# yamiel-abreu/distributed-pytorch-training

Hardware: AMD Instinct MI355X
Metric: images/sec (whole node) ResNet-50 bf16 training (higher is better)
Workload: dtype bf16

## Files before the change

csrc/bindings.cpp:

```cpp
#include <ATen/ATen.h>
#include <c10/hip/HIPGuard.h>
#include <c10/hip/HIPStream.h>
#include <torch/extension.h>

#include "kernels/kernels.h"
#include "host_comm.h"
#include "pg_comm.h"
#include "rccl_comm.h"
#include "watchdog.h"
#include "reducer.h"

namespace py = pybind11;
using at::Tensor;

namespace {

hipStream_t cur_stream(const Tensor& t) {
  return c10::hip::getCurrentHIPStream(t.device().index()).stream();
}

dpt::WireType wire_of(const Tensor& t) {
  switch (t.scalar_type()) {
    case at::kFloat: return dpt::WireType::kF32;
    case at::kBFloat16: return dpt::WireType::kBF16;
// ... 607 lines not shown
  dpt::launch_im2col(x.data_ptr(), x.scalar_type() == at::kBFloat16, reinterpret_cast<uint16_t*>(a.data_ptr()), N, H,
                     W, C, (int)R, (int)S, (int)stride, (int)pad, (int)Kp, cur_stream(x));
  return a;
}

void check_bf16_contig(const Tensor& t, const char* name) {
  TORCH_CHECK(t.is_cuda() && t.scalar_type() == at::kBFloat16 && t.is_contiguous(), name,
              " must be a contiguous bf16 GPU tensor");
  TORCH_CHECK(reinterpret_cast<uintptr_t>(t.data_ptr()) % 16 == 0, name, " must be 16-byte aligned");
}

std::vector<Tensor> attn_fwd(Tensor qkv, int64_t heads, double scale) {
  check_bf16_contig(qkv, "qkv");
  TORCH_CHECK(qkv.dim() == 3 && qkv.size(2) == 3 * heads * 64, "attn_fwd: qkv must be [B, S, 3*H*64]");
  const int B = qkv.size(0), S = qkv.size(1), H = heads;
  TORCH_CHECK(dpt::attn_supported(S, 64), "attn_fwd: needs S <= 256 and head dim 64");
  auto ctx = at::empty({B, S, H * 64}, qkv.options());
  auto lse = at::empty({(int64_t)B * H, dpt::attn_lse_stride(S)}, qkv.options().dtype(at::kFloat));
  if (B * H == 0) return {ctx, lse};
  c10::hip::HIPGuard guard(qkv.device().index());
  dpt::launch_attn_fwd(reinterpret_cast<const uint16_t*>(qkv.data_ptr()), reinterpret_cast<uint16_t*>(ctx.data_ptr()),
                       lse.data_ptr<float>(), B, S, H, (float)scale, cur_stream(qkv));
  return {ctx, lse};
}

Tensor attn_bwd(Tensor qkv, Tensor out, Tensor dout, Tensor lse, int64_t heads, double scale) {
  check_bf16_contig(qkv, "qkv");
  check_bf16_contig(out, "out");
  check_bf16_contig(dout, "grad_output");
  TORCH_CHECK(qkv.dim() == 3, "attn_bwd: qkv must be [B, S, 3*H*64]");
  const int B = qkv.size(0), S = qkv.size(1), H = heads;
  TORCH_CHECK(dpt::attn_supported(S, 64), "attn_bwd: needs S <= 256 and head dim 64");
  TORCH_CHECK(out.sizes() == dout.sizes() && out.dim() == 3 && out.size(0) == B && out.size(1) == S &&
                  out.size(2) == H * 64 && qkv.size(2) == 3 * H * 64, "attn_bwd: shape mismatch");
  TORCH_CHECK(lse.is_cuda() && lse.scalar_type() == at::kFloat && lse.is_contiguous() &&
                  lse.numel() == (int64_t)B * H * dpt::attn_lse_stride(S), "attn_bwd: bad lse");
  auto dqkv = at::empty_like(qkv);
  if (B * H == 0) return dqkv;
  c10::hip::HIPGuard guard(qkv.device().index());
  dpt::launch_attn_bwd(reinterpret_cast<const uint16_t*>(qkv.data_ptr()), reinterpret_cast<const uint16_t*>(out.data_ptr()),
                       reinterpret_cast<const uint16_t*>(dout.data_ptr()), lse.data_ptr<float>(),
                       reinterpret_cast<uint16_t*>(dqkv.data_ptr()), B, S, H, (float)scale, cur_stream(qkv));
  return dqkv;
}

std::vector<Tensor> attn_stream_fwd(Tensor qkv, int64_t heads, double scale) {
  check_bf16_contig(qkv, "qkv");
  TORCH_CHECK(qkv.dim() == 3 && qkv.size(2) == 3 * heads * 64, "attn_stream_fwd: qkv must be [B, S, 3*H*64]");
  const int B = qkv.size(0), S = qkv.size(1), H = heads;
  TORCH_CHECK(dpt::attn_stream_supported(S, 64), "attn_stream_fwd: needs 1 <= S <= 4096 and head dim 64");
  TORCH_CHECK((int64_t)B * H * ((S + 31) / 32) < (1LL << 31), "attn_stream_fwd: B * H * S too large for one grid");
  auto ctx = at::empty({B, S, H * 64}, qkv.options());
  auto lse = at::empty({(int64_t)B * H, dpt::attn_lse_stride(S)}, qkv.options().dtype(at::kFloat));
  if (B * H == 0) return {ctx, lse};
  c10::hip::HIPGuard guard(qkv.device().index());
  dpt::launch_attn_stream_fwd(reinterpret_cast<const uint16_t*>(qkv.data_ptr()),
                              reinterpret_cast<uint16_t*>(ctx.data_ptr()), lse.data_ptr<float>(), B, S, H,
                              (float)scale, cur_stream(qkv));
  return {ctx, lse};
}

Tensor attn_stream_bwd(Tensor qkv, Tensor out, Tensor dout, Tensor lse, int64_t heads, double scale) {
  check_bf16_contig(qkv, "qkv");
  check_bf16_contig(out, "out");
  check_bf16_contig(dout, "grad_output");
  TORCH_CHECK(qkv.dim() == 3, "attn_stream_bwd: qkv must be [B, S, 3*H*64]");
  const int B = qkv.size(0), S = qkv.size(1), H = heads;
  TORCH_CHECK(dpt::attn_stream_supported(S, 64), "attn_stream_bwd: needs 1 <= S <= 4096 and head dim 64");
  TORCH_CHECK(out.sizes() == dout.sizes() && out.dim() == 3 && out.size(0) == B && out.size(1) == S &&
                  out.size(2) == H * 64 && qkv.size(2) == 3 * H * 64, "attn_stream_bwd: shape mismatch");
  TORCH_CHECK(lse.is_cuda() && lse.scalar_type() == at::kFloat && lse.is_contiguous() &&
                  lse.numel() == (int64_t)B * H * dpt::attn_lse_stride(S), "attn_stream_bwd: bad lse");
  TORCH_CHECK((int64_t)B * H * ((S + 31) / 32) < (1LL << 31), "attn_stream_bwd: B * H * S too large for one grid");
  auto dqkv = at::empty_like(qkv);
  if (B * H == 0) return dqkv;
  auto dsum = at::empty_like(lse);
  c10::hip::HIPGuard guard(qkv.device().index());
  dpt::launch_attn_stream_bwd(reinterpret_cast<const uint16_t*>(qkv.data_ptr()),
                              reinterpret_cast<const uint16_t*>(out.data_ptr()),
                              reinterpret_cast<const uint16_t*>(dout.data_ptr()), lse.data_ptr<float>(),
                              dsum.data_ptr<float>(), reinterpret_cast<uint16_t*>(dqkv.data_ptr()), B, S, H,
                              (float)scale, cur_stream(qkv));
  return dqkv;
}

std::tuple<int64_t, int64_t, int64_t> attn_stream_tiles() {
  int qb, kc, qc;
  dpt::attn_stream_tiles(&qb, &kc, &qc);
  return {qb, kc, qc};
}

Tensor space_to_depth2(Tensor x, bool out_f16) {
  TORCH_CHECK(x.is_cuda() && x.dim() == 4 && (x.scalar_type() == at::kFloat || x.scalar_type() == at::kBFloat16),
              "space_to_depth2: x must be a 4-d fp32/bf16 GPU tensor");
  TORCH_CHECK(x.is_contiguous(at::MemoryFormat::ChannelsLast), "space_to_depth2: x must be channels_last");
  const int N = x.size(0), C = x.size(1), H = x.size(2), W = x.size(3);
  TORCH_CHECK(C <= 4 && H % 2 == 0 && W % 2 == 0, "space_to_depth2: needs C <= 4 and even H, W");
  auto a = at::empty({N, 16, H / 2, W / 2},
                     x.options().dtype(out_f16 ? at::kHalf : at::kBFloat16).memory_format(at::MemoryFormat::ChannelsLast));
  c10::hip::HIPGuard guard(x.device().index());
  dpt::launch_space_to_depth2(x.data_ptr(), x.scalar_type() == at::kBFloat16, reinterpret_cast<uint16_t*>(a.data_ptr()),
                              N, H, W, C, cur_stream(x), out_f16);
  return a;
}

std::vector<Tensor> bn_fwd_train(Tensor x, c10::optional<Tensor> residual, c10::optional<Tensor> weight,
                                 c10::optional<Tensor> bias, c10::optional<Tensor> running_mean,
                                 c10::optional<Tensor> running_var, c10::optional<Tensor> num_batches,
                                 double momentum, double eps, bool relu, c10::optional<Tensor> psum,
                                 c10::optional<Tensor> psq, bool apply, c10::optional<Tensor> mask_out) {
  auto [M, C] = bn_rows(x, "x");
  TORCH_CHECK(dpt::bn_supported(C), "fused BN: unsupported channel count ", C);
  const void* rp = nullptr;
  if (residual.has_value() && residual->defined()) {
    TORCH_CHECK(residual->sizes() == x.sizes() && residual->scalar_type() == x.scalar_type(), "residual mismatch");
    bn_rows(*residual, "residual");
    rp = residual->data_ptr();
  }
  int64_t* nb = nullptr;
  if (num_batches.has_value() && num_batches->defined()) {
    TORCH_CHECK(num_batches->is_cuda() && num_batches->scalar_type() == at::kLong, "num_batches must be int64 GPU");
    nb = num_batches->data_ptr<int64_t>();
  }
  auto y = apply ? at::empty_like(x) : at::empty({0}, x.options());
  void* yp = apply ? y.data_ptr() : nullptr;
  auto fopt = x.options().dtype(at::kFloat);
  auto mean = at::empty({C}, fopt), invstd = at::empty({C}, fopt);
  auto coef = at::empty({2 * C}, fopt);
  uint8_t* mp = relu_mask_ptr(mask_out, M, C, x, "bn_fwd_train");
  TORCH_CHECK(mp == nullptr || (relu && rp != nullptr && apply), "bn_fwd_train: mask_out needs relu + residual");
  c10::hip::HIPGuard guard(x.device().index());
  if (psum.has_value() && psum->defined()) {
    TORCH_CHECK(psq.has_value() && psq->defined(), "bn_fwd_train: psum without psq");
    TORCH_CHECK(psum->is_cuda() && psum->scalar_type() == at::kFloat && psum->dim() == 2 && psum->size(0) == C &&
                    psum->is_contiguous() && psq->sizes() == psum->sizes() && psq->is_contiguous(),
                "bn_fwd_train: partials must be contiguous fp32 [C, chunks]");
    dpt::launch_bn_fwd_from_partials(bn_dtype(x), x.data_ptr(), rp, yp, M, C, psum->data_ptr<float>(),
                                     psq->data_ptr<float>(), (int)psum->size(1), f32_param(weight, C, "weight"),
                                     f32_param(bias, C, "bias"), (float)eps, (float)momentum,
                                     f32_param(running_mean, C, "running_mean"),
                                     f32_param(running_var, C, "running_var"), nb, mean.data_ptr<float>(),
                                     invstd.data_ptr<float>(), coef.data_ptr<float>(), relu, cur_stream(x), mp);
    return {y, mean, invstd, coef};
  }
  auto ws = at::empty({dpt::bn_workspace_floats(M, C)}, fopt);
  dpt::launch_bn_fwd_train(bn_dtype(x), x.data_ptr(), rp, yp, M, C, f32_param(weight, C, "weight"),
                           f32_param(bias, C, "bias"), (float)eps, (float)momentum,
                           f32_param(running_mean, C, "running_mean"), f32_param(running_var, C, "running_var"), nb,
                           mean.data_ptr<float>(), invstd.data_ptr<float>(), coef.data_ptr<float>(),
                           ws.data_ptr<float>(), relu, cur_stream(x), mp);
  return {y, mean, invstd, coef};
}

Tensor bn_apply_aff(Tensor x, Tensor x2, Tensor coef, Tensor coef2, c10::optional<Tensor> mask_out) {
  auto [M, C] = bn_rows(x, "x");
  TORCH_CHECK(dpt::bn_supported(C), "fused BN: unsupported channel count ", C);
  TORCH_CHECK(x2.sizes() == x.sizes() && x2.scalar_type() == x.scalar_type(), "bn_apply_aff: x2 mismatch");
  bn_rows(x2, "x2");
  const float* a = f32_param(coef, 2 * C, "coef");
  const float* a2 = f32_param(coef2, 2 * C, "coef2");
  auto y = at::empty_like(x);
  c10::hip::HIPGuard guard(x.device().index());
  uint8_t* mp = relu_mask_ptr(mask_out, M, C, x, "bn_apply_aff");
  dpt::launch_bn_apply_aff(bn_dtype(x), x.data_ptr(), x2.data_ptr(), y.data_ptr(), M, C, a, a + C, a2, a2 + C,
                           cur_stream(x), mp);
  return y;
}

std::vector<Tensor> bn2_bwd_partials(Tensor dz, Tensor x, Tensor x2, c10::optional<Tensor> weight,
                                     c10::optional<Tensor> weight2, Tensor mean, Tensor invstd, Tensor mean2,
                                     Tensor invstd2, Tensor p1, Tensor p2, Tensor p3, bool want_dparams) {
  auto [M, C] = bn_rows(x, "x");
  TORCH_CHECK(dz.sizes() == x.sizes() && x2.sizes() == x.sizes() && dz.scalar_type() == x.scalar_type() &&
                  x2.scalar_type() == x.scalar_type(), "bn2_bwd_partials: shape/dtype mismatch");
  bn_rows(dz, "dz");
  bn_rows(x2, "x2");
  for (const Tensor* t : {&p1, &p2, &p3})
    TORCH_CHECK(t->is_cuda() && t->scalar_type() == at::kFloat && t->dim() == 2 && t->size(0) == C &&
                    t->is_contiguous() && t->sizes() == p1.sizes(), "bn2_bwd_partials: partials must be fp32 [C, chunks]");
  auto fopt = x.options().dtype(at::kFloat);
  auto dx = at::empty_like(x), dx2 = at::empty_like(x2);
  Tensor dg = want_dparams ? at::empty({C}, fopt) : Tensor(), db = want_dparams ? at::empty({C}, fopt) : Tensor();
  Tensor dg2 = want_dparams ? at::empty({C}, fopt) : Tensor(), db2 = want_dparams ? at::empty({C}, fopt) : Tensor();
  auto kbuf = at::empty({6 * C}, fopt);
  c10::hip::HIPGuard guard(x.device().index());
  dpt::launch_bn2_bwd_from_partials(
      bn_dtype(x), dz.data_ptr(), x.data_ptr(), x2.data_ptr(), M, C, f32_param(weight, C, "weight"),
      f32_param(mean, C, "mean"), f32_param(invstd, C, "invstd"), f32_param(weight2, C, "weight2"),
      f32_param(mean2, C, "mean2"), f32_param(invstd2, C, "invstd2"), p1.data_ptr<float>(), p2.data_ptr<float>(),
      p3.data_ptr<float>(), (int)p1.size(1), want_dparams ? dg.data_ptr<float>() : nullptr,
      want_dparams ? db.data_ptr<float>() : nullptr, want_dparams ? dg2.data_ptr<float>() : nullptr,
      want_dparams ? db2.data_ptr<float>() : nullptr, dx.data_ptr(), dx2.data_ptr(), kbuf.data_ptr<float>(),
      cur_stream(x));
  return {dx, dx2, dg, db, dg2, db2};
}

Tensor bn_apply(Tensor x, c10::optional<Tensor> residual, Tensor a, Tensor b, bool relu) {
  auto [M, C] = bn_rows(x, "x");
  TORCH_CHECK(dpt::bn_supported(C), "fused BN: unsupported channel count ", C);
  const void* rp = nullptr;
  if (residual.has_value() && residual->defined()) {
    TORCH_CHECK(residual->sizes() == x.sizes() && residual->scalar_type() == x.scalar_type(), "residual mismatch");
    bn_rows(*residual, "residual");
    rp = residual->data_ptr();
  }
  auto y = at::empty_like(x);
  c10::hip::HIPGuard guard(x.device().index());
  dpt::launch_bn_apply(bn_dtype(x), x.data_ptr(), rp, y.data_ptr(), M, C, f32_param(a, C, "a"),
                       f32_param(b, C, "b"), relu, cur_stream(x));
  return y;
}

std::vector<Tensor> bn_bwd(Tensor dy, c10::optional<Tensor> dy2, c10::optional<Tensor> y, Tensor x,
                           c10::optional<Tensor> weight, Tensor mean, Tensor invstd, bool relu, bool want_dz,
                           bool want_dparams, c10::optional<Tensor> coef) {
  auto [M, C] = bn_rows(x, "x");
  auto [Md, Cd] = bn_rows(dy, "grad_output");
  TORCH_CHECK(M == Md && C == Cd && dy.scalar_type() == x.scalar_type(), "grad_output mismatch");
  const void* d2 = nullptr;
  if (dy2.has_value() && dy2->defined()) {
    auto [M2, C2] = bn_rows(*dy2, "grad_output2");
    TORCH_CHECK(M2 == M && C2 == C && dy2->scalar_type() == x.scalar_type(), "grad_output2 mismatch");
    d2 = dy2->data_ptr();
  }
  const bool make_dz = want_dz || d2 != nullptr;
  const float* cp = nullptr;
  if (relu && !make_dz && coef.has_value() && coef->defined()) cp = f32_param(*coef, 2 * C, "coef");
  const void* yp = nullptr;
  if (relu && cp == nullptr) {
    TORCH_CHECK(y.has_value() && y->defined(), "relu backward needs the saved output (or coef)");
    bn_rows(*y, "y");
    yp = y->data_ptr();
  }
  auto fopt = x.options().dtype(at::kFloat);
  auto dx = at::empty_like(x);
  Tensor dz = make_dz ? at::empty_like(x) : Tensor();
  Tensor dg = want_dparams ? at::empty({C}, fopt) : Tensor();
  Tensor db = want_dparams ? at::empty({C}, fopt) : Tensor();
  auto ws = at::empty({dpt::bn_workspace_floats(M, C)}, fopt);
  c10::hip::HIPGuard guard(x.device().index());
  dpt::launch_bn_bwd(bn_dtype(x), dy.data_ptr(), d2, yp, x.data_ptr(), M, C, f32_param(weight, C, "weight"),
                     f32_param(mean, C, "mean"), f32_param(invstd, C, "invstd"), cp,
                     want_dparams ? dg.data_ptr<float>() : nullptr, want_dparams ? db.data_ptr<float>() : nullptr,
                     dx.data_ptr(), make_dz ? dz.data_ptr() : nullptr, ws.data_ptr<float>(), relu, cur_stream(x));
  return {dx, dg, db, dz};
}

std::vector<Tensor> bn_bwd_partials(Tensor dy, Tensor x, c10::optional<Tensor> weight, Tensor mean, Tensor invstd,
                                    c10::optional<Tensor> coef, Tensor p1, Tensor p2, bool want_dparams, bool from_dz) {
  auto [M, C] = bn_rows(x, "x");
  auto [Md, Cd] = bn_rows(dy, "grad_output");
  TORCH_CHECK(M == Md && C == Cd && dy.scalar_type() == x.scalar_type(), "grad_output mismatch");
  TORCH_CHECK(p1.is_cuda() && p1.scalar_type() == at::kFloat && p1.dim() == 2 && p1.size(0) == C &&
                  p1.is_contiguous() && p2.sizes() == p1.sizes() && p2.is_contiguous(),
              "bn_bwd_partials: partials must be contiguous fp32 [C, chunks]");
  TORCH_CHECK(from_dz || (coef.has_value() && coef->defined()), "bn_bwd_partials: coef needed unless from_dz");
  auto fopt = x.options().dtype(at::kFloat);
  auto dx = at::empty_like(x);
  Tensor dg = want_dparams ? at::empty({C}, fopt) : Tensor();
  Tensor db = want_dparams ? at::empty({C}, fopt) : Tensor();
  auto kbuf = at::empty({3 * C}, fopt);
  c10::hip::HIPGuard guard(x.device().index());
  dpt::launch_bn_bwd_from_partials(bn_dtype(x), dy.data_ptr(), x.data_ptr(), M, C, f32_param(weight, C, "weight"),
                                   f32_param(mean, C, "mean"), f32_param(invstd, C, "invstd"),
                                   f32_param(coef, 2 * C, "coef"), p1.data_ptr<float>(), p2.data_ptr<float>(),
                                   (int)p1.size(1), want_dparams ? dg.data_ptr<float>() : nullptr,
                                   want_dparams ? db.data_ptr<float>() : nullptr, dx.data_ptr(), kbuf.data_ptr<float>(),
                                   cur_stream(x), from_dz);
  return {dx, dg, db};
}

std::vector<Tensor> maxpool_fwd(Tensor x, int64_t k, int64_t stride, int64_t pad, c10::optional<Tensor> bn_coef) {
  TORCH_CHECK(x.is_cuda() && x.dim() == 4 && x.is_contiguous(at::MemoryFormat::ChannelsLast),
              "maxpool: x must be a 4-D channels_last GPU tensor");
  const int64_t B = x.size(0), C = x.size(1), H = x.size(2), W = x.size(3);
  TORCH_CHECK(!(bn_coef.has_value() && bn_coef->defined()) || k == 3, "maxpool: the folded BN needs a 3x3 window");
  TORCH_CHECK(C % 8 == 0 && k >= 1 && k * k <= 255 && stride >= 1 && pad >= 0 && pad <= k / 2, "maxpool: bad config");
  const int64_t Ho = (H + 2 * pad - k) / stride + 1, Wo = (W + 2 * pad - k) / stride + 1;
  auto y = at::empty({B, C, Ho, Wo}, x.options().memory_format(at::MemoryFormat::ChannelsLast));
  auto idx = at::empty({B, C, Ho, Wo}, x.options().dtype(at::kByte).memory_format(at::MemoryFormat::ChannelsLast));
  c10::hip::HIPGuard guard(x.device().index());
  dpt::launch_maxpool_fwd(bn_dtype(x), x.data_ptr(), y.data_ptr(), idx.data_ptr<uint8_t>(), B, (int)H, (int)W,
                          (int)C, (int)Ho, (int)Wo, (int)k, (int)stride, (int)pad, cur_stream(x),
                          bn_coef.has_value() && bn_coef->defined() ? f32_param(bn_coef, 2 * C, "bn_coef") : nullptr);
  
  return {y, idx};
}

std::vector<Tensor> maxpool_bwd(Tensor dy, Tensor idx, int64_t H, int64_t W, int64_t k, int64_t stride, int64_t pad,
                                c10::optional<Tensor> dy2, c10::optional<Tensor> bn_x, c10::optional<Tensor> bn_mean,
                                c10::optional<Tensor> bn_coef) {
  TORCH_CHECK(dy.is_cuda() && dy.dim() == 4 && dy.is_contiguous(at::MemoryFormat::ChannelsLast),
              "maxpool_bwd: grad must be channels_last");
  TORCH_CHECK(idx.sizes() == dy.sizes() && idx.scalar_type() == at::kByte &&
                  idx.is_contiguous(at::MemoryFormat::ChannelsLast), "maxpool_bwd: idx mismatch");
  const int64_t B = dy.size(0), C = dy.size(1), Ho = dy.size(2), Wo = dy.size(3);
  TORCH_CHECK(C % 8 == 0 && Ho == (H + 2 * pad - k) / stride + 1 && Wo == (W + 2 * pad - k) / stride + 1,
              "maxpool_bwd: geometry mismatch");
  const bool two = dy2.has_value() && dy2->defined();
  if (two)
    TORCH_CHECK(dy2->sizes() == dy.sizes() && dy2->scalar_type() == dy.scalar_type() &&
                    dy2->is_contiguous(at::MemoryFormat::ChannelsLast), "maxpool_bwd: dy2 must match grad_output");
  auto dx = at::empty({B, C, H, W}, dy.options().memory_format(at::MemoryFormat::ChannelsLast));
  const bool bns = bn_x.has_value() && bn_x->defined();
  Tensor p1, p2;
  if (bns) {
    TORCH_CHECK(k == 3 && stride == 2 && pad == 1, "maxpool_bwd: BN statistics only for the 3x3/2/1 pool");
    TORCH_CHECK(C <= 512 && (C & (C - 1)) == 0, "maxpool_bwd: BN statistics need a power-of-two C <= 512");
    TORCH_CHECK(bn_x->sizes() == dx.sizes() && bn_x->scalar_type() == dy.scalar_type() &&
                    bn_x->is_contiguous(at::MemoryFormat::ChannelsLast), "maxpool_bwd: bn_x must match dx");
    const int chunks = dpt::maxpool_bwd_bn_chunks(B, (int)H, (int)W, (int)C);
    p1 = at::empty({C, chunks}, dy.options().dtype(at::kFloat));
    p2 = at::empty({C, chunks}, dy.options().dtype(at::kFloat));
  }
  c10::hip::HIPGuard guard(dy.device().index());
  dpt::launch_maxpool_bwd(bn_dtype(dy), dy.data_ptr(), two ? dy2->data_ptr() : nullptr, idx.data_ptr<uint8_t>(),
                          dx.data_ptr(), B, (int)H, (int)W,
                          (int)C, (int)Ho, (int)Wo, (int)k, (int)stride, (int)pad, cur_stream(dy), bns ? bn_x->data_ptr() : nullptr,
                          bns ? f32_param(bn_mean, C, "bn_mean") : nullptr, bns ? f32_param(bn_coef, 2 * C, "bn_coef") : nullptr,
                          bns ? p1.data_ptr<float>() : nullptr, bns ? p2.data_ptr<float>() : nullptr);
  if (bns) return {dx, p1, p2};
  
  return {dx};
}

std::vector<Tensor> gap_bwd_bnr(Tensor g, Tensor y, Tensor x, Tensor mean) {
  TORCH_CHECK(g.is_cuda() && g.dim() == 2 && g.is_contiguous(), "gap_bwd_bnr: g must be a contiguous [N, C]");
  auto [M, C] = bn_rows(y, "y");
  auto [Mx, Cx] = bn_rows(x, "x");
  TORCH_CHECK(M == Mx && C == Cx && x.scalar_type() == y.scalar_type() && g.size(1) == C && g.size(0) == y.size(0),
              "gap_bwd_bnr: shape mismatch");
  TORCH_CHECK(C % 8 == 0 && 256 % (C / 8) == 0, "gap_bwd_bnr: needs C/8 | 256");
  const int64_t N = y.size(0), HW = y.size(2) * y.size(3);
  auto dz = at::empty_like(y);
  const int chunks = dpt::gap_bwd_bnr_chunks(M, C);
  auto p1 = at::empty({C, chunks}, y.options().dtype(at::kFloat));
  auto p2 = at::empty({C, chunks}, y.options().dtype(at::kFloat));
  c10::hip::HIPGuard guard(y.device().index());
  dpt::launch_gap_bwd_bnr(bn_dtype(y), bn_dtype(g), g.data_ptr(), dz.data_ptr(), y.data_ptr(), x.data_ptr(),
                          f32_param(mean, C, "mean"), N, HW, C, p1.data_ptr<float>(), p2.data_ptr<float>(),
                          cur_stream(y));
  return {dz, p1, p2};
}

Tensor gap_bwd(Tensor g, int64_t H, int64_t W, at::ScalarType dtype) {
  TORCH_CHECK(g.is_cuda() && g.dim() == 2 && g.is_contiguous() && g.size(1) % 8 == 0, "gap_bwd: g must be [N, C], C % 8 == 0");
  TORCH_CHECK(dtype == at::kFloat || dtype == at::kBFloat16 || dtype == at::kHalf, "gap_bwd: dtype");
  const int64_t N = g.size(0), C = g.size(1);
  TORCH_CHECK(N * H * W * (C / 8) < (int64_t(1) << 32) - 256, "gap_bwd: too large");
  auto dx = at::empty({N, C, H, W}, g.options().dtype(dtype).memory_format(at::MemoryFormat::ChannelsLast));
  c10::hip::HIPGuard guard(g.device().index());
  dpt::launch_gap_bwd(bn_dtype(dx), bn_dtype(g), g.data_ptr(), dx.data_ptr(), N, H * W, C, cur_stream(g));
  return dx;
}

int act16_kind(const Tensor& t, const char* name) {
  TORCH_CHECK(t.is_cuda() && t.is_contiguous(), name, " must be a contiguous GPU tensor");
  if (t.scalar_type() == at::kBFloat16) return 1;
  TORCH_CHECK(t.scalar_type() == at::kHalf, name, " must be bf16 or fp16");
  return 2;
}

int param_kind(const Tensor& t, int64_t D, const char* name) {
// ... 74 lines not shown
                     want_dparams ? dg.data_ptr<float>() : nullptr, want_dparams ? db.data_ptr<float>() : nullptr,
                     dbias.defined() ? dbias.data_ptr() : nullptr, dbk, T, D, cur_stream(sv));
  return {gx, ga, dg, db, dbias};
}

Tensor gelu_fwd(Tensor u, c10::optional<Tensor> bias) {
  const int kind = act16_kind(u, "gelu: u");
  const int64_t F = u.size(-1), T = u.numel() / F;
  TORCH_CHECK(F % 8 == 0, "gelu: width must be a multiple of 8");
  const void* bp = nullptr;
  int bk = 0;
  if (bias.has_value() && bias->defined()) {
    bk = param_kind(*bias, F, "gelu: bias");
    bp = bias->data_ptr();
  }
  auto h = at::empty_like(u);
  c10::hip::HIPGuard guard(u.device().index());
  dpt::launch_gelu_fwd(kind, static_cast<const uint16_t*>(u.data_ptr()), bp, bk, static_cast<uint16_t*>(h.data_ptr()),
                       T, F, cur_stream(u));
  return h;
}

std::vector<Tensor> gelu_bwd(Tensor gh, Tensor u, c10::optional<Tensor> bias, bool want_dbias) {
  const int kind = act16_kind(u, "gelu_bwd: u");
  TORCH_CHECK(act16_kind(gh, "gelu_bwd: grad") == kind && gh.sizes() == u.sizes(), "gelu_bwd: grad must match u");
  const int64_t F = u.size(-1), T = u.numel() / F;
  TORCH_CHECK(F % 8 == 0, "gelu_bwd: width must be a multiple of 8");
  const void* bp = nullptr;
  int bk = 0;
  if (bias.has_value() && bias->defined()) {
    bk = param_kind(*bias, F, "gelu_bwd: bias");
    bp = bias->data_ptr();
  }
  auto gu = at::empty_like(u);
  Tensor db = (want_dbias && bp) ? at::empty({F}, u.options().dtype(bias->scalar_type())) : Tensor();
  auto part = at::empty({(int64_t)dpt::gelu_bwd_chunks(T, F) * F}, u.options().dtype(at::kFloat));
  c10::hip::HIPGuard guard(u.device().index());
  dpt::launch_gelu_bwd(kind, static_cast<const uint16_t*>(gh.data_ptr()), static_cast<const uint16_t*>(u.data_ptr()),
                       bp, bk, static_cast<uint16_t*>(gu.data_ptr()), part.data_ptr<float>(),
                       db.defined() ? db.data_ptr() : nullptr, bk, T, F, cur_stream(u));
  return {gu, db};
}

std::vector<Tensor> linear_dgrad_dgelu(Tensor dy, Tensor wt, Tensor u, Tensor bias) {
  const int kind = act16_kind(u, "linear_dgrad_dgelu: u");
  TORCH_CHECK(act16_kind(dy, "linear_dgrad_dgelu: grad") == kind && act16_kind(wt, "linear_dgrad_dgelu: wt") == kind,
              "linear_dgrad_dgelu: grad, wt and u must share one 16-bit dtype");
  TORCH_CHECK(dy.dim() == 2 && wt.dim() == 2 && u.dim() == 2 && dy.is_contiguous() && wt.is_contiguous() &&
                  u.is_contiguous(), "linear_dgrad_dgelu: contiguous 2-D operands");
  const int64_t T = dy.size(0), n_out = dy.size(1), n_in = wt.size(0);
  TORCH_CHECK(wt.size(1) == n_out && u.size(0) == T && u.size(1) == n_in, "linear_dgrad_dgelu: shape mismatch");
  TORCH_CHECK(n_in % 128 == 0 && n_out % 64 == 0, "linear_dgrad_dgelu: n_in % 128 == 0 and n_out % 64 == 0");
  const bool b16 = bias.scalar_type() == u.scalar_type();
  TORCH_CHECK((b16 || bias.scalar_type() == at::kFloat) && bias.is_contiguous() && bias.numel() == n_in &&
                  bias.is_cuda(), "linear_dgrad_dgelu: fp32 or u-typed bias of n_in elements on the device");
  TORCH_CHECK(T * n_out < (1ll << 31) && T * n_in < (1ll << 31), "linear_dgrad_dgelu: too many elements");
  auto gu = at::empty_like(u);
  auto part = at::empty({(int64_t)dpt::linear_dgrad_dgelu_tiles(T), n_in}, u.options().dtype(at::kFloat));
  c10::hip::HIPGuard guard(u.device().index());
  dpt::launch_linear_dgrad_dgelu(static_cast<const uint16_t*>(dy.data_ptr()), static_cast<const uint16_t*>(wt.data_ptr()),
                                 static_cast<const uint16_t*>(u.data_ptr()),
                                 b16 ? nullptr : bias.data_ptr<float>(),
                                 b16 ? static_cast<const uint16_t*>(bias.data_ptr()) : nullptr,
                                 static_cast<uint16_t*>(gu.data_ptr()), part.data_ptr<float>(), T, (int)n_out,
                                 (int)n_in, kind == 2, cur_stream(u));
  return {gu, part};
}

Tensor bias_grad16(Tensor gy, int64_t out_kind) {
  const int kind = act16_kind(gy, "bias_grad16: grad");
  const int64_t F = gy.size(-1), T = gy.numel() / F;
  TORCH_CHECK(F % 8 == 0 && (out_kind >= 0 && out_kind <= 2), "bias_grad16: F % 8 == 0, kind 0..2");
  auto db = at::empty({F}, gy.options().dtype(out_kind == 0 ? at::kFloat : kind_dtype((int)out_kind)));
  auto part = at::empty({(int64_t)dpt::gelu_bwd_chunks(T, F) * F}, gy.options().dtype(at::kFloat));
  c10::hip::HIPGuard guard(gy.device().index());
  dpt::launch_bias_grad16(kind, static_cast<const uint16_t*>(gy.data_ptr()), part.data_ptr<float>(), db.data_ptr(),
                          (int)out_kind, T, F, cur_stream(gy));
  return db;
}

Tensor sum_partials(Tensor part, int64_t out_kind) {
  TORCH_CHECK(part.is_cuda() && part.scalar_type() == at::kFloat && part.is_contiguous() && part.dim() >= 2,
              "sum_partials: contiguous fp32 [S, ...]");
  const int64_t S = part.size(0), n = part.numel() / S;
  TORCH_CHECK(n % 4 == 0 && out_kind >= 0 && out_kind <= 2, "sum_partials: n % 4 == 0, kind 0..2");
  auto out = at::empty(part.sizes().slice(1),
                       part.options().dtype(out_kind == 0 ? at::kFloat : kind_dtype((int)out_kind)));
  c10::hip::HIPGuard guard(part.device().index());
  dpt::launch_sum_partials(part.data_ptr<float>(), n, (int)S, out.data_ptr(), (int)out_kind, cur_stream(part));
  return out;
}

Tensor colsum_rows(Tensor part, int64_t out_kind) {
  TORCH_CHECK(part.is_cuda() && part.scalar_type() == at::kFloat && part.is_contiguous() && part.dim() == 2,
              "colsum_rows: contiguous fp32 [n, D]");
  TORCH_CHECK(out_kind >= 0 && out_kind <= 2, "colsum_rows: kind 0..2");
  auto out = at::empty({part.size(1)}, part.options().dtype(out_kind == 0 ? at::kFloat : kind_dtype((int)out_kind)));
  c10::hip::HIPGuard guard(part.device().index());
  dpt::launch_colsum_rows(part.data_ptr<float>(), part.size(0), part.size(1), out.data_ptr(), (int)out_kind,
                          cur_stream(part));
  return out;
}

void copy_rows16(Tensor src, Tensor dst) {
  TORCH_CHECK(src.is_cuda() && dst.is_cuda() && src.device() == dst.device(), "copy_rows16: GPU tensors");
  TORCH_CHECK(src.scalar_type() == dst.scalar_type() && src.element_size() == 2, "copy_rows16: same 16-bit dtype");
  TORCH_CHECK(src.sizes() == dst.sizes() && src.dim() >= 1 && src.dim() <= 5, "copy_rows16: same shape, <= 5 dims");
  const int nd = (int)src.dim();
  const int64_t L = src.size(nd - 1);
  TORCH_CHECK(src.stride(nd - 1) == 1 && dst.stride(nd - 1) == 1 && L % 8 == 0, "copy_rows16: rows must be contiguous, L % 8 == 0");
  TORCH_CHECK(reinterpret_cast<uintptr_t>(src.data_ptr()) % 16 == 0 && reinterpret_cast<uintptr_t>(dst.data_ptr()) % 16 == 0,
              "copy_rows16: 16-byte aligned data");
  int n[4] = {1, 1, 1, 1};
  int64_t ss[4] = {0, 0, 0, 0}, ds[4] = {0, 0, 0, 0};
  for (int d = 0; d < nd - 1; ++d) {
    const int slot = 4 - (nd - 1) + d;
    TORCH_CHECK(src.size(d) < (1LL << 31), "copy_rows16: dim too large");
    TORCH_CHECK(src.stride(d) % 8 == 0 && dst.stride(d) % 8 == 0, "copy_rows16: row starts must be 16-byte aligned");
    n[slot] = (int)src.size(d);
    ss[slot] = src.stride(d);
    ds[slot] = dst.stride(d);
  }
  TORCH_CHECK((int64_t)n[0] * n[1] * n[2] * n[3] < (1LL << 32), "copy_rows16: too many rows");
  c10::hip::HIPGuard guard(src.device().index());
  dpt::launch_rows_copy16(static_cast<const uint16_t*>(src.data_ptr()), static_cast<uint16_t*>(dst.data_ptr()), n, ss,
                          ds, (int)L, cur_stream(src));
}

}

PYBIND11_MODULE(TORCH_EXTENSION_NAME, m) {
  m.doc() = "MI355X-native runtime: gfx950 kernels, RCCL communicator, C++ gradient reducer";
  m.def("grad_check", &grad_check, py::arg("grad"), py::arg("scale"), py::arg("host_factor"), py::arg("found_inf"));
  m.def("sgd_step", &sgd_step, py::arg("param"), py::arg("grad"), py::arg("momentum_buffer"), py::arg("lr"),
        py::arg("momentum"), py::arg("dampening"), py::arg("weight_decay"), py::arg("nesterov"), py::arg("scale"),
        py::arg("host_factor"), py::arg("found_inf"), py::arg("step"), py::arg("zero_grad"),
        py::arg("shadow") = py::none());
  m.def("adam_step", &adam_step, py::arg("param"), py::arg("grad"), py::arg("exp_avg"), py::arg("exp_avg_sq"),
        py::arg("lr"), py::arg("beta1"), py::arg("beta2"), py::arg("eps"), py::arg("weight_decay"), py::arg("adamw"),
        py::arg("scale"), py::arg("host_factor"), py::arg("found_inf"), py::arg("step"), py::arg("zero_grad"),
        py::arg("shadow") = py::none());
  m.def("optim_tail", &optim_tail, py::arg("scale"), py::arg("growth_tracker"), py::arg("found_inf"),
        py::arg("step"), py::arg("growth_factor"), py::arg("backoff_factor"), py::arg("growth_interval"));
  m.def("pack_bf16", &pack_bf16);
  m.def("unpack_bf16", &unpack_bf16);
  m.def("accumulate_metrics", &accumulate_metrics, py::arg("logits"), py::arg("targets"), py::arg("loss"), py::arg("acc"));
  m.def("augment", &augment, py::arg("data"), py::arg("idx"), py::arg("offs"), py::arg("flips"), py::arg("out"),
        py::arg("nhwc"), py::arg("pad"), py::arg("mean"), py::arg("std"));
  m.def("bn_supported", [](int64_t C) { return dpt::bn_supported(C); });
  m.def("bn_fwd_train", &bn_fwd_train, py::arg("x"), py::arg("residual"), py::arg("weight"), py::arg("bias"),
        py::arg("running_mean"), py::arg("running_var"), py::arg("num_batches"), py::arg("momentum"), py::arg("eps"),
        py::arg("relu"), py::arg("psum") = py::none(), py::arg("psq") = py::none(), py::arg("apply") = true,
        py::arg("mask_out") = py::none());
  m.def("bn_apply", &bn_apply, py::arg("x"), py::arg("residual"), py::arg("a"), py::arg("b"), py::arg("relu"));
  m.def("bn_apply_aff", &bn_apply_aff, py::arg("x"), py::arg("x2"), py::arg("coef"), py::arg("coef2"),
        py::arg("mask_out") = py::none());
  m.def("bn2_bwd_partials", &bn2_bwd_partials, py::arg("dz"), py::arg("x"), py::arg("x2"), py::arg("weight"),
        py::arg("weight2"), py::arg("mean"), py::arg("invstd"), py::arg("mean2"), py::arg("invstd2"), py::arg("p1"),
        py::arg("p2"), py::arg("p3"), py::arg("want_dparams"));
  m.def("bn_bwd", &bn_bwd, py::arg("grad_output"), py::arg("grad_output2"), py::arg("y"), py::arg("x"),
        py::arg("weight"), py::arg("mean"), py::arg("invstd"), py::arg("relu"), py::arg("want_dz"),
        py::arg("want_dparams"), py::arg("coef") = py::none());
  m.def("ln_supported", &dpt::ln_supported, py::arg("D"));
  m.def("ln_fwd", &ln_fwd, py::arg("x"), py::arg("a"), py::arg("bias"), py::arg("gamma"), py::arg("beta"),
        py::arg("eps"), py::arg("out_kind") = 1);
  m.def("ln_bwd", &ln_bwd, py::arg("grad_s"), py::arg("grad_h"), py::arg("s"), py::arg("mean"), py::arg("rstd"),
        py::arg("gamma"), py::arg("want_ga"), py::arg("bias_like"), py::arg("want_dparams"));
  m.def("gelu_fwd", &gelu_fwd, py::arg("u"), py::arg("bias"));
  m.def("gelu_bwd", &gelu_bwd, py::arg("grad"), py::arg("u"), py::arg("bias"), py::arg("want_dbias"));
  m.def("linear_dgrad_dgelu", &linear_dgrad_dgelu, py::arg("grad"), py::arg("wt"), py::arg("u"), py::arg("bias"));
  m.def("vit_set_gelu_blocks_per_cu", &dpt::vit_set_gelu_blocks_per_cu, py::arg("n"));
  m.def("copy_rows16", &copy_rows16, py::arg("src"), py::arg("dst"));
  m.def("bias_grad16", &bias_grad16, py::arg("grad"), py::arg("out_kind"));
  m.def("sum_partials", &sum_partials, py::arg("part"), py::arg("out_kind"));
  m.def("colsum_rows", &colsum_rows, py::arg("part"), py::arg("out_kind"));
  m.def("maxpool_fwd", &maxpool_fwd, py::arg("x"), py::arg("k"), py::arg("stride"), py::arg("pad"),
        py::arg("bn_coef") = py::none());
  m.def("gap_bwd", &gap_bwd, py::arg("g"), py::arg("H"), py::arg("W"), py::arg("dtype"));
  m.def("gap_bwd_bnr", &gap_bwd_bnr, py::arg("g"), py::arg("y"), py::arg("x"), py::arg("mean"));
  m.def("maxpool_bwd", &maxpool_bwd, py::arg("grad_output"), py::arg("idx"), py::arg("H"), py::arg("W"),
        py::arg("k"), py::arg("stride"), py::arg("pad"), py::arg("grad_output2") = py::none(),
        py::arg("bn_x") = py::none(), py::arg("bn_mean") = py::none(), py::arg("bn_coef") = py::none());
  m.def("conv_fwd", &conv_fwd, py::arg("x"), py::arg("w"), py::arg("stride"), py::arg("pad"), py::arg("want_stats"),
        py::arg("out_h") = 0, py::arg("out_w") = 0);
  m.def("space_to_depth2", &space_to_depth2, py::arg("x"), py::arg("out_f16") = false);
  m.def("conv_wgrad", &conv_wgrad, py::arg("grad_output"), py::arg("x"), py::arg("weight_shape"), py::arg("stride"),
        py::arg("pad"), py::arg("fp32_out"), py::arg("target_blocks") = 0);
  m.def("conv_f32_fwd", &conv_f32_fwd, py::arg("x"), py::arg("w"), py::arg("stride"), py::arg("pad"),
        py::arg("split") = false);
  m.def("conv_f32_dgrad", &conv_f32_dgrad, py::arg("grad_output"), py::arg("w"), py::arg("stride"), py::arg("pad"),
        py::arg("H"), py::arg("W"), py::arg("split") = false);
  m.def("conv_f32_wgrad", &conv_f32_wgrad, py::arg("grad_output"), py::arg("x"), py::arg("weight_shape"),
        py::arg("stride"), py::arg("pad"), py::arg("split") = false);
  m.def("im2col", &im2col, py::arg("x"), py::arg("R"), py::arg("S"), py::arg("stride"), py::arg("pad"), py::arg("Kp"));
  m.def("attn_fwd", &attn_fwd, py::arg("qkv"), py::arg("heads"), py::arg("scale"));
  m.def("attn_set_bwd_split", &dpt::attn_set_bwd_split, py::arg("on"));
  m.def("attn_bwd", &attn_bwd, py::arg("qkv"), py::arg("out"), py::arg("grad_output"), py::arg("lse"),
        py::arg("heads"), py::arg("scale"));
  m.def("attn_stream_fwd", &attn_stream_fwd, py::arg("qkv"), py::arg("heads"), py::arg("scale"));
  m.def("attn_stream_bwd", &attn_stream_bwd, py::arg("qkv"), py::arg("out"), py::arg("grad_output"), py::arg("lse"),
        py::arg("heads"), py::arg("scale"));
  m.def("attn_stream_tiles", &attn_stream_tiles,
        "(queries per workgroup, keys per chunk, query rows per backward chunk) of the streaming attention kernels");
  m.def("conv_set_variant", &dpt::conv_set_variant, py::arg("variant"));
  m.def("bn_set_skip_finalize", &dpt::bn_set_skip_finalize, py::arg("on"),
        "measurement only: skip every BatchNorm finalize launch (wrong values; timing upper bound)");
  m.def("conv_set_splitk_policy", &dpt::conv_set_splitk_policy, py::arg("tiles"), py::arg("eager_tiles"),
        py::arg("eager_min_k"), py::arg("target"), "split-K thresholds (A/B knob; <= 0 keeps a value)");
  m.def("conv_set_big", &dpt::conv_set_big, py::arg("on"));
  m.def("conv_set_halo", &dpt::conv_set_halo, py::arg("on"));
  m.def("conv_set_breg", &dpt::conv_set_breg, py::arg("mode"));
  m.def("conv_set_wgrad_stages", &dpt::conv_set_wgrad_stages, py::arg("mode"));
  m.def("conv_get_breg", &dpt::conv_get_breg);
  m.def("conv_set_streamk", &dpt::conv_set_streamk, py::arg("mode"), py::arg("eff") = 0.0);
  m.def("conv_get_streamk", &dpt::conv_get_streamk);
  m.def("conv_sk_prepare", &dpt::conv_sk_prepare);
  m.def("conv_sk_errors", &dpt::conv_sk_errors);
  m.def("conv_sk_blocks", &dpt::conv_sk_blocks, py::arg("tiles"), py::arg("nk"), py::arg("bn"), py::arg("mode"));
  m.def("conv_set_wgrad_target", &dpt::conv_set_wgrad_target, py::arg("blocks"));
  m.def("conv_set_wgrad_halo", &dpt::conv_set_wgrad_halo, py::arg("mode"));
  m.def("conv_fwd_splits", [](int64_t M, int Cout, int64_t K, bool graph) {
          return dpt::conv_fwd_splits_for(M, Cout, K, graph);
        }, py::arg("M"), py::arg("Cout"), py::arg("K"), py::arg("graph") = false);
  m.def("conv_set_splitk", &dpt::conv_set_splitk, py::arg("mode"));
  m.def("conv_get_splitk", &dpt::conv_get_splitk);
  m.def("conv_set_fwd_shape_policy", &dpt::conv_set_fwd_shape_policy, py::arg("bits"));
  m.def("conv_dgrad", &conv_dgrad, py::arg("grad_output"), py::arg("w"), py::arg("pad"));
  m.def("conv_dgrad_bnstats", &conv_dgrad_bnstats, py::arg("grad_output"), py::arg("w"), py::arg("pad"),
        py::arg("bn_x"), py::arg("bn_mean"), py::arg("bn_coef"), py::arg("bn_y") = py::none(),
        py::arg("bn_res") = py::none(), py::arg("w_flipped") = py::none(), py::arg("bn_x2") = py::none(),
        py::arg("bn_mean2") = py::none(), py::arg("wgrad_reduce") = nullptr, py::arg("bn_mask") = py::none(),
        py::arg("bn_res_s2") = false);
  m.def("conv_wt_flip_multi", &conv_wt_flip_multi, py::arg("ws"));
  m.def("conv_dgrad_preflipped", &conv_dgrad_preflipped, py::arg("grad_output"), py::arg("w_flipped"), py::arg("pad"),
        py::arg("wgrad_reduce") = nullptr);
  m.def("bn_bwd_partials", &bn_bwd_partials, py::arg("grad_output"), py::arg("x"), py::arg("weight"), py::arg("mean"),
        py::arg("invstd"), py::arg("coef"), py::arg("p1"), py::arg("p2"), py::arg("want_dparams"),
        py::arg("from_dz") = false);
  m.def("conv_dgrad_s2", &conv_dgrad_s2, py::arg("grad_output"), py::arg("w"), py::arg("pad"), py::arg("H"),
        py::arg("W"), py::arg("bn_x") = py::none(), py::arg("bn_mean") = py::none(), py::arg("bn_coef") = py::none(),
        py::arg("wgrad_reduce") = nullptr, py::arg("compact") = false);
  m.def("conv_dgrad_flip", &conv_dgrad_flip, py::arg("grad_output"), py::arg("w"), py::arg("pad"),
        py::arg("wgrad_reduce") = nullptr);
  py::class_<PendingReduce, PendingReducePtr>(m, "PendingWgradReduce")
      .def_property_readonly("done", &PendingReduce::done)
      .def_property_readonly("splits", [](const PendingReduce& p) { return p.r.splits; });
  m.def("conv_wgrad_deferred", &conv_wgrad_deferred, py::arg("grad_output"), py::arg("x"), py::arg("weight_shape"),
        py::arg("stride"), py::arg("pad"));
  m.def("conv_reduce_flush", &conv_reduce_flush, py::arg("pending"));
  m.def("rccl_version", []() { return std::string(dpt::rccl_version_string()); });

  py::class_<dpt::Collective, std::shared_ptr<dpt::Collective>>(m, "Collective")
      .def("all_reduce", [](dpt::Collective& c, Tensor t, bool on_current_stream) {
             TORCH_CHECK(t.is_cuda() && t.is_contiguous(), "all_reduce needs a contiguous GPU tensor");
             c10::hip::HIPGuard guard(t.device().index());
             hipStream_t s = cur_stream(t);
             c.all_reduce(t.data_ptr(), (size_t)t.numel(), wire_of(t), on_current_stream ? s : c.stream());
           }, py::arg("tensor"), py::arg("on_current_stream") = true)
      .def("broadcast", [](dpt::Collective& c, Tensor t, int root) {
             TORCH_CHECK(t.is_cuda() && t.is_contiguous(), "broadcast needs a contiguous GPU tensor");
             c10::hip::HIPGuard guard(t.device().index());
             c.broadcast(t.data_ptr(), (size_t)t.numel(), wire_of(t), root, cur_stream(t));
           }, py::arg("tensor"), py::arg("root") = 0)
      .def("abort", &dpt::Collective::abort)
      .def("destroy", &dpt::Collective::destroy)
      .def("check", &dpt::Collective::check)
      .def_property_readonly("kind", &dpt::Collective::kind)
      .def_property_readonly("ops", &dpt::Collective::ops)
      .def_property_readonly("sequence_hash", &dpt::Collective::sequence_hash)
      .def_property_readonly("rank", &dpt::Collective::rank)
      .def_property_readonly("world_size", &dpt::Collective::world_size)
      .def_property_readonly("device", &dpt::Collective::device)
      .def("track", [](dpt::Collective& c) {
             c10::hip::HIPGuard guard(c.device());
             c.track(c10::hip::getCurrentHIPStream(c.device()).stream());
           }, "hand the watchdog a completion marker for the work enqueued on the current stream")
      .def("_test_spin", [](dpt::Collective& c, double ms, bool on_current_stream) {
             TORCH_CHECK(ms >= 0 && ms <= 20000, "spin: 0..20000 ms");
             c10::hip::HIPGuard guard(c.device());
             dpt::launch_spin(ms, on_current_stream ? c10::hip::getCurrentHIPStream(c.device()).stream()
                                                    : c.stream());
           }, py::arg("ms"), py::arg("on_current_stream") = false,
           "test hook: enqueue a wall-clock busy-wait on the communicator (or current) stream");

  py::class_<dpt::RcclComm, dpt::Collective, std::shared_ptr<dpt::RcclComm>>(m, "RcclComm")
      .def(py::init<const std::string&, int, int, int, int, int, double>(), py::arg("unique_id"), py::arg("rank"),
           py::arg("world_size"), py::arg("device"), py::arg("min_ctas") = 0, py::arg("max_ctas") = 0,
           py::arg("init_timeout_s") = 0.0,
           py::call_guard<py::gil_scoped_release>())
      .def_property_readonly("min_ctas", &dpt::RcclComm::min_ctas)
      .def_property_readonly("max_ctas", &dpt::RcclComm::max_ctas)
      .def_property_readonly("handle", &dpt::RcclComm::handle)
      .def("inject_async_error", &dpt::RcclComm::inject_async_error, py::arg("message"))
      .def_static("new_unique_id", []() { return py::bytes(dpt::RcclComm::new_unique_id()); })
      .def("enable_watchdog", &dpt::RcclComm::enable_watchdog, py::arg("timeout_s"), py::arg("poll_s") = 0.5,
           py::arg("exit_grace_s") = 30.0)
      .def_property_readonly("watchdog_tripped", &dpt::RcclComm::watchdog_tripped)
      .def_property_readonly("watchdog_outstanding", &dpt::RcclComm::watchdog_outstanding)
      .def_property_readonly("watchdog_tracked", &dpt::RcclComm::watchdog_tracked)
      .def("async_error", &dpt::RcclComm::async_error);

  py::class_<dpt::HostBridgeComm, dpt::Collective, std::shared_ptr<dpt::HostBridgeComm>>(m, "HostBridgeComm")
      .def(py::init([](py::object ar, py::object bc, int rank, int ws, int dev, bool async_mode, py::object pg) {
             c10::intrusive_ptr<c10d::ProcessGroup> p;
             if (!pg.is_none()) p = pg.cast<c10::intrusive_ptr<c10d::ProcessGroup>>();
             return std::make_shared<dpt::HostBridgeComm>(std::move(ar), std::move(bc), rank, ws, dev, async_mode,
                                                          std::move(p));
           }),
           py::arg("all_reduce_fn"), py::arg("broadcast_fn"), py::arg("rank"), py::arg("world_size"),
// ... 56 lines not shown
```

csrc/kernels/bn_kernels.hip:

```cpp
#include <cstdlib>

#include "carry.h"
#include "common.h"
#include "kernels.h"

namespace dpt {

struct BF16 {
  using raw = uint16_t;
  __device__ static void load8(const void* p, int64_t i, float f[8]) {
    uint4 w = *reinterpret_cast<const uint4*>(static_cast<const uint16_t*>(p) + i);
    uint32_t u[4] = {w.x, w.y, w.z, w.w};
#pragma unroll
    for (int k = 0; k < 4; ++k) {
      f[2 * k] = bf16_to_f32(u[k] & 0xffff);
      f[2 * k + 1] = bf16_to_f32(u[k] >> 16);
    }
  }
  __device__ static void store8(void* p, int64_t i, const float f[8]) {
    uint4 w;
    w.x = (uint32_t)f32_to_bf16(f[0]) | ((uint32_t)f32_to_bf16(f[1]) << 16);
    w.y = (uint32_t)f32_to_bf16(f[2]) | ((uint32_t)f32_to_bf16(f[3]) << 16);
    w.z = (uint32_t)f32_to_bf16(f[4]) | ((uint32_t)f32_to_bf16(f[5]) << 16);
    w.w = (uint32_t)f32_to_bf16(f[6]) | ((uint32_t)f32_to_bf16(f[7]) << 16);
    *reinterpret_cast<uint4*>(static_cast<uint16_t*>(p) + i) = w;
  }
  __device__ static bool pos16(uint32_t h) { return !(h & 0x8000u) && (h & 0x7fffu) && (h & 0x7fffu) <= 0x7f80u; }
  __device__ static uint32_t store8m(void* p, int64_t i, const float f[8]) {
    uint32_t h[8];
#pragma unroll
    for (int k = 0; k < 8; ++k) h[k] = f32_to_bf16(f[k]);
    *reinterpret_cast<uint4*>(static_cast<uint16_t*>(p) + i) =
        make_uint4(h[0] | (h[1] << 16), h[2] | (h[3] << 16), h[4] | (h[5] << 16), h[6] | (h[7] << 16));
    uint32_t m = 0;
#pragma unroll
    for (int k = 0; k < 8; ++k) m |= (pos16(h[k]) ? 1u : 0u) << k;
    return m;
  }
  __device__ static void pos8(const void* p, int64_t i, bool m[8]) {
    uint4 w = *reinterpret_cast<const uint4*>(static_cast<const uint16_t*>(p) + i);
    uint32_t u[4] = {w.x, w.y, w.z, w.w};
#pragma unroll
    for (int k = 0; k < 4; ++k) {
      uint16_t lo = u[k] & 0xffff, hi = u[k] >> 16;
      m[2 * k] = !(lo & 0x8000) && (lo & 0x7fff) && (lo & 0x7fff) <= 0x7f80;
      m[2 * k + 1] = !(hi & 0x8000) && (hi & 0x7fff) && (hi & 0x7fff) <= 0x7f80;
    }
  }
};

struct F16 {
  __device__ static void load8(const void* p, int64_t i, float f[8]) {
    uint4 w = *reinterpret_cast<const uint4*>(static_cast<const uint16_t*>(p) + i);
    uint32_t u[4] = {w.x, w.y, w.z, w.w};
#pragma unroll
    for (int k = 0; k < 4; ++k) {
      f[2 * k] = f16_to_f32(u[k] & 0xffff);
      f[2 * k + 1] = f16_to_f32(u[k] >> 16);
    }
  }
  __device__ static uint16_t to16(float v) { return __builtin_bit_cast(uint16_t, (_Float16)v); }
  __device__ static void store8(void* p, int64_t i, const float f[8]) {
    uint4 w;
    w.x = (uint32_t)to16(f[0]) | ((uint32_t)to16(f[1]) << 16);
    w.y = (uint32_t)to16(f[2]) | ((uint32_t)to16(f[3]) << 16);
    w.z = (uint32_t)to16(f[4]) | ((uint32_t)to16(f[5]) << 16);
    w.w = (uint32_t)to16(f[6]) | ((uint32_t)to16(f[7]) << 16);
    *reinterpret_cast<uint4*>(static_cast<uint16_t*>(p) + i) = w;
  }
  __device__ static uint32_t store8m(void* p, int64_t i, const float f[8]) {
    store8(p, i, f);
    uint32_t m = 0;
#pragma unroll
    for (int k = 0; k < 8; ++k) m |= ((float)__builtin_bit_cast(_Float16, to16(f[k])) > 0.0f ? 1u : 0u) << k;
    return m;
  }
  __device__ static void pos8(const void* p, int64_t i, bool m[8]) {
    float f[8];
    load8(p, i, f);
#pragma unroll
    for (int k = 0; k < 8; ++k) m[k] = f[k] > 0.0f;
  }
};

struct F32 {
  __device__ static void load8(const void* p, int64_t i, float f[8]) {
    const float4* q = reinterpret_cast<const float4*>(static_cast<const float*>(p) + i);
    float4 a = q[0], b = q[1];
    f[0] = a.x; f[1] = a.y; f[2] = a.z; f[3] = a.w; f[4] = b.x; f[5] = b.y; f[6] = b.z; f[7] = b.w;
  }
  __device__ static void store8(void* p, int64_t i, const float f[8]) {
    float4* q = reinterpret_cast<float4*>(static_cast<float*>(p) + i);
    q[0] = make_float4(f[0], f[1], f[2], f[3]);
    q[1] = make_float4(f[4], f[5], f[6], f[7]);
  }
  __device__ static uint32_t store8m(void* p, int64_t i, const float f[8]) {
    store8(p, i, f);
    uint32_t m = 0;
#pragma unroll
    for (int k = 0; k < 8; ++k) m |= (f[k] > 0.0f ? 1u : 0u) << k;
    return m;
  }
  __device__ static void pos8(const void* p, int64_t i, bool m[8]) {
    float f[8];
    load8(p, i, f);
#pragma unroll
    for (int k = 0; k < 8; ++k) m[k] = f[k] > 0.0f;
  }
};

template <typename IO>
__global__ __launch_bounds__(kBlock) void bn_fwd_stats_kernel(const void* __restrict__ x, int64_t M, int C,
                                                              int64_t rows_per_chunk, int chunks,
                                                              float* __restrict__ psum,
                                                              float* __restrict__ psq) {
  __shared__ float lds[2 * kBlock * 8];
  const int tpr = C >> 3, rpi = kBlock / tpr;
  const int cg = threadIdx.x % tpr, rr = threadIdx.x / tpr;
  const int64_t row0 = (int64_t)blockIdx.x * rows_per_chunk;
  const int64_t row1 = min(row0 + rows_per_chunk, M);
  float s[8] = {0, 0, 0, 0, 0, 0, 0, 0}, q[8] = {0, 0, 0, 0, 0, 0, 0, 0};
  int64_t r = row0 + rr;
  for (; r + 3 * rpi < row1; r += 4 * rpi) {
    float a[4][8];
#pragma unroll
    for (int u = 0; u < 4; ++u) IO::load8(x, (r + u * rpi) * C + cg * 8, a[u]);
#pragma unroll
    for (int u = 0; u < 4; ++u)
#pragma unroll
      for (int k = 0; k < 8; ++k) {
        s[k] += a[u][k];
        q[k] += a[u][k] * a[u][k];
      }
  }
  for (; r < row1; r += rpi) {
    float a[8];
    IO::load8(x, r * C + cg * 8, a);
#pragma unroll
    for (int k = 0; k < 8; ++k) { s[k] += a[k]; q[k] += a[k] * a[k]; }
  }
  float* ls = lds;
  float* lq = lds + kBlock * 8;
#pragma unroll
  for (int k = 0; k < 8; ++k) {
    ls[rr * C + cg * 8 + k] = s[k];
    lq[rr * C + cg * 8 + k] = q[k];
  }
  __syncthreads();
  for (int c = threadIdx.x; c < C; c += kBlock) {
    float ts = 0.f, tq = 0.f;
    for (int j = 0; j < rpi; ++j) { ts += ls[j * C + c]; tq += lq[j * C + c]; }
    psum[(int64_t)c * chunks + blockIdx.x] = ts;
    psq[(int64_t)c * chunks + blockIdx.x] = tq;
  }
}

__global__ __launch_bounds__(kBlock) void bn_fwd_finalize_kernel(
    const float* __restrict__ psum, const float* __restrict__ psq, int chunks, int C, int64_t M,
    const float* __restrict__ gamma, const float* __restrict__ beta, float eps, float momentum,
    float* run_mean, float* run_var, int64_t* num_batches, float* save_mean, float* save_invstd,
    float* coef_a, float* coef_b) {
  const int lane = threadIdx.x & 63, wave = threadIdx.x >> 6;
  const int64_t c = (int64_t)blockIdx.x * 8 + wave * 2 + (lane >> 5);
  const int part = lane & 31;
  if (blockIdx.x == 0 && threadIdx.x == 0 && num_batches) num_batches[0] += 1;
  if (c >= C) return;
  double s, q;
  half_wave_sum2(psum, psq, c, chunks, part, s, q);
  if (part != 0) return;
  const double mean = s / (double)M;
  double var = q / (double)M - mean * mean;
  if (var < 0.0) var = 0.0;
  const float invstd = (float)(1.0 / sqrt(var + (double)eps));
  const float g = gamma ? gamma[c] : 1.0f, bt = beta ? beta[c] : 0.0f;
  const float a = g * invstd;
  save_mean[c] = (float)mean;
  save_invstd[c] = invstd;
  coef_a[c] = a;
  coef_b[c] = bt - (float)mean * a;
  if (run_mean) {
    const double unbiased = M > 1 ? var * (double)M / (double)(M - 1) : var;
    run_mean[c] = (1.0f - momentum) * run_mean[c] + momentum * (float)mean;
    run_var[c] = (1.0f - momentum) * run_var[c] + momentum * (float)unbiased;
  }
}


template <int NT>
__global__ __launch_bounds__(NT) void bn_fwd_finalize_wide_kernel(
    const float* __restrict__ psum, const float* __restrict__ psq, int chunks, int C, int64_t M,
    const float* __restrict__ gamma, const float* __restrict__ beta, float eps, float momentum,
    float* run_mean, float* run_var, int64_t* num_batches, float* save_mean, float* save_invstd,
    float* coef_a, float* coef_b) {
  __shared__ double red[2][NT / 64];
  const int c = blockIdx.x, lane = threadIdx.x & 63, wave = threadIdx.x >> 6;
  if (c == 0 && threadIdx.x == 0 && num_batches) num_batches[0] += 1;
  double s, q;
  block_row_sum2<NT>(psum + (int64_t)c * chunks, psq + (int64_t)c * chunks, chunks, s, q);
  if (lane == 0) { red[0][wave] = s; red[1][wave] = q; }
  __syncthreads();
  if (threadIdx.x != 0) return;
  s = 0.0;
  q = 0.0;
#pragma unroll
  for (int w = 0; w < NT / 64; ++w) { s += red[0][w]; q += red[1][w]; }
  const double mean = s / (double)M;
  double var = q / (double)M - mean * mean;
  if (var < 0.0) var = 0.0;
  const float invstd = (float)(1.0 / sqrt(var + (double)eps));
  const float g = gamma ? gamma[c] : 1.0f, bt = beta ? beta[c] : 0.0f;
  const float a = g * invstd;
  save_mean[c] = (float)mean;
  save_invstd[c] = invstd;
  coef_a[c] = a;
  coef_b[c] = bt - (float)mean * a;
  if (run_mean) {
    const double unbiased = M > 1 ? var * (double)M / (double)(M - 1) : var;
    run_mean[c] = (1.0f - momentum) * run_mean[c] + momentum * (float)mean;
    run_var[c] = (1.0f - momentum) * run_var[c] + momentum * (float)unbiased;
  }
}

template <typename IO, bool RELU, bool RES, bool AFF = false>
__global__ __launch_bounds__(kBlock) void bn_fwd_apply_kernel(const void* __restrict__ x,
                                                              const void* __restrict__ res,
                                                              void* __restrict__ y,
                                                              const float* __restrict__ coef_a,
                                                              const float* __restrict__ coef_b,
                                                              int64_t M, int C, int rev,
                                                              const float* __restrict__ coef_a2 = nullptr,
                                                              const float* __restrict__ coef_b2 = nullptr,
                                                              uint8_t* __restrict__ mask = nullptr) {
  const int tpr = C >> 3, rpi = kBlock / tpr;
  const int cg = threadIdx.x % tpr, rr = threadIdx.x / tpr;
  float a[8], b[8], a2[8], b2[8];
#pragma unroll
  for (int k = 0; k < 8; ++k) {
    a[k] = coef_a[cg * 8 + k];
    b[k] = coef_b[cg * 8 + k];
    a2[k] = AFF ? coef_a2[cg * 8 + k] : 0.f;
    b2[k] = AFF ? coef_b2[cg * 8 + k] : 0.f;
  }
  const int64_t stride = (int64_t)gridDim.x * rpi;
  for (int64_t rf = (int64_t)blockIdx.x * rpi + rr; rf < M; rf += 2 * stride) {
    const bool two = rf + stride < M;
    const int64_t r = rev ? M - 1 - rf : rf;
    const int64_t r2 = rev ? r - stride : r + stride;
    float v0[8], v1[8], q0[8], q1[8];
    IO::load8(x, r * C + cg * 8, v0);
    if (two) IO::load8(x, r2 * C + cg * 8, v1);
    if (RES) {
      IO::load8(res, r * C + cg * 8, q0);
      if (two) IO::load8(res, r2 * C + cg * 8, q1);
    }
#pragma unroll
    for (int k = 0; k < 8; ++k) {
      float o0 = __builtin_fmaf(v0[k], a[k], b[k]);
      float o1 = __builtin_fmaf(v1[k], a[k], b[k]);
      if (RES && AFF) {
        o0 += __builtin_fmaf(q0[k], a2[k], b2[k]);
        o1 += __builtin_fmaf(q1[k], a2[k], b2[k]);
      } else if (RES) {
// ... 173 lines not shown
    mu[k] = mean[cg * 8 + k];
    c1[k] = k1[cg * 8 + k];
    c2[k] = k2[cg * 8 + k];
    c3[k] = k3[cg * 8 + k];
    fa[k] = MX ? coef[cg * 8 + k] : 0.f;
    fb[k] = MX ? coef[C + cg * 8 + k] : 0.f;
  }
  const int64_t stride = (int64_t)apply_grid * rpi;
  for (int64_t rf = (int64_t)blockIdx.x * rpi + rr; rf < M; rf += stride) {
    const int64_t r = rev ? M - 1 - rf : rf;
    float g[8], xv[8], o[8];
    bool m[8];
    IO::load8(dy, r * C + cg * 8, g);
    IO::load8(x, r * C + cg * 8, xv);
    if (RELU && !FROM_DZ) relu_mask8<IO, MX>(y, r * C + cg * 8, xv, fa, fb, m);
#pragma unroll
    for (int k = 0; k < 8; ++k) {
      float dz = (FROM_DZ || !RELU || m[k]) ? g[k] : 0.0f;
      o[k] = c1[k] * dz + c2[k] * (xv[k] - mu[k]) + c3[k];
    }
    IO::store8(dx, r * C + cg * 8, o);
  }
}

template <typename IO>
__global__ __launch_bounds__(kBlock) void bn_bwd_apply2_kernel(const void* __restrict__ dz,
                                                               const void* __restrict__ x,
                                                               const void* __restrict__ x2,
                                                               const float* __restrict__ mean,
                                                               const float* __restrict__ mean2,
                                                               const float* __restrict__ k,
                                                               const float* __restrict__ j, void* dx, void* dx2,
                                                               int64_t M, int C, int rev) {
  const int tpr = C >> 3, rpi = kBlock / tpr;
  const int cg = threadIdx.x % tpr, rr = threadIdx.x / tpr;
  float mu[8], mu2[8], c1[8], c2[8], c3[8], e1[8], e2[8], e3[8];
#pragma unroll
  for (int q = 0; q < 8; ++q) {
    const int c = cg * 8 + q;
    mu[q] = mean[c];
    mu2[q] = mean2[c];
    c1[q] = k[c]; c2[q] = k[C + c]; c3[q] = k[2 * C + c];
    e1[q] = j[c]; e2[q] = j[C + c]; e3[q] = j[2 * C + c];
  }
  const int64_t stride = (int64_t)gridDim.x * rpi;
  for (int64_t rf = (int64_t)blockIdx.x * rpi + rr; rf < M; rf += stride) {
    const int64_t r = rev ? M - 1 - rf : rf;
    const int64_t off = r * C + cg * 8;
    float g[8], xv[8], x2v[8], o[8], o2[8];
    IO::load8(dz, off, g);
    IO::load8(x, off, xv);
    IO::load8(x2, off, x2v);
#pragma unroll
    for (int q = 0; q < 8; ++q) {
      o[q] = c1[q] * g[q] + c2[q] * (xv[q] - mu[q]) + c3[q];
      o2[q] = e1[q] * g[q] + e2[q] * (x2v[q] - mu2[q]) + e3[q];
    }
    IO::store8(dx, off, o);
    IO::store8(dx2, off, o2);
  }
}

bool bn_supported(int64_t C) {
  return C >= 8 && C % 8 == 0 && C <= 8 * kBlock && kBlock % (C / 8) == 0;
}

constexpr int kBnMaxChunks = 512;
constexpr int kBnBwdUnroll = 2;
constexpr int kBnApplyMax = 32768;
constexpr int kBnBwdApplyMax = 4 * kMaxBlocks;
constexpr int kBnReverse = 1;

BnGeometry bn_geometry(int64_t M, int64_t C) {
  BnGeometry g;
  const int64_t rpi = kBlock / (C / 8);
  int64_t rows = (M + kBnMaxChunks - 1) / kBnMaxChunks;
  if (rows < 64) rows = 64;
  rows = (rows + rpi - 1) / rpi * rpi;
  g.rows_per_chunk = rows;
  g.chunks = (int)((M + rows - 1) / rows);
  if (g.chunks < 1) g.chunks = 1;
  int64_t apply = (M + rpi * 2 - 1) / (rpi * 2);
  g.apply_blocks = (int)(apply < 1 ? 1 : (apply > kBnApplyMax ? kBnApplyMax : apply));
  return g;
}

template <typename IO>
static void fwd_apply_dispatch(bool relu, bool res, const void* x, const void* r, void* y, const float* a,
                               const float* b, int64_t M, int C, int blocks, hipStream_t s, uint8_t* mask = nullptr) {
  dim3 gr(blocks), bl(kBlock);
  const int rev = kBnReverse;
  if (relu && res)
    hipLaunchKernelGGL((bn_fwd_apply_kernel<IO, true, true>), gr, bl, 0, s, x, r, y, a, b, M, C, rev, nullptr, nullptr,
                       mask);
  else if (relu) hipLaunchKernelGGL((bn_fwd_apply_kernel<IO, true, false>), gr, bl, 0, s, x, r, y, a, b, M, C, rev);
  else if (res) hipLaunchKernelGGL((bn_fwd_apply_kernel<IO, false, true>), gr, bl, 0, s, x, r, y, a, b, M, C, rev);
  else hipLaunchKernelGGL((bn_fwd_apply_kernel<IO, false, false>), gr, bl, 0, s, x, r, y, a, b, M, C, rev);
}

void launch_bn_fwd_train(int dtype, const void* x, const void* res, void* y, int64_t M, int64_t C,
                         const float* gamma, const float* beta, float eps, float momentum, float* run_mean,
                         float* run_var, int64_t* num_batches, float* save_mean, float* save_invstd,
                         float* save_coef, float* workspace, bool relu, hipStream_t s, uint8_t* mask) {
  BnGeometry g = bn_geometry(M, C);
  float* psum = workspace;
  float* psq = psum + (int64_t)C * g.chunks;
  float* ca = save_coef ? save_coef : psq + (int64_t)C * g.chunks;
  float* cb = ca + C;
  dim3 bl(kBlock);
  switch (dtype) {
    case 0: hipLaunchKernelGGL(bn_fwd_stats_kernel<F32>, dim3(g.chunks), bl, 0, s, x, M, (int)C, g.rows_per_chunk, g.chunks, psum, psq); break;
    case 1: hipLaunchKernelGGL(bn_fwd_stats_kernel<BF16>, dim3(g.chunks), bl, 0, s, x, M, (int)C, g.rows_per_chunk, g.chunks, psum, psq); break;
    default: hipLaunchKernelGGL(bn_fwd_stats_kernel<F16>, dim3(g.chunks), bl, 0, s, x, M, (int)C, g.rows_per_chunk, g.chunks, psum, psq); break;
  }
  hipLaunchKernelGGL(bn_fwd_finalize_kernel, dim3((unsigned)((C + 7) / 8)), bl, 0, s, psum, psq, g.chunks, (int)C, M,
                     gamma, beta, eps, momentum, run_mean, run_var, num_batches, save_mean, save_invstd, ca, cb);
  if (y == nullptr) return;
  switch (dtype) {
    case 0: fwd_apply_dispatch<F32>(relu, res != nullptr, x, res, y, ca, cb, M, (int)C, g.apply_blocks, s, mask); break;
    case 1: fwd_apply_dispatch<BF16>(relu, res != nullptr, x, res, y, ca, cb, M, (int)C, g.apply_blocks, s, mask); break;
    default: fwd_apply_dispatch<F16>(relu, res != nullptr, x, res, y, ca, cb, M, (int)C, g.apply_blocks, s, mask); break;
  }
}

void launch_bn_fwd_from_partials(int dtype, const void* x, const void* res, void* y, int64_t M, int64_t C,
                                 const float* psum, const float* psq, int chunks, const float* gamma,
                                 const float* beta, float eps, float momentum, float* run_mean, float* run_var,
                                 int64_t* num_batches, float* save_mean, float* save_invstd, float* save_coef,
                                 bool relu, hipStream_t s, uint8_t* mask) {
  BnGeometry g = bn_geometry(M, C);
  float* ca = save_coef;
  float* cb = ca + C;
  if (g_bn_skip_finalize) {
  } else if (chunks > 256) {
#define DPT_FWD_FIN(NT)                                                                                        \
  hipLaunchKernelGGL(bn_fwd_finalize_wide_kernel<NT>, dim3((unsigned)C), dim3(NT), 0, s, psum, psq, chunks, (int)C, \
                     M, gamma, beta, eps, momentum, run_mean, run_var, num_batches, save_mean, save_invstd, ca, cb)
    if (chunks > 8192) DPT_FWD_FIN(1024);
    else DPT_FWD_FIN(kBlock);
#undef DPT_FWD_FIN
  } else
    hipLaunchKernelGGL(bn_fwd_finalize_kernel, dim3((unsigned)((C + 7) / 8)), dim3(kBlock), 0, s, psum, psq, chunks,
                       (int)C, M, gamma, beta, eps, momentum, run_mean, run_var, num_batches, save_mean, save_invstd,
                       ca, cb);
  if (y == nullptr) return;
  switch (dtype) {
    case 0: fwd_apply_dispatch<F32>(relu, res != nullptr, x, res, y, ca, cb, M, (int)C, g.apply_blocks, s, mask); break;
    case 1: fwd_apply_dispatch<BF16>(relu, res != nullptr, x, res, y, ca, cb, M, (int)C, g.apply_blocks, s, mask); break;
    default: fwd_apply_dispatch<F16>(relu, res != nullptr, x, res, y, ca, cb, M, (int)C, g.apply_blocks, s, mask); break;
  }
}

void launch_bn_apply(int dtype, const void* x, const void* res, void* y, int64_t M, int64_t C,
                     const float* coef_a, const float* coef_b, bool relu, hipStream_t s) {
  BnGeometry g = bn_geometry(M, C);
  switch (dtype) {
    case 0: fwd_apply_dispatch<F32>(relu, res != nullptr, x, res, y, coef_a, coef_b, M, (int)C, g.apply_blocks, s); break;
    case 1: fwd_apply_dispatch<BF16>(relu, res != nullptr, x, res, y, coef_a, coef_b, M, (int)C, g.apply_blocks, s); break;
    default: fwd_apply_dispatch<F16>(relu, res != nullptr, x, res, y, coef_a, coef_b, M, (int)C, g.apply_blocks, s); break;
  }
}

template <typename IO, int UNR>
static void bwd_stats_dispatch(bool relu, const void* dy, const void* dy2, const void* y, const void* x,
                               const float* mean, const float* coef, int64_t M, int C, const BnGeometry& g,
                               float* p1, float* p2, void* dz, hipStream_t s) {
  dim3 bl(kBlock), gs(g.chunks);
  const int64_t rpc = g.rows_per_chunk;
#define DPT_BN_STATS(R, T, W, MXV) \
  hipLaunchKernelGGL((bn_bwd_stats_kernel<IO, R, T, W, UNR, MXV>), gs, bl, 0, s, dy, dy2, y, x, mean, coef, M, C, \
                     rpc, g.chunks, p1, p2, dz)
  if (dz != nullptr) {
    if (relu && dy2) DPT_BN_STATS(true, true, true, false);
    else if (relu) DPT_BN_STATS(true, false, true, false);
    else if (dy2) DPT_BN_STATS(false, true, true, false);
    else DPT_BN_STATS(false, false, true, false);
  } else {
    if (relu && coef) DPT_BN_STATS(true, false, false, true);
    else if (relu) DPT_BN_STATS(true, false, false, false);
    else DPT_BN_STATS(false, false, false, false);
  }
#undef DPT_BN_STATS
}

template <typename IO>
static void bwd_dispatch(bool relu, const void* dy, const void* dy2, const void* y, const void* x,
                         const float* mean, const float* coef, int64_t M, int C, const BnGeometry& g, float* p1,
                         float* p2, const float* gamma, const float* invstd, float* dgamma, float* dbeta,
                         float* k1, float* k2, float* k3, void* dx, void* dz, hipStream_t s) {
  dim3 bl(kBlock);
  bwd_stats_dispatch<IO, kBnBwdUnroll>(relu, dy, dy2, y, x, mean, coef, M, C, g, p1, p2, dz, s);
  launch_bn_bwd_fin(make_bn_bwd_fin(p1, p2, g.chunks, C, M, gamma, invstd, dgamma, dbeta, k1, k2, k3, 0), s);
  dim3 ga(g.apply_blocks * 2 > kBnBwdApplyMax ? kBnBwdApplyMax : g.apply_blocks * 2);
  if (dz != nullptr) hipLaunchKernelGGL((bn_bwd_apply_kernel<IO, false, true, false>), ga, bl, 0, s, dz, y, x, mean, coef, k1, k2, k3, dx, M, C, kBnReverse, ReduceCarry{});
  else if (relu && coef) hipLaunchKernelGGL((bn_bwd_apply_kernel<IO, true, false, true>), ga, bl, 0, s, dy, y, x, mean, coef, k1, k2, k3, dx, M, C, kBnReverse, ReduceCarry{});
  else if (relu) hipLaunchKernelGGL((bn_bwd_apply_kernel<IO, true, false, false>), ga, bl, 0, s, dy, y, x, mean, coef, k1, k2, k3, dx, M, C, kBnReverse, ReduceCarry{});
  else hipLaunchKernelGGL((bn_bwd_apply_kernel<IO, false, false, false>), ga, bl, 0, s, dy, y, x, mean, coef, k1, k2, k3, dx, M, C, kBnReverse, ReduceCarry{});
}

void launch_bn_bwd(int dtype, const void* dy, const void* dy2, const void* y, const void* x, int64_t M,
                   int64_t C, const float* gamma, const float* mean, const float* invstd, const float* coef,
                   float* dgamma, float* dbeta, void* dx, void* dz, float* workspace, bool relu, hipStream_t s) {
  BnGeometry g = bn_geometry(M, C);
  float* p1 = workspace;
  float* p2 = p1 + (int64_t)C * g.chunks;
  float* k1 = p2 + (int64_t)C * g.chunks;
  float* k2 = k1 + C;
  float* k3 = k2 + C;
  switch (dtype) {
    case 0: bwd_dispatch<F32>(relu, dy, dy2, y, x, mean, dz ? nullptr : coef, M, (int)C, g, p1, p2, gamma, invstd, dgamma, dbeta, k1, k2, k3, dx, dz, s); break;
    case 1: bwd_dispatch<BF16>(relu, dy, dy2, y, x, mean, dz ? nullptr : coef, M, (int)C, g, p1, p2, gamma, invstd, dgamma, dbeta, k1, k2, k3, dx, dz, s); break;
    default: bwd_dispatch<F16>(relu, dy, dy2, y, x, mean, dz ? nullptr : coef, M, (int)C, g, p1, p2, gamma, invstd, dgamma, dbeta, k1, k2, k3, dx, dz, s); break;
  }
}


void launch_bn_bwd_apply_pre(int dtype, const void* dy, const void* x, int64_t M, int64_t C, const float* mean,
                             const float* coef, const float* kbuf, void* dx, hipStream_t s, bool from_dz) {
  BnGeometry g = bn_geometry(M, C);
  const float* k1 = kbuf;
  const float* k2 = k1 + C;
  const float* k3 = k2 + C;
  dim3 bl(kBlock);
  ReduceCarry rc;
  const int ga = (g.apply_blocks * 2 > kBnBwdApplyMax ? kBnBwdApplyMax : g.apply_blocks * 2) +
                 take_attached_reduce(rc);
  if (from_dz) {
    switch (dtype) {
      case 0: hipLaunchKernelGGL((bn_bwd_apply_kernel<F32, false, true, false>), dim3(ga), bl, 0, s, dy, nullptr, x, mean, coef, k1, k2, k3, dx, M, (int)C, kBnReverse, rc); break;
      case 1: hipLaunchKernelGGL((bn_bwd_apply_kernel<BF16, false, true, false>), dim3(ga), bl, 0, s, dy, nullptr, x, mean, coef, k1, k2, k3, dx, M, (int)C, kBnReverse, rc); break;
      default: hipLaunchKernelGGL((bn_bwd_apply_kernel<F16, false, true, false>), dim3(ga), bl, 0, s, dy, nullptr, x, mean, coef, k1, k2, k3, dx, M, (int)C, kBnReverse, rc); break;
    }
    return;
  }
  switch (dtype) {
    case 0: hipLaunchKernelGGL((bn_bwd_apply_kernel<F32, true, false, true>), dim3(ga), bl, 0, s, dy, nullptr, x, mean, coef, k1, k2, k3, dx, M, (int)C, kBnReverse, rc); break;
    case 1: hipLaunchKernelGGL((bn_bwd_apply_kernel<BF16, true, false, true>), dim3(ga), bl, 0, s, dy, nullptr, x, mean, coef, k1, k2, k3, dx, M, (int)C, kBnReverse, rc); break;
    default: hipLaunchKernelGGL((bn_bwd_apply_kernel<F16, true, false, true>), dim3(ga), bl, 0, s, dy, nullptr, x, mean, coef, k1, k2, k3, dx, M, (int)C, kBnReverse, rc); break;
  }
}

void launch_bn_bwd_from_partials(int dtype, const void* dy, const void* x, int64_t M, int64_t C, const float* gamma,
                                 const float* mean, const float* invstd, const float* coef, const float* p1,
                                 const float* p2, int chunks, float* dgamma, float* dbeta, void* dx, float* kbuf,
                                 hipStream_t s, bool from_dz) {
  BnGeometry g = bn_geometry(M, C);
  float* k1 = kbuf;
  float* k2 = k1 + C;
  float* k3 = k2 + C;
  dim3 bl(kBlock);
  launch_bn_bwd_fin(make_bn_bwd_fin(p1, p2, chunks, (int)C, M, gamma, invstd, dgamma, dbeta, k1, k2, k3, -1), s);
  launch_bn_bwd_apply_pre(dtype, dy, x, M, C, mean, coef, kbuf, dx, s, from_dz);
}

void launch_bn_apply_aff(int dtype, const void* x, const void* x2, void* y, int64_t M, int64_t C, const float* a,
                         const float* b, const float* a2, const float* b2, hipStream_t s, uint8_t* mask) {
  BnGeometry g = bn_geometry(M, C);
  dim3 gr(g.apply_blocks), bl(kBlock);
  switch (dtype) {
    case 0: hipLaunchKernelGGL((bn_fwd_apply_kernel<F32, true, true, true>), gr, bl, 0, s, x, x2, y, a, b, M, (int)C, kBnReverse, a2, b2, mask); break;
    case 1: hipLaunchKernelGGL((bn_fwd_apply_kernel<BF16, true, true, true>), gr, bl, 0, s, x, x2, y, a, b, M, (int)C, kBnReverse, a2, b2, mask); break;
    default: hipLaunchKernelGGL((bn_fwd_apply_kernel<F16, true, true, true>), gr, bl, 0, s, x, x2, y, a, b, M, (int)C, kBnReverse, a2, b2, mask); break;
  }
}

void launch_bn2_bwd_from_partials(int dtype, const void* dz, const void* x, const void* x2, int64_t M, int64_t C,
                                  const float* gamma, const float* mean, const float* invstd, const float* gamma2,
                                  const float* mean2, const float* invstd2, const float* p1, const float* p2,
                                  const float* p3, int chunks, float* dgamma, float* dbeta, float* dgamma2,
                                  float* dbeta2, void* dx, void* dx2, float* kbuf, hipStream_t s) {
  BnGeometry g = bn_geometry(M, C);
  float* k = kbuf;
  float* j = kbuf + 3 * C;
  dim3 bl(kBlock);
  const BnBwdFin f1 = make_bn_bwd_fin(p1, p2, chunks, (int)C, M, gamma, invstd, dgamma, dbeta, k, k + C, k + 2 * C, -1);
  const BnBwdFin f2 =
      make_bn_bwd_fin(p1, p3, chunks, (int)C, M, gamma2, invstd2, dgamma2, dbeta2, j, j + C, j + 2 * C, -1);
  if (!g_bn_skip_finalize)
    hipLaunchKernelGGL(bn_bwd_finalize2_kernel, dim3((unsigned)(f1.blocks + f2.blocks)), dim3(kBlock), 0, s, f1, f2);
  dim3 ga(g.apply_blocks * 2 > kBnBwdApplyMax ? kBnBwdApplyMax : g.apply_blocks * 2);
  switch (dtype) {
    case 0: hipLaunchKernelGGL(bn_bwd_apply2_kernel<F32>, ga, bl, 0, s, dz, x, x2, mean, mean2, k, j, dx, dx2, M, (int)C, kBnReverse); break;
    case 1: hipLaunchKernelGGL(bn_bwd_apply2_kernel<BF16>, ga, bl, 0, s, dz, x, x2, mean, mean2, k, j, dx, dx2, M, (int)C, kBnReverse); break;
    default: hipLaunchKernelGGL(bn_bwd_apply2_kernel<F16>, ga, bl, 0, s, dz, x, x2, mean, mean2, k, j, dx, dx2, M, (int)C, kBnReverse); break;
  }
}

int64_t bn_workspace_floats(int64_t M, int64_t C) {
  BnGeometry g = bn_geometry(M, C);
  return 2 * (int64_t)C * g.chunks + 3 * C;
}

}
```

csrc/kernels/conv_kernels.hip:

```cpp
#include <algorithm>
#include <cmath>
#include <cstdlib>
#include <mutex>
#include <stdexcept>
#include <type_traits>

#include "carry.h"
#include "gelu.h"
#include "common.h"
#include "kernels.h"
#include "mfma.h"

namespace dpt {


#ifndef DPT_WGRAD_WAVES
#define DPT_WGRAD_WAVES 4
#endif
#ifndef DPT_CONV_HALF_EPI
#define DPT_CONV_HALF_EPI 0
#endif

namespace conv {

constexpr int BM = 128;
constexpr int BK = 64;
constexpr int kThreads = 256;
constexpr int kRowBytes = BK * 2;

__device__ __forceinline__ int swz(int row, int chunk) { return chunk ^ ((row >> 1) & 7); }

__device__ __forceinline__ int opaque_v(int v) {
  asm volatile("" : "+v"(v));
  return v;
}

__device__ __forceinline__ int xcd_remap(int bid, int nwg) {
  const int q = nwg >> 3, r = nwg & 7, xcd = bid & 7, idx = bid >> 3;
  return (xcd < r ? xcd * (q + 1) : r * (q + 1) + (xcd - r) * q) + idx;
}

}

typedef _Float16 f16x8_t __attribute__((ext_vector_type(8)));
typedef _Float16 f16x2_t __attribute__((ext_vector_type(2)));

template <bool F16>
__device__ __forceinline__ f32x16_t cmfma(bf16x8_t a, bf16x8_t b, f32x16_t c) {
  if constexpr (F16)
    return __builtin_amdgcn_mfma_f32_32x32x16_f16(__builtin_bit_cast(f16x8_t, a), __builtin_bit_cast(f16x8_t, b), c,
                                                  0, 0, 0);
  else
    return __builtin_amdgcn_mfma_f32_32x32x16_bf16(a, b, c, 0, 0, 0);
}
template <bool F16>
__device__ __forceinline__ uint32_t cpack(f32x2_t v) {
  if constexpr (F16) return __builtin_bit_cast(uint32_t, __builtin_convertvector(v, f16x2_t));
  else return __builtin_bit_cast(uint32_t, __builtin_convertvector(v, bf16x2_t));
}
template <bool F16>
__device__ __forceinline__ float cunpack(uint32_t u, int h) {
  if constexpr (F16) return (float)__builtin_bit_cast(_Float16, (uint16_t)(h ? (u >> 16) : (u & 0xffffu)));
  else return __uint_as_float(h ? (u & 0xffff0000u) : (u << 16));
}

struct ConvSk {
  float* part = nullptr;
  unsigned* flags = nullptr;
  unsigned* err = nullptr;
  int G = 0;
  uint32_t part_bytes = 0;
};

struct ConvFwdArgs {
  const uint16_t* x = nullptr;
  const uint16_t* w = nullptr;
  uint16_t* y = nullptr;
  float* psum = nullptr;
  float* psq = nullptr;
  int N = 0, H = 0, W = 0, C = 0, Ho = 0, Wo = 0, Cout = 0, R = 0, S = 0, stride = 0, pad = 0;
  int64_t M = 0;
  int m_tiles = 0, n_tiles = 0;
  int mt256 = 0;
  const uint16_t* bnx = nullptr;
  const float* bn_mean = nullptr;
  const float* bn_coef = nullptr;
  float* bp1 = nullptr;
  float* bp2 = nullptr;
  const uint16_t* bny = nullptr;
  const uint16_t* bnres = nullptr;
  const uint8_t* bnmask = nullptr;
  int rHo = 0, rWo = 0;
  const uint16_t* bias16 = nullptr;
  const uint16_t* bnx2 = nullptr;
  const float* bn_mean2 = nullptr;
  float* bp3 = nullptr;
  int Rw = 0, Sw = 0, tr0 = 0, trs = 0, ts0 = 0, tss = 0;
  int oH = 0, oW = 0, oph = 0, opw = 0;
  int bp_ld = 0, bp_off = 0;
  int f16 = 0;
  float* part = nullptr;
  int splits = 1, kps = 0;
  ReduceCarry red;
  ConvSk sk;
};


template <int N>
__device__ __forceinline__ void vmcnt_wait() {
  asm volatile("s_waitcnt vmcnt(%0)" ::"n"(N) : "memory");
}

template <int RB>
__device__ __forceinline__ bf16x8_t wg_frag(const unsigned char* img, int krow0, int col0, int lane) {
  return tr_frag<RB, false>(img, krow0, col0, lane);
}

__device__ __attribute__((aligned(64))) uint4 g_conv_zero16[4];

template <int BMT, int BN, int STAGES, bool LDSEPI, bool BKN, bool STATS = true, bool BNB = false,
          bool BNR = false, bool REMAP = false, bool ZSIB = false, bool BNR2 = false, bool F16 = false,
          int NT = conv::kThreads, bool SPLIT = false, bool HALO = false, int HB = 1, bool SK = false,
          bool DGELU = false, bool BREG = false, bool RS2 = false>
__global__ __launch_bounds__(NT, (SK || BREG) ? 4 : 2) void conv_fwd_kernel(ConvFwdArgs p) {
  static_assert(!RS2 || (BNR && !BNR2 && !REMAP && LDSEPI && !HALO && !BREG), "RS2 config");
  using namespace conv;
  constexpr int BM = BMT;
  constexpr int NW = NT / 64;
  constexpr int WCOL = BREG ? 32 : 64;
  constexpr int WN = BN / WCOL;
  constexpr int WM = NW / WN;
  constexpr int MI = BM / (WM * 32);
  constexpr int NI = WCOL / 32;
  static_assert(WM * WN == NW && MI >= 1 && MI * WM * 32 == BM, "conv_fwd_kernel: bad wave tiling");
  constexpr int A_PER_T = BM * 8 / NT;
  constexpr int B_PER_T = BN * 8 / NT;
  static_assert(!HALO || (BMT == 128 && STAGES == 1 && !BKN && !SPLIT && NT == conv::kThreads), "HALO config");
  static_assert(!SK || (STAGES == 1 && !HALO && !SPLIT && LDSEPI && !BNR2 && NT == conv::kThreads), "SK config");
  static_assert(!DGELU || (BNB && !BNR && !STATS && !REMAP && LDSEPI && !SK), "DGELU config");
  static_assert(!BREG || (BMT == 128 && STAGES == 1 && LDSEPI && !BKN && !SPLIT && !SK && HB == 1 &&
                          NT == conv::kThreads && (BN == 128 || BN == 64)), "BREG config");
  constexpr int HROWS = 136;
  static_assert(HB == 1 || (HALO && HB == 3), "HB");
  constexpr int A_BYTES = (HALO ? HROWS : BM) * kRowBytes, B_BYTES = BN * kRowBytes;
  constexpr int STAGE = A_BYTES + (BREG ? 0 : HB * B_BYTES);
  constexpr int NSTAGE = BREG ? 2 : STAGES;
  constexpr int C_STRIDE = BN * 2 + 16;
  constexpr int RED = 2 * WM * BN * 4;
  constexpr int ZROW = NSTAGE * STAGE;
  constexpr int LDS_MAIN = NSTAGE * STAGE + (HALO ? kRowBytes : 0);
  constexpr bool HALF = DPT_CONV_HALF_EPI && LDSEPI && BM == 128 && NT == conv::kThreads && MI * 32 <= 64 && !BNB &&
                        !SPLIT;
  constexpr int EROWS = HALF ? 64 : BM;
  constexpr int LDS_EPI = (LDSEPI ? EROWS * C_STRIDE : 0) + RED;
  constexpr int LDS = LDS_MAIN > LDS_EPI ? LDS_MAIN : LDS_EPI;
  __shared__ __attribute__((aligned(16))) unsigned char lds[LDS];
  if constexpr (NT == conv::kThreads) {
    if (p.red.blocks) {
      const int nconv = (int)gridDim.x - p.red.blocks;
      if ((int)blockIdx.x >= nconv) {
        carry_reduce(p.red, (int)blockIdx.x - nconv, lds);
        return;
      }
    }
  }

  const int tid = threadIdx.x, lane = tid & 63, wid = tid >> 6;
  const int wm = wid / WN, wn = wid % WN;
  const int tiles = (BM == 256 ? p.mt256 : p.m_tiles) * p.n_tiles;
  const int nk_all = (int)((int64_t)p.R * p.S * p.C / BK);

  auto tile_body = [&](const int mt, const int nt, const int sp, const int ks0, const int ks1, const int sk_role,
                       const int sk_slot, const int sk_c0, const int sk_c1) {
  const int tid = SK ? conv::opaque_v((int)threadIdx.x) : (int)threadIdx.x, lane = tid & 63;
  const int wid = SK ? __builtin_amdgcn_readfirstlane(tid >> 6) : tid >> 6;
  const int wm = wid / WN, wn = wid % WN;
  const int64_t m0 = (int64_t)mt * BM;
  const int n0 = nt * BN;

  int hi0[A_PER_T], wi0[A_PER_T], aoff[A_PER_T];
  const int64_t HoWo = (int64_t)p.Ho * p.Wo;
#pragma unroll
  for (int i = 0; i < A_PER_T; ++i) {
    const int arow = (wid * A_PER_T + i) * 8 + (lane >> 3);
    const int achunk = (lane & 7) ^ ((arow >> 1) & 7);
    const int64_t m = m0 + arow;
    if (m < p.M) {
      const int64_t n = m / HoWo;
      const int rem = (int)(m - n * HoWo);
      const int ho = rem / p.Wo, wo = rem - ho * p.Wo;
      hi0[i] = ho * p.stride - p.pad;
      wi0[i] = wo * p.stride - p.pad + (p.C < BK ? achunk * 8 / p.C : 0);
      aoff[i] = (int)(((n * p.H + hi0[i]) * (int64_t)p.W + wo * p.stride - p.pad) * p.C + achunk * 8);
    } else {
      hi0[i] = -(1 << 28);
      wi0[i] = 0;
      aoff[i] = 0;
    }
  }
  const int64_t Kg = (int64_t)p.R * p.S * p.C;
  int woff[B_PER_T];
  constexpr int RBK = BN * 2;
  constexpr int KN_RPI = 1024 / RBK;
#pragma unroll
  for (int i = 0; i < B_PER_T; ++i) {
    if (BKN) {
      const int krow = (wid * B_PER_T + i) * KN_RPI + lane / (RBK / 16);
      const int kchunk = wg_slot<RBK>(krow, lane % (RBK / 16));
      woff[i] = krow * p.Rw * p.Sw * p.Cout + n0 + kchunk * 8;
    } else {
      const int brow = (wid * B_PER_T + i) * 8 + (lane >> 3);
      const int bchunk = (lane & 7) ^ ((brow >> 1) & 7);
      woff[i] = (int)((n0 + brow) * Kg) + bchunk * 8;
    }
  }
  constexpr uint32_t kOOB = 0xFFFFFF00u;
  const __amdgpu_buffer_rsrc_t rx = __builtin_amdgcn_make_buffer_rsrc(
// ... 2375 lines not shown
```

csrc/kernels/kernels.h:

```cpp
#pragma once

#include <hip/hip_runtime.h>
#include <stdint.h>

namespace dpt {

struct AugNorm {
  float mean[4];
  float inv_std[4];
};

void launch_grad_check(const float* g, int64_t n, const float* scale, float host_factor,
                       float* found_inf, hipStream_t s);
void launch_sgd(float* p, float* g, float* buf, int64_t n, float lr, float momentum,
                float dampening, float wd, bool nesterov, const float* scale, float host_factor,
                const float* found_inf, const float* step, bool zero_grad, uint16_t* shadow,
                int shadow_kind, hipStream_t s);
void launch_adam(float* p, float* g, float* m, float* v, int64_t n, double lr, double beta1,
                 double beta2, double eps, double wd, bool adamw, const float* scale, float host_factor,
                 const float* found_inf, const float* step, bool zero_grad, uint16_t* shadow,
                 int shadow_kind, hipStream_t s);
void launch_optim_tail(float* scale, int* growth_tracker, float* found_inf, float* step,
                       float growth_factor, float backoff_factor, int growth_interval,
                       hipStream_t s);

void launch_pack_bf16(const float* src, uint16_t* dst, int64_t n, hipStream_t s);
void launch_unpack_bf16(const uint16_t* src, float* dst, int64_t n, const float* scale,
                        float host_factor, float* found_inf, hipStream_t s);
void launch_spin(double ms, hipStream_t s);

void launch_metrics(const void* logits, int dtype, int64_t rows, int64_t cols, int64_t ld,
                    const int64_t* targets, const float* loss, double* acc, hipStream_t s);

void launch_augment(const uint8_t* data, const int64_t* idx, const int32_t* offs,
                    const uint8_t* flips, void* out, bool out_bf16, bool nhwc, int64_t B, int C,
                    int H, int W, int pad, AugNorm norm, hipStream_t s);

struct BnGeometry {
  int64_t rows_per_chunk;
  int chunks;
  int apply_blocks;
};
bool bn_supported(int64_t C);
BnGeometry bn_geometry(int64_t M, int64_t C);
int64_t bn_workspace_floats(int64_t M, int64_t C);
void launch_bn_fwd_train(int dtype, const void* x, const void* res, void* y, int64_t M, int64_t C,
                         const float* gamma, const float* beta, float eps, float momentum, float* run_mean,
                         float* run_var, int64_t* num_batches, float* save_mean, float* save_invstd,
                         float* save_coef, float* workspace, bool relu, hipStream_t s, uint8_t* mask = nullptr);
void launch_bn_fwd_from_partials(int dtype, const void* x, const void* res, void* y, int64_t M, int64_t C,
                                 const float* psum, const float* psq, int chunks, const float* gamma,
                                 const float* beta, float eps, float momentum, float* run_mean, float* run_var,
                                 int64_t* num_batches, float* save_mean, float* save_invstd, float* save_coef,
                                 bool relu, hipStream_t s, uint8_t* mask = nullptr);
void launch_bn_bwd_from_partials(int dtype, const void* dy, const void* x, int64_t M, int64_t C, const float* gamma,
                                 const float* mean, const float* invstd, const float* coef, const float* p1,
                                 const float* p2, int chunks, float* dgamma, float* dbeta, void* dx, float* kbuf,
                                 hipStream_t s, bool from_dz = false);
void launch_bn_apply_aff(int dtype, const void* x, const void* x2, void* y, int64_t M, int64_t C, const float* a,
                         const float* b, const float* a2, const float* b2, hipStream_t s, uint8_t* mask = nullptr);
void launch_bn2_bwd_from_partials(int dtype, const void* dz, const void* x, const void* x2, int64_t M, int64_t C,
                                  const float* gamma, const float* mean, const float* invstd, const float* gamma2,
                                  const float* mean2, const float* invstd2, const float* p1, const float* p2,
                                  const float* p3, int chunks, float* dgamma, float* dbeta, float* dgamma2,
                                  float* dbeta2, void* dx, void* dx2, float* kbuf, hipStream_t s);
void bn_set_skip_finalize(int on);
void launch_bn_apply(int dtype, const void* x, const void* res, void* y, int64_t M, int64_t C,
                     const float* coef_a, const float* coef_b, bool relu, hipStream_t s);
void launch_bn_bwd(int dtype, const void* dy, const void* dy2, const void* y, const void* x, int64_t M,
                   int64_t C, const float* gamma, const float* mean, const float* invstd, const float* coef,
                   float* dgamma, float* dbeta, void* dx, void* dz, float* workspace, bool relu, hipStream_t s);

void launch_maxpool_fwd(int dtype, const void* x, void* y, uint8_t* idx, int64_t B, int H, int W, int C, int Ho,
                        int Wo, int K, int S, int P, hipStream_t s, const float* coef = nullptr);
void launch_gap_bwd(int dtype, int gdtype, const void* g, void* dx, int64_t N, int64_t HW, int64_t C, hipStream_t s);
int gap_bwd_bnr_chunks(int64_t M, int64_t C);
void launch_gap_bwd_bnr(int dtype, int gdtype, const void* g, void* dz, const void* y, const void* x,
                        const float* mean, int64_t N, int64_t HW, int64_t C, float* p1, float* p2, hipStream_t s);
void launch_maxpool_bwd(int dtype, const void* dy, const void* dy2, const uint8_t* idx, void* dx, int64_t B, int H,
                        int W, int C, int Ho, int Wo, int K, int S, int P, hipStream_t s, const void* bnx = nullptr,
                        const float* bn_mean = nullptr, const float* bn_coef = nullptr, float* bp1 = nullptr,
                        float* bp2 = nullptr);
int maxpool_bwd_bn_chunks(int64_t B, int H, int W, int C);

constexpr int kGatherMax = 48;
struct GatherBatch {
  const void* src[kGatherMax];
  float* dst[kGatherMax];
  int64_t numel[kGatherMax];
  int8_t kind[kGatherMax];
  int count;
};
void launch_gather(const GatherBatch& batch, bool accumulate, hipStream_t s);

bool ln_supported(int64_t D);
int ln_bwd_blocks(int64_t T);
int gelu_bwd_chunks(int64_t T, int64_t F);
void vit_set_gelu_blocks_per_cu(int n);
void launch_ln_fwd(int kind, const float* x, const uint16_t* a, const void* bias, int bias_kind, const float* gamma,
                   const float* beta, float* s_out, uint16_t* h_out, float* mean, float* rstd, int64_t T, int64_t D,
                   float eps, hipStream_t s);
void launch_ln_bwd(int kind, const float* gs, const uint16_t* gh, const float* sv, const float* mean,
                   const float* rstd, const float* gamma, float* gx, uint16_t* ga, float* part, float* dgamma,
                   float* dbeta, void* dbias, int dbias_kind, int64_t T, int64_t D, hipStream_t s);
void launch_gelu_fwd(int kind, const uint16_t* u, const void* bias, int bias_kind, uint16_t* h, int64_t T, int64_t F,
                     hipStream_t s);
void launch_gelu_bwd(int kind, const uint16_t* gh, const uint16_t* u, const void* bias, int bias_kind, uint16_t* gu,
                     float* part, void* dbias, int dbias_kind, int64_t T, int64_t F, hipStream_t s);
void launch_bias_grad16(int kind, const uint16_t* gy, float* part, void* dbias, int dbias_kind, int64_t T, int64_t F,
                        hipStream_t s);
void launch_sum_partials(const float* part, int64_t n, int S, void* out, int out_kind, hipStream_t s);
void launch_colsum_rows(const float* part, int64_t n, int64_t D, void* out, int out_kind, hipStream_t s);
void launch_rows_copy16(const uint16_t* src, uint16_t* dst, const int n[4], const int64_t ss[4], const int64_t ds[4],
                        int L, hipStream_t s);

bool conv_supported(int C, int Cout);
bool conv_supported_narrow(int C, int Cout, int S);
int conv_m_tiles(int64_t M);
void conv_set_variant(int v);
void conv_set_big(int on);
void conv_set_wgrad_stages(int mode);
void conv_set_breg(int mode);
int conv_get_breg();
void conv_set_halo(int on);
void launch_linear_dgrad_dgelu(const uint16_t* dy, const uint16_t* wt, const uint16_t* u, const float* bias,
                               const uint16_t* bias16, uint16_t* gu, float* bp1, int64_t T, int n_out, int n_in,
                               bool f16, hipStream_t s);
int linear_dgrad_dgelu_tiles(int64_t T);
void conv_set_streamk(int mode, double eff);
int conv_get_streamk();
void conv_sk_prepare();
unsigned conv_sk_errors();
int conv_sk_blocks(int64_t tiles, int nk, int bn, int mode);
void conv_set_wgrad_target(int blocks);
int conv_fwd_splits(int64_t M, int Cout, int64_t K, int* kps = nullptr, hipStream_t s = nullptr);
int conv_fwd_splits_for(int64_t M, int Cout, int64_t K, bool graph, int* kps = nullptr);
int conv_split_cols(int64_t M);
void conv_set_splitk_policy(int tiles, int eager_tiles, int eager_min_k, int target);
void conv_set_splitk(int mode);
int conv_get_splitk();
void conv_set_fwd_shape_policy(int bits);
void launch_conv_fwd(const uint16_t* x, const uint16_t* w, uint16_t* y, int N, int H, int W, int C, int Cout,
                     int R, int S, int stride, int pad, float* psum, float* psq, hipStream_t s, int Ho = 0,
                     int Wo = 0, bool f16 = false, float* ws = nullptr);
struct ConvWgradPlan {
  int Ho, Wo, bmw, bnw, splits, steps_per_split;
  int64_t part_floats;
  int halo = 0;
};
void conv_set_wgrad_halo(int mode);
ConvWgradPlan conv_wgrad_plan(int N, int H, int W, int C, int Cout, int R, int S, int stride, int pad, int Ho = 0,
                              int Wo = 0, int target_blocks = 0);
struct WgradReduce {
  const float* part;
  void* out;
  int64_t n4;
  int splits, kind;
  bool consumed;
};
void launch_wgrad_reduce(const WgradReduce& r, hipStream_t s);
void launch_conv_wgrad(const uint16_t* dy, const uint16_t* x, float* part, void* dw, int dw_kind, int N, int H,
                       int W, int C, int Cout, int R, int S, int stride, int pad, const ConvWgradPlan& plan,
                       hipStream_t s, bool f16 = false, WgradReduce* defer = nullptr);
void launch_bn_bwd_apply_pre(int dtype, const void* dy, const void* x, int64_t M, int64_t C, const float* mean,
                             const float* coef, const float* kbuf, void* dx, hipStream_t s, bool from_dz);
struct ReduceCarry;
int take_attached_reduce(ReduceCarry& rc);
class AttachWgradReduce {
 public:
  AttachWgradReduce(WgradReduce* r, hipStream_t s);
  ~AttachWgradReduce();
  AttachWgradReduce(const AttachWgradReduce&) = delete;
  AttachWgradReduce& operator=(const AttachWgradReduce&) = delete;

 private:
  WgradReduce* r_;
  hipStream_t s_;
};
void launch_conv_dgrad_bnstats(const uint16_t* dy, const uint16_t* wt, uint16_t* dx, int N, int Ho, int Wo, int Cout,
                               int C, int R, int S, int pad, const uint16_t* bnx, const float* bn_mean,
                               const float* bn_coef, float* bp1, float* bp2, hipStream_t s,
                               const uint16_t* bny = nullptr, const uint16_t* bnres = nullptr,
                               const uint16_t* bnx2 = nullptr, const float* bn_mean2 = nullptr,
                               float* bp3 = nullptr, bool f16 = false, float* ws = nullptr,
                               const uint8_t* bnmask = nullptr, bool res_s2 = false);
constexpr int kWtFlipMax = 64;
struct WtFlipBatch {
  const uint16_t* w[kWtFlipMax];
  uint16_t* wt[kWtFlipMax];
  int Cout[kWtFlipMax], R[kWtFlipMax], S[kWtFlipMax], C[kWtFlipMax];
  int blk0[kWtFlipMax];
  int count;
};
void launch_conv_wt_flip_multi(WtFlipBatch b, hipStream_t s);
struct ConvS2Plan {
  int chunks;
  int64_t ws_floats;
};
ConvS2Plan conv_dgrad_s2_plan(int N, int H, int W, int C, int Cout, int R, int S, int pad, hipStream_t s);
void launch_conv_dgrad_s2(const uint16_t* dy, const uint16_t* w, uint16_t* dx, int N, int Ho, int Wo, int Cout,
                          int C, int R, int S, int pad, int H, int W, hipStream_t s, const uint16_t* bnx = nullptr,
                          const float* bn_mean = nullptr, const float* bn_coef = nullptr, float* bp1 = nullptr,
                          float* bp2 = nullptr, bool f16 = false, float* ws = nullptr, bool compact = false);
int conv_dgrad_s2_chunks(int N, int H, int W, int R, int S, int pad);
void launch_conv_dgrad(const uint16_t* dy, const uint16_t* w, uint16_t* dx, int N, int Ho, int Wo, int Cout, int C,
                       int R, int S, int pad, hipStream_t s, bool f16 = false);
void launch_space_to_depth2(const void* x, bool x_bf16, uint16_t* a, int N, int H, int W, int C, hipStream_t s,
                            bool out_f16 = false);
void launch_im2col(const void* x, bool x_bf16, uint16_t* a, int N, int H, int W, int C, int R, int S, int stride,
                   int pad, int Kp, hipStream_t s);
void launch_conv_wt_flip(const uint16_t* w, uint16_t* wt, int Cout, int R, int S, int C, hipStream_t s);

bool attn_supported(int S, int Dh);
int attn_lse_stride(int S);
void attn_set_bwd_split(int on);
void launch_attn_fwd(const uint16_t* qkv, uint16_t* ctx, float* lse2, int B, int S, int H, float scale,
                     hipStream_t s);
void launch_attn_bwd(const uint16_t* qkv, const uint16_t* out, const uint16_t* dout, const float* lse2,
                     uint16_t* dqkv, int B, int S, int H, float scale, hipStream_t s);

bool attn_stream_supported(int S, int Dh);
// ... 15 lines not shown
```

csrc/kernels/mfma.h:

```cpp
#pragma once

#include <hip/hip_runtime.h>
#include <stdint.h>

namespace dpt {

typedef __bf16 bf16x8_t __attribute__((ext_vector_type(8)));
typedef float f32x16_t __attribute__((ext_vector_type(16)));
typedef __bf16 bf16x2_t __attribute__((ext_vector_type(2)));
typedef float f32x2_t __attribute__((ext_vector_type(2)));
typedef short i16x4_t __attribute__((ext_vector_type(4)));
typedef short i16x8_t __attribute__((ext_vector_type(8)));

__device__ __forceinline__ f32x16_t mfma32(bf16x8_t a, bf16x8_t b, f32x16_t c) {
  return __builtin_amdgcn_mfma_f32_32x32x16_bf16(a, b, c, 0, 0, 0);
}

template <int RB>
__device__ __forceinline__ int wg_slot(int row, int ch) {
  if (RB == 256 || RB == 512) return ch ^ (((row & 3) << 2) | ((row >> 2) & 3));
  return ch ^ ((((row >> 1) & 1) << 2) | ((row >> 2) & 3));
}

template <int RB>
__device__ __forceinline__ bf16x8_t row_frag(const unsigned char* img, int row, int ch) {
  return *reinterpret_cast<const bf16x8_t*>(img + row * RB + wg_slot<RB>(row, ch) * 16);
}

template <int RB, bool PERM = false>
__device__ __forceinline__ bf16x8_t tr_frag(const unsigned char* img, int krow0, int col0, int lane) {
  const int g = lane >> 4, q = (lane & 15) >> 2, pp = lane & 3;
  const int colb = col0 + 16 * (g & 1) + 4 * pp;
  const int ch = colb >> 3, sub = (colb & 7) * 2;
  const int r1 = PERM ? krow0 + 4 * (g >> 1) + q : krow0 + 8 * (g >> 1) + q;
  const int r2 = PERM ? r1 + 8 : r1 + 4;
  typedef __attribute__((address_space(3))) i16x4_t lds_v4;
  const i16x4_t lo = __builtin_amdgcn_ds_read_tr16_b64_v4i16(
      (lds_v4*)(img + r1 * RB + wg_slot<RB>(r1, ch) * 16 + sub));
  const i16x4_t hi = __builtin_amdgcn_ds_read_tr16_b64_v4i16(
      (lds_v4*)(img + r2 * RB + wg_slot<RB>(r2, ch) * 16 + sub));
  i16x8_t v = {lo[0], lo[1], lo[2], lo[3], hi[0], hi[1], hi[2], hi[3]};
  return __builtin_bit_cast(bf16x8_t, v);
}

__device__ __forceinline__ bf16x8_t acc_frag(const f32x16_t& x, int s) {
  bf16x8_t f;
#pragma unroll
  for (int j = 0; j < 8; j += 2) {
    const f32x2_t v = {x[8 * s + j], x[8 * s + j + 1]};
    const bf16x2_t h = __builtin_convertvector(v, bf16x2_t);
    f[j] = h[0];
    f[j + 1] = h[1];
  }
  return f;
}

}
```

distributed_pytorch_training_amd/models/layers.py:

```python
from __future__ import annotations

import os
from typing import Optional

import torch
import torch.nn as nn
import torch.nn.functional as F

from ..ops import bn as fused_bn
from ..ops.conv_f32 import NativeConv2d
from ..ops import pool as fused_pool


class FusedBatchNorm2d(nn.BatchNorm2d):

    def can_fuse(self, x: torch.Tensor) -> bool:
        if not (self.affine and self.track_running_stats and self.momentum is not None):
            return False
        if not self.training and torch.is_grad_enabled() and x.requires_grad:
            return False
        return fused_bn.bn_act_supported(x, self.num_features)

    def act(self, x: torch.Tensor, relu: bool, residual: Optional[torch.Tensor], pair: bool = False):
        if self.training:
            return fused_bn.bn_act_train(x, residual, self.weight, self.bias, self.running_mean,
                                         self.running_var, self.num_batches_tracked, self.momentum,
                                         self.eps, relu, pair)
        y = fused_bn.bn_act_eval(x, residual, self.weight, self.bias, self.running_mean,
                                 self.running_var, self.eps, relu)
        return (y, y) if pair else y

    def forward(self, x: torch.Tensor) -> torch.Tensor:
        if self.can_fuse(x):
            return self.act(x, False, None)
        return super().forward(x)


def bn_act(bn: nn.Module, x: torch.Tensor, relu: bool = True,
           residual: Optional[torch.Tensor] = None) -> torch.Tensor:
    if isinstance(bn, FusedBatchNorm2d) and bn.can_fuse(x):
        return bn.act(x, relu, residual)
    out = bn(x)
    if residual is not None:
        out += residual
    return F.relu(out, inplace=True) if relu else out


class DeferredBN:

    __slots__ = ("bn", "x")

    def __init__(self, bn: nn.Module, x: torch.Tensor) -> None:
        self.bn, self.x = bn, x

    def materialize(self) -> torch.Tensor:
        return self.bn(self.x)


DS_FUSE = os.environ.get("DPT_DS_FUSE", "1") != "0"


def downsample_branch(ds: nn.Module, x: torch.Tensor, tail_bn: nn.Module):
    if (DS_FUSE and isinstance(ds, nn.Sequential) and len(ds) == 2 and isinstance(ds[1], FusedBatchNorm2d)
            and isinstance(tail_bn, FusedBatchNorm2d) and ds[1].training and tail_bn.training
            and torch.is_grad_enabled()):
        h = ds[0](x)
        return DeferredBN(ds[1], h) if ds[1].can_fuse(h) else ds[1](h)
    return ds(x)


def bn_act_block_out(bn: nn.Module, x: torch.Tensor, residual):
    if isinstance(residual, DeferredBN):
        if (isinstance(bn, FusedBatchNorm2d) and bn.can_fuse(x) and bn.training
                and residual.x.shape == x.shape and residual.x.dtype == x.dtype):
            return fused_bn.bn2_add_relu_train(x, bn, residual.x, residual.bn)
        residual = residual.materialize()
    if isinstance(bn, FusedBatchNorm2d) and bn.can_fuse(x):
        return bn.act(x, True, residual, pair=True)
    return bn_act(bn, x, True, residual)


STEM_FUSE = os.environ.get("DPT_STEM_FUSE", "1") != "0"


def bn_relu_maxpool(bn: nn.Module, pool: nn.Module, x: torch.Tensor):
    if (STEM_FUSE and isinstance(bn, FusedBatchNorm2d) and isinstance(pool, FusedMaxPool2d) and pool.dpt_pair
            and bn.training and torch.is_grad_enabled() and bn.can_fuse(x)
            and fused_pool.bn_relu_maxpool_supported(x, bn, pool)):
        return fused_pool.bn_relu_maxpool_train(x, bn)
    return pool(bn_act(bn, x))


def split_block_input(x):
    return x if isinstance(x, tuple) else (x, x)


class FusedMaxPool2d(nn.MaxPool2d):

    dpt_pair = False

    def forward(self, x: torch.Tensor):
        if not self.return_indices and fused_pool.maxpool_supported(
                x, self.kernel_size, self.stride, self.padding, self.dilation, self.ceil_mode):
            as_int = lambda v: v if isinstance(v, int) else v[0]
            pair = self.dpt_pair and self.training and torch.is_grad_enabled()
            return fused_pool.max_pool2d_nhwc(x, as_int(self.kernel_size), as_int(self.stride),
                                              as_int(self.padding), pair)
        return super().forward(x)


class FusedAdaptiveAvgPool2d(nn.AdaptiveAvgPool2d):

    def forward(self, x: torch.Tensor) -> torch.Tensor:
        if fused_pool.gap_supported(x) and torch.is_grad_enabled() and x.requires_grad:
            return fused_pool.global_avg_pool_nhwc(x)
        return super().forward(x)


class GemmConv1x1(nn.Conv2d):

    def gemm_ok(self, x: torch.Tensor) -> bool:
        return (x.is_cuda and x.dim() == 4 and self.groups == 1 and self.bias is None
                and self.kernel_size == (1, 1) and self.stride == (1, 1) and self.padding == (0, 0)
                and self.dilation == (1, 1) and x.is_contiguous(memory_format=torch.channels_last))

    def forward(self, x: torch.Tensor) -> torch.Tensor:
        if not self.gemm_ok(x):
            return super().forward(x)
        n, c, h, w = x.shape
        y = F.linear(x.permute(0, 2, 3, 1), self.weight.view(self.out_channels, c))
        return y.permute(0, 3, 1, 2)


def set_conv_routing(model: nn.Module, native_conv: bool = True, min_pixels=None, native_f32=None,
                     f32_mode=None) -> None:
    if f32_mode is not None:
        from ..ops.conv_f32 import MODES
        if f32_mode not in MODES:
            raise ValueError(f"f32_mode must be one of {MODES} or None, got {f32_mode!r}")
    for m in model.modules():
        if type(m) is nn.Conv2d:
            m.__class__ = NativeConv2d
        if isinstance(m, nn.Conv2d):
            m.dpt_native_conv = bool(native_conv)
            m.dpt_min_pixels = min_pixels
            m.dpt_native_conv_f32 = None if native_f32 is None else bool(native_f32)
            m.dpt_conv_f32_mode = f32_mode


def fuse_native_layers(model: nn.Module, gemm_1x1: bool = False, native_conv: bool = True,
                       min_pixels=None, native_f32=None, f32_mode=None) -> int:
    set_conv_routing(model, native_conv, min_pixels, native_f32, f32_mode)
    n = fuse_batchnorm(model)
    for parent in model.modules():
        for name, child in list(parent.named_children()):
            new_cls = None
            if type(child) is nn.MaxPool2d:
                new_cls = FusedMaxPool2d
            elif type(child) is nn.AdaptiveAvgPool2d and child.output_size in (1, (1, 1)):
                new_cls = FusedAdaptiveAvgPool2d
            elif gemm_1x1 and type(child) is nn.Conv2d and child.kernel_size == (1, 1) \
                    and child.stride == (1, 1) and child.groups == 1 and child.bias is None:
                new_cls = GemmConv1x1
            if new_cls is not None:
                new = new_cls.__new__(new_cls)
                new.__dict__ = child.__dict__
                if new_cls is FusedMaxPool2d and name == "maxpool" and hasattr(parent, "layer1"):
                    new.dpt_pair = True
                setattr(parent, name, new)
                n += 1
    tag_conv_bn_pairs(model)
    return n


def tag_conv_bn_pairs(model: nn.Module) -> int:
    n = 0
    for parent in model.modules():
        kids = dict(parent.named_children())
        pairs = []
        if isinstance(parent, nn.Sequential):
            seq = list(parent)
            pairs = [(a, b) for a, b in zip(seq, seq[1:])]
        else:
            for name, child in kids.items():
                if name.startswith("conv") and ("bn" + name[4:]) in kids:
                    pairs.append((child, kids["bn" + name[4:]]))
        for conv, bn in pairs:
            if isinstance(conv, nn.Conv2d) and isinstance(bn, FusedBatchNorm2d) and conv.bias is None:
                conv.dpt_bn_stats = True
                n += 1
    return n


def fuse_batchnorm(model: nn.Module) -> int:
    n = 0
    for parent in model.modules():
        for name, child in list(parent.named_children()):
            if type(child) is nn.BatchNorm2d:
                new = FusedBatchNorm2d.__new__(FusedBatchNorm2d)
                new.__dict__ = child.__dict__
                setattr(parent, name, new)
                n += 1
    return n
```

distributed_pytorch_training_amd/models/resnet.py:

```python
from __future__ import annotations

from typing import List, Optional, Type, Union

import torch
import torch.nn as nn

from .layers import bn_act, bn_act_block_out, bn_relu_maxpool, downsample_branch, split_block_input


def _conv3x3(cin: int, cout: int, stride: int = 1) -> nn.Conv2d:
    return nn.Conv2d(cin, cout, kernel_size=3, stride=stride, padding=1, bias=False)


def _conv1x1(cin: int, cout: int, stride: int = 1) -> nn.Conv2d:
    return nn.Conv2d(cin, cout, kernel_size=1, stride=stride, bias=False)


class BasicBlock(nn.Module):
    expansion = 1

    def __init__(self, cin: int, width: int, stride: int = 1,
                 downsample: Optional[nn.Module] = None) -> None:
        super().__init__()
        self.conv1 = _conv3x3(cin, width, stride)
        self.bn1 = nn.BatchNorm2d(width)
        self.relu = nn.ReLU(inplace=True)
        self.conv2 = _conv3x3(width, width)
        self.bn2 = nn.BatchNorm2d(width)
        self.downsample = downsample
        self.stride = stride

    def forward(self, x):
        xc, xi = split_block_input(x)
        out = bn_act(self.bn1, self.conv1(xc))
        identity = xi if self.downsample is None else downsample_branch(self.downsample, xi, self.bn2)
        return bn_act_block_out(self.bn2, self.conv2(out), identity)


class Bottleneck(nn.Module):

    expansion = 4

    def __init__(self, cin: int, width: int, stride: int = 1,
                 downsample: Optional[nn.Module] = None) -> None:
        super().__init__()
        self.conv1 = _conv1x1(cin, width)
        self.bn1 = nn.BatchNorm2d(width)
        self.conv2 = _conv3x3(width, width, stride)
        self.bn2 = nn.BatchNorm2d(width)
        self.conv3 = _conv1x1(width, width * self.expansion)
        self.bn3 = nn.BatchNorm2d(width * self.expansion)
        self.relu = nn.ReLU(inplace=True)
        self.downsample = downsample
        self.stride = stride

    def forward(self, x):
        xc, xi = split_block_input(x)
        out = bn_act(self.bn1, self.conv1(xc))
        identity = xi if self.downsample is None else downsample_branch(self.downsample, xi, self.bn3)
        out = bn_act(self.bn2, self.conv2(out))
        return bn_act_block_out(self.bn3, self.conv3(out), identity)


class ResNet(nn.Module):
    def __init__(self, block: Type[Union[BasicBlock, Bottleneck]], layers: List[int],
                 num_classes: int = 1000, zero_init_residual: bool = False) -> None:
        super().__init__()
        self.inplanes = 64
        self.conv1 = nn.Conv2d(3, 64, kernel_size=7, stride=2, padding=3, bias=False)
        self.bn1 = nn.BatchNorm2d(64)
        self.relu = nn.ReLU(inplace=True)
        self.maxpool = nn.MaxPool2d(kernel_size=3, stride=2, padding=1)
        self.layer1 = self._make_layer(block, 64, layers[0])
        self.layer2 = self._make_layer(block, 128, layers[1], stride=2)
        self.layer3 = self._make_layer(block, 256, layers[2], stride=2)
        self.layer4 = self._make_layer(block, 512, layers[3], stride=2)
        self.avgpool = nn.AdaptiveAvgPool2d((1, 1))
        self.fc = nn.Linear(512 * block.expansion, num_classes)

        for m in self.modules():
            if isinstance(m, nn.Conv2d):
                nn.init.kaiming_normal_(m.weight, mode="fan_out", nonlinearity="relu")
            elif isinstance(m, (nn.BatchNorm2d, nn.GroupNorm)):
                nn.init.constant_(m.weight, 1)
                nn.init.constant_(m.bias, 0)
        if zero_init_residual:
            for m in self.modules():
                if isinstance(m, Bottleneck):
                    nn.init.constant_(m.bn3.weight, 0)
                elif isinstance(m, BasicBlock):
                    nn.init.constant_(m.bn2.weight, 0)

    def _make_layer(self, block, width: int, blocks: int, stride: int = 1) -> nn.Sequential:
        downsample = None
        if stride != 1 or self.inplanes != width * block.expansion:
            downsample = nn.Sequential(
                _conv1x1(self.inplanes, width * block.expansion, stride),
                nn.BatchNorm2d(width * block.expansion),
            )
        layers = [block(self.inplanes, width, stride, downsample)]
        self.inplanes = width * block.expansion
        for _ in range(1, blocks):
            layers.append(block(self.inplanes, width))
        return nn.Sequential(*layers)

    def forward(self, x: torch.Tensor) -> torch.Tensor:
        x = bn_relu_maxpool(self.bn1, self.maxpool, self.conv1(x))
        x = self.layer4(self.layer3(self.layer2(self.layer1(x))))
        if isinstance(x, tuple):
            x = x[0]
        x = torch.flatten(self.avgpool(x), 1)
        return self.fc(x)


def resnet18(num_classes: int = 1000, **kw) -> ResNet:
    return ResNet(BasicBlock, [2, 2, 2, 2], num_classes=num_classes, **kw)


def resnet34(num_classes: int = 1000, **kw) -> ResNet:
    return ResNet(BasicBlock, [3, 4, 6, 3], num_classes=num_classes, **kw)


def resnet50(num_classes: int = 1000, **kw) -> ResNet:
    return ResNet(Bottleneck, [3, 4, 6, 3], num_classes=num_classes, **kw)


def resnet101(num_classes: int = 1000, **kw) -> ResNet:
    return ResNet(Bottleneck, [3, 4, 23, 3], num_classes=num_classes, **kw)
```

distributed_pytorch_training_amd/ops/bn.py:

```python
from __future__ import annotations

from typing import Optional

import torch

import os

from . import native, native_available
from .conv import COMPACT_RES, MASKED_NO_RES, take_bnb_partials

BNR_FUSE = os.environ.get("DPT_BNR_FUSE", "1") != "0"


def _cl(t: torch.Tensor) -> torch.Tensor:
    if t.dim() == 4 and not t.is_contiguous(memory_format=torch.channels_last):
        return t.contiguous(memory_format=torch.channels_last)
    return t


def _relu_mask(x: torch.Tensor) -> torch.Tensor:
    c = x.shape[1]
    return torch.empty((x.numel() // c, c // 8), dtype=torch.uint8, device=x.device)


class _BNActTrain(torch.autograd.Function):
    @staticmethod
    def forward(ctx, x, residual, weight, bias, running_mean, running_var, num_batches, momentum, eps, relu,
                partials, links):
        y = _fwd(ctx, x, residual, weight, bias, running_mean, running_var, num_batches, momentum, eps, relu,
                 partials=partials, links=links)
        return y

    @staticmethod
    def backward(ctx, dy):
        return _bwd(ctx, dy, None) + (None,) * 8


class _BNActTrainPair(torch.autograd.Function):

    @staticmethod
    def forward(ctx, x, residual, weight, bias, running_mean, running_var, num_batches, momentum, eps, relu,
                partials, links):
        y = _fwd(ctx, x, residual, weight, bias, running_mean, running_var, num_batches, momentum, eps, relu,
                 pair=True, partials=partials, links=links)
        ctx.set_materialize_grads(False)
        return y, y.view_as(y)

    @staticmethod
    def backward(ctx, dy, dy2):
        return _bwd(ctx, dy, dy2) + (None,) * 8


def _fwd(ctx, x, residual, weight, bias, running_mean, running_var, num_batches, momentum, eps, relu,
         pair=False, partials=None, links=(None, None)):
    ps, pq = partials if partials is not None else (None, None)
    own_slot, res_slot = links
    mask = _relu_mask(x) if (own_slot is not None and relu and residual is not None) else None
    y, mean, invstd, coef = native().bn_fwd_train(x, residual, weight, bias, running_mean, running_var,
                                                  num_batches, float(momentum), float(eps), bool(relu), ps, pq,
                                                  mask_out=mask)
    ctx.relu = bool(relu)
    ctx.has_res = residual is not None
    mask_from_x = ctx.relu and not ctx.has_res and not pair
    ctx.save_for_backward(x, y if (relu and not mask_from_x) else None, weight, mean, invstd,
                          coef if mask_from_x else None)
    if mask_from_x:
        y._dpt_bn_src = (x, mean, coef)
    ctx.res_slot = res_slot
    if own_slot is not None:
        if mask is not None:
            own_slot["mask"] = mask
        y._dpt_bn_src = (x, mean, own_slot)
    return y


def _bwd(ctx, dy, dy2):
    x, y, weight, mean, invstd, coef = ctx.saved_tensors
    if dy is None:
        dy, dy2 = dy2, None
    if dy is None:
        return (None, None, None, None)
    want_params = weight is not None and (ctx.needs_input_grad[2] or ctx.needs_input_grad[3])
    want_dz = ctx.has_res and ctx.needs_input_grad[1]
    if coef is not None and dy2 is None:
        part = take_bnb_partials(dy)
        if part is not None:
            dx, dg, db = native().bn_bwd_partials(dy, x, weight, mean, invstd, coef, part[0], part[1],
                                                  bool(want_params))
            return (dx, None, dg if want_params else None, db if want_params else None)
    if dy2 is not None and ctx.relu and ctx.has_res:
        part = take_bnb_partials(dy)
        if part is not None and part[3] is not None:
            raise RuntimeError("fused block-tail backward: unexpected downsample statistic")
        if part is not None:
            if part[2] != dy2.data_ptr():
                raise RuntimeError("fused block-tail backward: the identity-path gradient folded into the "
                                   "conv's dgrad is not the one autograd delivered (alias used twice?)")
            dx, dg, db = native().bn_bwd_partials(dy, x, weight, mean, invstd, None, part[0], part[1],
                                                  bool(want_params), True)
            if ctx.res_slot is not None:
                ctx.res_slot["dres"] = dy
            return (dx, dy if want_dz else None, dg if want_params else None, db if want_params else None)
    if dy2 is None and ctx.relu and ctx.has_res:
        part = take_bnb_partials(dy)
        if part is not None and part[2] in (MASKED_NO_RES, COMPACT_RES):
            dx, dg, db = native().bn_bwd_partials(dy, x, weight, mean, invstd, None, part[0], part[1],
                                                  bool(want_params), True)
            if ctx.res_slot is not None:
                ctx.res_slot["dres"] = dy
            return (dx, dy if want_dz else None, dg if want_params else None, db if want_params else None)
    dx, dg, db, dz = native().bn_bwd(_cl(dy), None if dy2 is None else _cl(dy2), y, x, weight, mean, invstd,
                                     ctx.relu, bool(want_dz), bool(want_params), coef)
    if want_dz and ctx.res_slot is not None:
        ctx.res_slot["dres"] = dz
    return (dx, dz if want_dz else None, dg if want_params else None, db if want_params else None)


class _BN2AddReLUPair(torch.autograd.Function):

    @staticmethod
    def forward(ctx, x, x2, w, b, rm, rv, nb, w2, b2, rm2, rv2, nb2, momentum, eps, momentum2, eps2,
                partials, partials2, own_slot):
        C = native()
        ps, pq = partials if partials is not None else (None, None)
        ps2, pq2 = partials2 if partials2 is not None else (None, None)
        _, mean, invstd, coef = C.bn_fwd_train(x, None, w, b, rm, rv, nb, float(momentum), float(eps), True,
                                               ps, pq, False)
        _, mean2, invstd2, coef2 = C.bn_fwd_train(x2, None, w2, b2, rm2, rv2, nb2, float(momentum2), float(eps2),
                                                  False, ps2, pq2, False)
        mask = _relu_mask(x) if own_slot is not None else None
        y = C.bn_apply_aff(x, x2, coef, coef2, mask_out=mask)
        ctx.save_for_backward(x, x2, y, w, w2, mean, invstd, mean2, invstd2)
        ctx.set_materialize_grads(False)
        if own_slot is not None:
            own_slot["mask"] = mask
            y._dpt_bn_src = (x, mean, own_slot, x2, mean2)
        return y, y.view_as(y)

    @staticmethod
    def backward(ctx, dy, dy2):
        x, x2, y, w, w2, mean, invstd, mean2, invstd2 = ctx.saved_tensors
        if dy is None:
            dy, dy2 = dy2, None
        if dy is None:
            return (None,) * 19
        want = [ctx.needs_input_grad[i] for i in (2, 3, 7, 8)]
        want_params = any(want)
        C = native()
        part = take_bnb_partials(dy) if dy2 is not None else None
        if part is not None and part[3] is not None:
            if part[2] != dy2.data_ptr():
                raise RuntimeError("fused block-tail backward: the identity-path gradient folded into the "
                                   "conv's dgrad is not the one autograd delivered (alias used twice?)")
            dx, dx2, dg, db, dg2, db2 = C.bn2_bwd_partials(dy, x, x2, w, w2, mean, invstd, mean2, invstd2,
                                                           part[0], part[1], part[3], bool(want_params))
        else:
            if part is not None:
                raise RuntimeError("fused block-tail backward: partials without the downsample statistic")
            dx, dg, db, dz = C.bn_bwd(_cl(dy), None if dy2 is None else _cl(dy2), y, x, w, mean, invstd,
                                      True, True, bool(want_params), None)
            dx2, dg2, db2, _ = C.bn_bwd(dz, None, None, x2, w2, mean2, invstd2, False, False,
                                        bool(want_params), None)
        g = [dg, db, dg2, db2]
        g = [t if (want_params and want[i]) else None for i, t in enumerate(g)]
        return (dx, dx2, g[0], g[1], None, None, None, g[2], g[3]) + (None,) * 10


def bn2_add_relu_train(x, bn, x2, bn2):
    x2 = _cl(x2.to(x.dtype))
    partials = x.__dict__.pop("_dpt_bn_partials", None)
    partials2 = x2.__dict__.pop("_dpt_bn_partials", None)
    own_slot = {} if (BNR_FUSE and x.dtype in (torch.bfloat16, torch.float16)) else None
    out = _BN2AddReLUPair.apply(x, x2, bn.weight, bn.bias, bn.running_mean, bn.running_var, bn.num_batches_tracked,
                                bn2.weight, bn2.bias, bn2.running_mean, bn2.running_var, bn2.num_batches_tracked,
                                bn.momentum, bn.eps, bn2.momentum, bn2.eps, partials, partials2, own_slot)
    if own_slot is not None:
        out[1]._dpt_res_slot = own_slot
    return out


def bn_act_supported(x: torch.Tensor, num_features: int) -> bool:
    return (x.is_cuda and native_available() and x.dim() == 4
            and x.dtype in (torch.bfloat16, torch.float16, torch.float32)
            and x.is_contiguous(memory_format=torch.channels_last)
            and native().bn_supported(num_features))


def bn_act_train(x: torch.Tensor, residual: Optional[torch.Tensor], weight, bias, running_mean, running_var,
                 num_batches, momentum: float, eps: float, relu: bool, pair: bool = False):
    res_slot = None
    if residual is not None:
        if residual.dtype == x.dtype and residual.is_contiguous(memory_format=torch.channels_last):
            res_slot = residual.__dict__.get("_dpt_res_slot")
        residual = _cl(residual.to(x.dtype))
    partials = x.__dict__.pop("_dpt_bn_partials", None)
    own_slot = {} if (pair and relu and residual is not None and BNR_FUSE
                      and x.dtype in (torch.bfloat16, torch.float16)) else None
    fn = _BNActTrainPair if pair else _BNActTrain
    out = fn.apply(x, residual, weight, bias, running_mean, running_var, num_batches, momentum, eps, relu,
                   partials, (own_slot, res_slot))
    if own_slot is not None:
        out[1]._dpt_res_slot = own_slot
    return out


@torch.no_grad()
def bn_act_eval(x: torch.Tensor, residual: Optional[torch.Tensor], weight, bias, running_mean, running_var,
                eps: float, relu: bool) -> torch.Tensor:
    a = torch.rsqrt(running_var.float() + eps)
    if weight is not None:
        a = a * weight.float()
    b = -running_mean.float() * a
    if bias is not None:
        b = b + bias.float()
    if residual is not None:
        residual = _cl(residual.to(x.dtype))
    return native().bn_apply(x, residual, a.contiguous(), b.contiguous(), bool(relu))


def reference_bn_act(x, residual, weight, bias, running_mean, running_var, training, momentum, eps, relu):
    y = torch.nn.functional.batch_norm(x, running_mean, running_var, weight, bias, training, momentum, eps)
    if residual is not None:
        y = y + residual
    return torch.relu(y) if relu else y
```

distributed_pytorch_training_amd/ops/conv.py:

```python
from __future__ import annotations

import os

import torch

from . import native, native_available

_CL = torch.channels_last
_DT16 = (torch.bfloat16, torch.float16)
ENABLED = os.environ.get("DPT_NATIVE_CONV", "1") != "0"
BN_BWD_FUSE = os.environ.get("DPT_BN_BWD_FUSE", "1") != "0"
_BNB_PARTIALS = {}
_GEN = [0]
S2_DGRAD = os.environ.get("DPT_S2_DGRAD", "1") != "0"
S2_COMPACT_DRES = os.environ.get("DPT_S2_COMPACT_DRES", "1") != "0"
WGRAD_REDUCE_FUSE = os.environ.get("DPT_WGRAD_REDUCE_FUSE", "1") != "0"
STEM_ENABLED = os.environ.get("DPT_NATIVE_STEM", "0") == "1"


MIN_PIXELS = int(os.environ.get("DPT_CONV_MIN_PIXELS", "0"))


def supported(x: torch.Tensor, w: torch.Tensor, stride, padding, dilation, groups, min_pixels=None) -> bool:
    if not (ENABLED and x.is_cuda and native_available() and x.dtype in _DT16
# ... 38 lines not shown

def _note(kind, x, w, stride, pad, variant, e0, out_hw=(0, 0)):
    if _CALLS is None or e0 is None:
        return
    co, ci, r, _ = w.shape
    key = (ci, x.shape[2], x.shape[3], co, r, int(stride), int(pad), tuple(int(v) for v in out_hw))
    _CALLS.append((kind, key, variant, e0, _mark()))


def _backward(ctx, dy):
    x, w = ctx.saved_tensors
    dy = _cl(dy.to(x.dtype))
    s, p = ctx.stride, ctx.pad
    dx = dw = red = None
    e0 = _mark()
    if ctx.needs_input_grad[1]:
        if ctx.needs_input_grad[0] and WGRAD_REDUCE_FUSE:
            dw, red = native().conv_wgrad_deferred(dy, x, list(w.shape), s, p)
        else:
            dw = native().conv_wgrad(dy, x, list(w.shape), s, p, False)
        _note("wgrad", x, w, s, p, "deferred-reduce" if red is not None else "reduce", e0)
        e0 = _mark()
    variant = None
    if ctx.needs_input_grad[0]:
        src = ctx.bn_src if (s == 1 and BN_BWD_FUSE) else None
        dres = None
        wt = _flipped(w) if s == 1 else None
        slot = ctx.bn_src[2] if (ctx.bn_src is not None and isinstance(ctx.bn_src[2], dict)) else None
        compact = False
        if slot is not None:
            slot.pop("fold_s2", None)
            compact = bool(slot.pop("dres_s2", False))
            if compact and not (src is not None and len(src) == 3 and _is_compact_of(slot.get("dres"), x)):
                raise RuntimeError("fused block-tail backward: a downsample conv handed over a compact "
                                   "identity-path gradient that this conv's backward-data cannot fold")
        if src is not None and not isinstance(src[2], dict):
            bn_x, bn_mean, bn_coef = src
            dx, p1, p2, _ = native().conv_dgrad_bnstats(dy, w, p, bn_x, bn_mean, bn_coef, w_flipped=wt,
                                                        wgrad_reduce=red)
            _put_bnb(dx, p1, p2, None, None)
            variant = "bnrelu-stats"
        elif (src is not None and _dres_ok(dres := src[2].pop("dres", None), x)
              and (compact or dres.shape == x.shape)):
            bn_x, bn_mean = src[0], src[1]
            x2, mean2 = (src[3], src[4]) if len(src) > 3 else (None, None)
            dx, p1, p2, p3 = native().conv_dgrad_bnstats(dy, w, p, bn_x, bn_mean, None, x, dres, wt, x2, mean2,
                                                         wgrad_reduce=red, bn_mask=src[2].get("mask"),
                                                         bn_res_s2=compact)
            _put_bnb(dx, p1, p2, COMPACT_RES if compact else dres.data_ptr(), p3 if x2 is not None else None)
            variant = "tail-stats-s2res" if compact else "tail+ds-stats" if x2 is not None else "tail-stats"
        elif s == 1:
            dx = (native().conv_dgrad_flip(dy, w, p, wgrad_reduce=red)[0] if wt is None
                  else native().conv_dgrad_preflipped(dy, wt, p, wgrad_reduce=red))
            variant = "plain"
        elif s == 2 and S2_DGRAD and x.dim() == 4:
            src = ctx.bn_src if BN_BWD_FUSE else None
            rs = ctx.res_slot
            if (ctx.compact_dres and S2_COMPACT_DRES and BN_BWD_FUSE and rs is not None and rs.get("fold_s2")
                    and "dres" not in rs):
                rs["dres"] = native().conv_dgrad_s2(dy, w, p, x.shape[2], x.shape[3], wgrad_reduce=red,
                                                    compact=True)[0]
                rs["dres_s2"] = True
                variant = "s2-compact"
            elif src is not None and not isinstance(src[2], dict) and w.shape[2] > 1:
                dx, p1, p2 = native().conv_dgrad_s2(dy, w, p, x.shape[2], x.shape[3], src[0], src[1], src[2],
                                                    wgrad_reduce=red)
                _put_bnb(dx, p1, p2, None, None)
                variant = "s2-bnrelu-stats"
            else:
                dx = native().conv_dgrad_s2(dy, w, p, x.shape[2], x.shape[3], wgrad_reduce=red)[0]
                variant = "s2"
        else:
            dx = torch.ops.aten.convolution_backward(dy, x, w, None, (s, s), (p, p), (1, 1), False, (0, 0), 1,
                                                     (True, False, False))[0]
    if red is not None and not red.done:
        native().conv_reduce_flush(red)
    if variant is not None:
        _note("dgrad", x, w, s, p, variant + ("+reduce" if red is not None else ""), e0)
    if variant == "s2-compact":
        return None, dw
    if dx is not None and ctx.res_slot is not None:
        ctx.res_slot["dres"] = dx
    return dx, dw


_FLIP = {"on": False, "pending": {}, "done": {}}


def reset_side_channels() -> None:
    _GEN[0] += 1
    _BNB_PARTIALS.clear()


def _put_bnb(dx, p1, p2, dres_ptr, p3) -> None:
    _BNB_PARTIALS[dx.data_ptr()] = (_GEN[0], dx._version, p1, p2, tuple(dx.shape), dres_ptr, p3)


def begin_step() -> None:
    reset_side_channels()
    _FLIP["on"] = True
    _FLIP["pending"].clear()
    _FLIP["done"].clear()


def end_caching() -> None:
    _FLIP["on"] = False
    _FLIP["pending"].clear()
    _FLIP["done"].clear()


def _flipped(w: torch.Tensor):
    if not _FLIP["on"]:
        return None
    key = (w.data_ptr(), tuple(w.shape))
    wt = _FLIP["done"].get(key)
    if wt is None:
        pend = _FLIP["pending"]
        pend.setdefault(key, w)
        keys = list(pend.keys())
        for k, t in zip(keys, native().conv_wt_flip_multi([pend[k] for k in keys])):
            _FLIP["done"][k] = t
        pend.clear()
        wt = _FLIP["done"][key]
    return wt


def _is_compact_of(dres, x) -> bool:
    n, c, h, w = x.shape
    return (dres is not None and dres.dtype == x.dtype and dres.is_contiguous(memory_format=_CL)
            and tuple(dres.shape) == (n, c, (h + 1) // 2, (w + 1) // 2))


def _dres_ok(dres, x) -> bool:
    return (dres is not None and dres.dtype == x.dtype and (dres.shape == x.shape or _is_compact_of(dres, x))
            and dres.is_contiguous(memory_format=_CL))


class _Conv(torch.autograd.Function):
    @staticmethod
    def forward(ctx, x, w, stride: int, pad: int, out_hw, bn_src, res_slot, compact_dres):
        e0 = _mark()
        y = native().conv_fwd(x, w, stride, pad, False, *out_hw)[0]
        _note("fwd", x, w, stride, pad, "plain", e0, out_hw)
        ctx.save_for_backward(x, w)
        ctx.stride, ctx.pad, ctx.bn_src, ctx.res_slot = stride, pad, bn_src, res_slot
        ctx.compact_dres = compact_dres
        return y

    @staticmethod
    def backward(ctx, dy):
        return _backward(ctx, dy) + (None,) * 6


class _ConvStats(torch.autograd.Function):
    @staticmethod
    def forward(ctx, x, w, stride: int, pad: int, out_hw, bn_src, res_slot, compact_dres):
        e0 = _mark()
        y, ps, pq = native().conv_fwd(x, w, stride, pad, True, *out_hw)
        _note("fwd", x, w, stride, pad, "stats", e0, out_hw)
        ctx.save_for_backward(x, w)
        ctx.stride, ctx.pad, ctx.bn_src, ctx.res_slot = stride, pad, bn_src, res_slot
        ctx.compact_dres = compact_dres
        ctx.mark_non_differentiable(ps, pq)
        ctx.set_materialize_grads(False)
        return y, ps, pq

    @staticmethod
    def backward(ctx, dy, _dps, _dpq):
        return _backward(ctx, dy) + (None,) * 6


def conv2d(x: torch.Tensor, w: torch.Tensor, stride: int, pad: int, bn_stats: bool = False,
           out_hw=(0, 0)) -> torch.Tensor:
    w = _cl(w)
    if _FLIP["on"] and int(stride) == 1 and x.requires_grad:
        _FLIP["pending"].setdefault((w.data_ptr(), tuple(w.shape)), w)
    bn_src = x.__dict__.get("_dpt_bn_src")
    res_slot = x.__dict__.get("_dpt_res_slot")
    one_by_one = w.shape[2] == 1 and w.shape[3] == 1
    if (int(stride) == 1 and one_by_one and BN_BWD_FUSE and bn_src is not None and len(bn_src) == 3
            and isinstance(bn_src[2], dict)):
        bn_src[2]["fold_s2"] = True
    compact_dres = bool(S2_COMPACT_DRES and S2_DGRAD and int(stride) == 2 and one_by_one and int(pad) == 0
                        and tuple(out_hw) == (0, 0) and res_slot is not None and res_slot.get("fold_s2"))
    if not bn_stats:
        return _Conv.apply(x, w, int(stride), int(pad), tuple(out_hw), bn_src, res_slot, compact_dres)
    y, ps, pq = _ConvStats.apply(x, w, int(stride), int(pad), tuple(out_hw), bn_src, res_slot, compact_dres)
    y._dpt_bn_partials = (ps, pq)
    return y


MASKED_NO_RES = -1
COMPACT_RES = -2


def register_bnb_partials(dx: torch.Tensor, p1: torch.Tensor, p2: torch.Tensor, masked: bool = False) -> None:
    _put_bnb(dx, p1, p2, MASKED_NO_RES if masked else None, None)


def take_bnb_partials(dy: torch.Tensor):
    if not _BNB_PARTIALS:
        return None
    ent = _BNB_PARTIALS.pop(dy.data_ptr(), None)
    if ent is None:
        return None
    gen, ver, p1, p2, shape, dres_ptr, p3 = ent
    if gen != _GEN[0] or ver != dy._version or shape != tuple(dy.shape):
        return None
    return p1, p2, dres_ptr, p3


def take_bn_partials(x: torch.Tensor):
    part = x.__dict__.pop("_dpt_bn_partials", None)
    return part


def s2d_stem_supported(x: torch.Tensor, w: torch.Tensor, stride, padding, dilation, groups) -> bool:
    if not (ENABLED and x.is_cuda and native_available() and x.dim() == 4 and groups == 1
            and x.dtype in (torch.float32, torch.bfloat16) and w.dtype in _DT16):
        return False
    cout, cin, r, s = w.shape
    return (cin <= 4 and cout % 64 == 0 and (r, s) == (7, 7) and tuple(stride) == (2, 2)
            and tuple(padding) == (3, 3) and tuple(dilation) == (1, 1) and not x.requires_grad
            and x.shape[1] == cin and x.shape[2] % 2 == 0 and x.shape[3] % 2 == 0
            and x.is_contiguous(memory_format=_CL))


def s2d_stem_conv2d(x: torch.Tensor, w: torch.Tensor, bn_stats: bool = False) -> torch.Tensor:
    cout, cin = w.shape[0], w.shape[1]
    x2 = native().space_to_depth2(x, w.dtype == torch.float16)
    wk = torch.nn.functional.pad(w.permute(0, 2, 3, 1), (0, 4 - cin, 1, 0, 1, 0))
    w2 = wk.reshape(cout, 4, 2, 4, 2, 4).permute(0, 1, 3, 2, 4, 5).reshape(cout, 4, 4, 16)
    w2 = w2.permute(0, 3, 1, 2)
    return conv2d(x2, w2, 1, 2, bn_stats, out_hw=(x.shape[2] // 2, x.shape[3] // 2))


def stem_supported(x: torch.Tensor, w: torch.Tensor, stride, padding, dilation, groups) -> bool:
    if not (ENABLED and x.is_cuda and native_available() and x.dim() == 4 and groups == 1
            and x.dtype in (torch.float32, torch.bfloat16) and w.dtype == torch.bfloat16):
        return False
    cout, cin, r, s = w.shape
    return (cin < 64 and cout % 64 == 0 and not x.requires_grad and tuple(dilation) == (1, 1)
            and stride[0] == stride[1] and padding[0] == padding[1] and x.shape[1] == cin
            and x.is_contiguous(memory_format=_CL))


def stem_conv2d(x: torch.Tensor, w: torch.Tensor, stride: int, pad: int, bn_stats: bool = False) -> torch.Tensor:
    cout, cin, r, s = w.shape
    k = r * s * cin
    kp = (k + 63) // 64 * 64
    a = native().im2col(x, r, s, int(stride), int(pad), kp)
    wf = torch.nn.functional.pad(w.permute(0, 2, 3, 1).reshape(cout, k), (0, kp - k))
    return conv2d(a, wf.view(cout, kp, 1, 1), 1, 0, bn_stats)
```

Measured before the change: 12680.

## Fuse bottleneck tail BN-add-ReLU apply into the next 1x1 conv forward

```diff
diff --git a/csrc/bindings.cpp b/csrc/bindings.cpp
--- a/csrc/bindings.cpp
+++ b/csrc/bindings.cpp
@@ -783,14 +783,23 @@
   return {y, mean, invstd, coef};
 }
 
-Tensor bn_apply_aff(Tensor x, Tensor x2, Tensor coef, Tensor coef2, c10::optional<Tensor> mask_out) {
+static Tensor apply_out(const c10::optional<Tensor>& y_out, const Tensor& x, const char* who) {
+  if (!y_out.has_value() || !y_out->defined()) return at::empty_like(x);
+  TORCH_CHECK(y_out->device() == x.device() && y_out->scalar_type() == x.scalar_type() && y_out->sizes() == x.sizes() &&
+                  y_out->strides() == x.strides(),
+              who, ": y_out must match x in device, dtype, shape and layout");
+  return *y_out;
+}
+
+Tensor bn_apply_aff(Tensor x, Tensor x2, Tensor coef, Tensor coef2, c10::optional<Tensor> mask_out,
+                    c10::optional<Tensor> y_out) {
   auto [M, C] = bn_rows(x, "x");
   TORCH_CHECK(dpt::bn_supported(C), "fused BN: unsupported channel count ", C);
   TORCH_CHECK(x2.sizes() == x.sizes() && x2.scalar_type() == x.scalar_type(), "bn_apply_aff: x2 mismatch");
   bn_rows(x2, "x2");
   const float* a = f32_param(coef, 2 * C, "coef");
   const float* a2 = f32_param(coef2, 2 * C, "coef2");
-  auto y = at::empty_like(x);
+  auto y = apply_out(y_out, x, "bn_apply_aff");
   c10::hip::HIPGuard guard(x.device().index());
   uint8_t* mp = relu_mask_ptr(mask_out, M, C, x, "bn_apply_aff");
   dpt::launch_bn_apply_aff(bn_dtype(x), x.data_ptr(), x2.data_ptr(), y.data_ptr(), M, C, a, a + C, a2, a2 + C,
@@ -826,7 +835,8 @@
   return {dx, dx2, dg, db, dg2, db2};
 }
 
-Tensor bn_apply(Tensor x, c10::optional<Tensor> residual, Tensor a, Tensor b, bool relu) {
+Tensor bn_apply(Tensor x, c10::optional<Tensor> residual, Tensor a, Tensor b, bool relu,
+                c10::optional<Tensor> mask_out, c10::optional<Tensor> y_out) {
   auto [M, C] = bn_rows(x, "x");
   TORCH_CHECK(dpt::bn_supported(C), "fused BN: unsupported channel count ", C);
   const void* rp = nullptr;
@@ -835,11 +845,48 @@
     bn_rows(*residual, "residual");
     rp = residual->data_ptr();
   }
-  auto y = at::empty_like(x);
+  auto y = apply_out(y_out, x, "bn_apply");
+  uint8_t* mp = relu_mask_ptr(mask_out, M, C, x, "bn_apply");
+  TORCH_CHECK(mp == nullptr || (relu && rp != nullptr), "bn_apply: mask_out needs relu + residual");
   c10::hip::HIPGuard guard(x.device().index());
   dpt::launch_bn_apply(bn_dtype(x), x.data_ptr(), rp, y.data_ptr(), M, C, f32_param(a, C, "a"),
-                       f32_param(b, C, "b"), relu, cur_stream(x));
+                       f32_param(b, C, "b"), relu, cur_stream(x), mp);
   return y;
+}
+
+std::vector<Tensor> conv1x1_tail_fwd(Tensor x3, Tensor r, Tensor coef, c10::optional<Tensor> coef2, Tensor w,
+                                     Tensor y_out, Tensor mask_out, int64_t stride, int64_t pad) {
+  check_cl_bf16(x3, "x3");
+  check_cl_bf16(r, "residual");
+  check_cl_bf16(w, "w");
+  check_cl_bf16(y_out, "y_out");
+  same_16(x3, w, "conv1x1_tail_fwd");
+  TORCH_CHECK(r.sizes() == x3.sizes() && r.scalar_type() == x3.scalar_type(), "conv1x1_tail_fwd: residual mismatch");
+  TORCH_CHECK(y_out.sizes() == x3.sizes() && y_out.scalar_type() == x3.scalar_type(),
+              "conv1x1_tail_fwd: y_out mismatch");
+  const int N = x3.size(0), C = x3.size(1), H = x3.size(2), W = x3.size(3);
+  const int64_t M = (int64_t)N * H * W;
+  const int Cout = w.size(0);
+  TORCH_CHECK(w.size(1) == C, "conv1x1_tail_fwd: channel mismatch");
+  TORCH_CHECK(w.size(2) == 1 && w.size(3) == 1 && stride == 1 && pad == 0,
+              "conv1x1_tail_fwd: a 1x1 / stride-1 / unpadded conv only");
+  const char* why = dpt::tail_conv1_refusal(M, C, Cout);
+  TORCH_CHECK(why == nullptr, "conv1x1_tail_fwd: ", why ? why : "");
+  const float* a = f32_param(coef, 2 * C, "coef");
+  const float* a2 = f32_param(coef2, 2 * C, "coef2");
+  uint8_t* mp = relu_mask_ptr(mask_out, M, C, x3, "conv1x1_tail_fwd");
+  TORCH_CHECK(mp != nullptr, "conv1x1_tail_fwd: mask_out is required");
+  auto x1 = at::empty({N, Cout, H, W}, x3.options().memory_format(at::MemoryFormat::ChannelsLast));
+  const int64_t mt = dpt::conv_m_tiles(M);
+  auto ps = at::empty({Cout, mt}, x3.options().dtype(at::kFloat));
+  auto pq = at::empty({Cout, mt}, x3.options().dtype(at::kFloat));
+  c10::hip::HIPGuard guard(x3.device().index());
+  dpt::launch_tail_conv1_fwd(is_f16(x3), reinterpret_cast<const uint16_t*>(x3.data_ptr()),
+                             reinterpret_cast<const uint16_t*>(r.data_ptr()), a, a2,
+                             reinterpret_cast<const uint16_t*>(w.data_ptr()), reinterpret_cast<uint16_t*>(y_out.data_ptr()),
+                             mp, reinterpret_cast<uint16_t*>(x1.data_ptr()), ps.data_ptr<float>(), pq.data_ptr<float>(), M,
+                             C, Cout, cur_stream(x3));
+  return {x1, ps, pq};
 }
 
 std::vector<Tensor> bn_bwd(Tensor dy, c10::optional<Tensor> dy2, c10::optional<Tensor> y, Tensor x,
@@ -1220,9 +1267,17 @@
         py::arg("running_mean"), py::arg("running_var"), py::arg("num_batches"), py::arg("momentum"), py::arg("eps"),
         py::arg("relu"), py::arg("psum") = py::none(), py::arg("psq") = py::none(), py::arg("apply") = true,
         py::arg("mask_out") = py::none());
-  m.def("bn_apply", &bn_apply, py::arg("x"), py::arg("residual"), py::arg("a"), py::arg("b"), py::arg("relu"));
+  m.def("bn_apply", &bn_apply, py::arg("x"), py::arg("residual"), py::arg("a"), py::arg("b"), py::arg("relu"),
+        py::arg("mask_out") = py::none(), py::arg("y_out") = py::none());
   m.def("bn_apply_aff", &bn_apply_aff, py::arg("x"), py::arg("x2"), py::arg("coef"), py::arg("coef2"),
-        py::arg("mask_out") = py::none());
+        py::arg("mask_out") = py::none(), py::arg("y_out") = py::none());
+  m.def("conv1x1_tail_fwd", &conv1x1_tail_fwd, py::arg("x3"), py::arg("res_or_x2"), py::arg("coef"), py::arg("coef2"),
+        py::arg("w"), py::arg("y_out"), py::arg("mask_out"), py::arg("stride") = 1, py::arg("pad") = 0);
+  m.def("conv1x1_tail_refusal", [](int64_t M, int64_t Cin, int64_t Cout) -> py::object {
+          const char* why = dpt::tail_conv1_refusal(M, Cin, Cout);
+          return why ? py::object(py::str(why)) : py::object(py::none());
+        }, py::arg("M"), py::arg("Cin"), py::arg("Cout"),
+        "why conv1x1_tail_fwd refuses this shape (None: it takes it)");
   m.def("bn2_bwd_partials", &bn2_bwd_partials, py::arg("dz"), py::arg("x"), py::arg("x2"), py::arg("weight"),
         py::arg("weight2"), py::arg("mean"), py::arg("invstd"), py::arg("mean2"), py::arg("invstd2"), py::arg("p1"),
         py::arg("p2"), py::arg("p3"), py::arg("want_dparams"));
diff --git a/csrc/kernels/bn_io.h b/csrc/kernels/bn_io.h
--- /dev/null
+++ b/csrc/kernels/bn_io.h
@@ -0,0 +1,110 @@
+#pragma once
+
+#include "common.h"
+
+namespace dpt {
+
+struct BF16 {
+  using raw = uint16_t;
+  __device__ static void load8(const void* p, int64_t i, float f[8]) {
+    uint4 w = *reinterpret_cast<const uint4*>(static_cast<const uint16_t*>(p) + i);
+    uint32_t u[4] = {w.x, w.y, w.z, w.w};
+#pragma unroll
+    for (int k = 0; k < 4; ++k) {
+      f[2 * k] = bf16_to_f32(u[k] & 0xffff);
+      f[2 * k + 1] = bf16_to_f32(u[k] >> 16);
+    }
+  }
+  __device__ static void store8(void* p, int64_t i, const float f[8]) {
+    uint4 w;
+    w.x = (uint32_t)f32_to_bf16(f[0]) | ((uint32_t)f32_to_bf16(f[1]) << 16);
+    w.y = (uint32_t)f32_to_bf16(f[2]) | ((uint32_t)f32_to_bf16(f[3]) << 16);
+    w.z = (uint32_t)f32_to_bf16(f[4]) | ((uint32_t)f32_to_bf16(f[5]) << 16);
+    w.w = (uint32_t)f32_to_bf16(f[6]) | ((uint32_t)f32_to_bf16(f[7]) << 16);
+    *reinterpret_cast<uint4*>(static_cast<uint16_t*>(p) + i) = w;
+  }
+  __device__ static bool pos16(uint32_t h) { return !(h & 0x8000u) && (h & 0x7fffu) && (h & 0x7fffu) <= 0x7f80u; }
+  __device__ static uint32_t store8m(void* p, int64_t i, const float f[8]) {
+    uint32_t h[8];
+#pragma unroll
+    for (int k = 0; k < 8; ++k) h[k] = f32_to_bf16(f[k]);
+    *reinterpret_cast<uint4*>(static_cast<uint16_t*>(p) + i) =
+        make_uint4(h[0] | (h[1] << 16), h[2] | (h[3] << 16), h[4] | (h[5] << 16), h[6] | (h[7] << 16));
+    uint32_t m = 0;
+#pragma unroll
+    for (int k = 0; k < 8; ++k) m |= (pos16(h[k]) ? 1u : 0u) << k;
+    return m;
+  }
+  __device__ static void pos8(const void* p, int64_t i, bool m[8]) {
+    uint4 w = *reinterpret_cast<const uint4*>(static_cast<const uint16_t*>(p) + i);
+    uint32_t u[4] = {w.x, w.y, w.z, w.w};
+#pragma unroll
+    for (int k = 0; k < 4; ++k) {
+      uint16_t lo = u[k] & 0xffff, hi = u[k] >> 16;
+      m[2 * k] = !(lo & 0x8000) && (lo & 0x7fff) && (lo & 0x7fff) <= 0x7f80;
+      m[2 * k + 1] = !(hi & 0x8000) && (hi & 0x7fff) && (hi & 0x7fff) <= 0x7f80;
+    }
+  }
+};
+
+struct F16 {
+  __device__ static void load8(const void* p, int64_t i, float f[8]) {
+    uint4 w = *reinterpret_cast<const uint4*>(static_cast<const uint16_t*>(p) + i);
+    uint32_t u[4] = {w.x, w.y, w.z, w.w};
+#pragma unroll
+    for (int k = 0; k < 4; ++k) {
+      f[2 * k] = f16_to_f32(u[k] & 0xffff);
+      f[2 * k + 1] = f16_to_f32(u[k] >> 16);
+    }
+  }
+  __device__ static uint16_t to16(float v) { return __builtin_bit_cast(uint16_t, (_Float16)v); }
+  __device__ static void store8(void* p, int64_t i, const float f[8]) {
+    uint4 w;
+    w.x = (uint32_t)to16(f[0]) | ((uint32_t)to16(f[1]) << 16);
+    w.y = (uint32_t)to16(f[2]) | ((uint32_t)to16(f[3]) << 16);
+    w.z = (uint32_t)to16(f[4]) | ((uint32_t)to16(f[5]) << 16);
+    w.w = (uint32_t)to16(f[6]) | ((uint32_t)to16(f[7]) << 16);
+    *reinterpret_cast<uint4*>(static_cast<uint16_t*>(p) + i) = w;
+  }
+  __device__ static uint32_t store8m(void* p, int64_t i, const float f[8]) {
+    store8(p, i, f);
+    uint32_t m = 0;
+#pragma unroll
+    for (int k = 0; k < 8; ++k) m |= ((float)__builtin_bit_cast(_Float16, to16(f[k])) > 0.0f ? 1u : 0u) << k;
+    return m;
+  }
+  __device__ static void pos8(const void* p, int64_t i, bool m[8]) {
+    float f[8];
+    load8(p, i, f);
+#pragma unroll
+    for (int k = 0; k < 8; ++k) m[k] = f[k] > 0.0f;
+  }
+};
+
+struct F32 {
+  __device__ static void load8(const void* p, int64_t i, float f[8]) {
+    const float4* q = reinterpret_cast<const float4*>(static_cast<const float*>(p) + i);
+    float4 a = q[0], b = q[1];
+    f[0] = a.x; f[1] = a.y; f[2] = a.z; f[3] = a.w; f[4] = b.x; f[5] = b.y; f[6] = b.z; f[7] = b.w;
+  }
+  __device__ static void store8(void* p, int64_t i, const float f[8]) {
+    float4* q = reinterpret_cast<float4*>(static_cast<float*>(p) + i);
+    q[0] = make_float4(f[0], f[1], f[2], f[3]);
+    q[1] = make_float4(f[4], f[5], f[6], f[7]);
+  }
+  __device__ static uint32_t store8m(void* p, int64_t i, const float f[8]) {
+    store8(p, i, f);
+    uint32_t m = 0;
+#pragma unroll
+    for (int k = 0; k < 8; ++k) m |= (f[k] > 0.0f ? 1u : 0u) << k;
+    return m;
+  }
+  __device__ static void pos8(const void* p, int64_t i, bool m[8]) {
+    float f[8];
+    load8(p, i, f);
+#pragma unroll
+    for (int k = 0; k < 8; ++k) m[k] = f[k] > 0.0f;
+  }
+};
+
+}
diff --git a/csrc/kernels/bn_kernels.hip b/csrc/kernels/bn_kernels.hip
--- a/csrc/kernels/bn_kernels.hip
+++ b/csrc/kernels/bn_kernels.hip
@@ -1,113 +1,11 @@
 #include <cstdlib>
 
+#include "bn_io.h"
 #include "carry.h"
 #include "common.h"
 #include "kernels.h"
 
 namespace dpt {
-
-struct BF16 {
-  using raw = uint16_t;
-  __device__ static void load8(const void* p, int64_t i, float f[8]) {
-    uint4 w = *reinterpret_cast<const uint4*>(static_cast<const uint16_t*>(p) + i);
-    uint32_t u[4] = {w.x, w.y, w.z, w.w};
-#pragma unroll
-    for (int k = 0; k < 4; ++k) {
-      f[2 * k] = bf16_to_f32(u[k] & 0xffff);
-      f[2 * k + 1] = bf16_to_f32(u[k] >> 16);
-    }
-  }
-  __device__ static void store8(void* p, int64_t i, const float f[8]) {
-    uint4 w;
-    w.x = (uint32_t)f32_to_bf16(f[0]) | ((uint32_t)f32_to_bf16(f[1]) << 16);
-    w.y = (uint32_t)f32_to_bf16(f[2]) | ((uint32_t)f32_to_bf16(f[3]) << 16);
-    w.z = (uint32_t)f32_to_bf16(f[4]) | ((uint32_t)f32_to_bf16(f[5]) << 16);
-    w.w = (uint32_t)f32_to_bf16(f[6]) | ((uint32_t)f32_to_bf16(f[7]) << 16);
-    *reinterpret_cast<uint4*>(static_cast<uint16_t*>(p) + i) = w;
-  }
-  __device__ static bool pos16(uint32_t h) { return !(h & 0x8000u) && (h & 0x7fffu) && (h & 0x7fffu) <= 0x7f80u; }
-  __device__ static uint32_t store8m(void* p, int64_t i, const float f[8]) {
-    uint32_t h[8];
-#pragma unroll
-    for (int k = 0; k < 8; ++k) h[k] = f32_to_bf16(f[k]);
-    *reinterpret_cast<uint4*>(static_cast<uint16_t*>(p) + i) =
-        make_uint4(h[0] | (h[1] << 16), h[2] | (h[3] << 16), h[4] | (h[5] << 16), h[6] | (h[7] << 16));
-    uint32_t m = 0;
-#pragma unroll
-    for (int k = 0; k < 8; ++k) m |= (pos16(h[k]) ? 1u : 0u) << k;
-    return m;
-  }
-  __device__ static void pos8(const void* p, int64_t i, bool m[8]) {
-    uint4 w = *reinterpret_cast<const uint4*>(static_cast<const uint16_t*>(p) + i);
-    uint32_t u[4] = {w.x, w.y, w.z, w.w};
-#pragma unroll
-    for (int k = 0; k < 4; ++k) {
-      uint16_t lo = u[k] & 0xffff, hi = u[k] >> 16;
-      m[2 * k] = !(lo & 0x8000) && (lo & 0x7fff) && (lo & 0x7fff) <= 0x7f80;
-      m[2 * k + 1] = !(hi & 0x8000) && (hi & 0x7fff) && (hi & 0x7fff) <= 0x7f80;
-    }
-  }
-};
-
-struct F16 {
-  __device__ static void load8(const void* p, int64_t i, float f[8]) {
-    uint4 w = *reinterpret_cast<const uint4*>(static_cast<const uint16_t*>(p) + i);
-    uint32_t u[4] = {w.x, w.y, w.z, w.w};
-#pragma unroll
-    for (int k = 0; k < 4; ++k) {
-      f[2 * k] = f16_to_f32(u[k] & 0xffff);
-      f[2 * k + 1] = f16_to_f32(u[k] >> 16);
-    }
-  }
-  __device__ static uint16_t to16(float v) { return __builtin_bit_cast(uint16_t, (_Float16)v); }
-  __device__ static void store8(void* p, int64_t i, const float f[8]) {
-    uint4 w;
-    w.x = (uint32_t)to16(f[0]) | ((uint32_t)to16(f[1]) << 16);
-    w.y = (uint32_t)to16(f[2]) | ((uint32_t)to16(f[3]) << 16);
-    w.z = (uint32_t)to16(f[4]) | ((uint32_t)to16(f[5]) << 16);
-    w.w = (uint32_t)to16(f[6]) | ((uint32_t)to16(f[7]) << 16);
-    *reinterpret_cast<uint4*>(static_cast<uint16_t*>(p) + i) = w;
-  }
-  __device__ static uint32_t store8m(void* p, int64_t i, const float f[8]) {
-    store8(p, i, f);
-    uint32_t m = 0;
-#pragma unroll
-    for (int k = 0; k < 8; ++k) m |= ((float)__builtin_bit_cast(_Float16, to16(f[k])) > 0.0f ? 1u : 0u) << k;
-    return m;
-  }
-  __device__ static void pos8(const void* p, int64_t i, bool m[8]) {
-    float f[8];
-    load8(p, i, f);
-#pragma unroll
-    for (int k = 0; k < 8; ++k) m[k] = f[k] > 0.0f;
-  }
-};
-
-struct F32 {
-  __device__ static void load8(const void* p, int64_t i, float f[8]) {
-    const float4* q = reinterpret_cast<const float4*>(static_cast<const float*>(p) + i);
-    float4 a = q[0], b = q[1];
-    f[0] = a.x; f[1] = a.y; f[2] = a.z; f[3] = a.w; f[4] = b.x; f[5] = b.y; f[6] = b.z; f[7] = b.w;
-  }
-  __device__ static void store8(void* p, int64_t i, const float f[8]) {
-    float4* q = reinterpret_cast<float4*>(static_cast<float*>(p) + i);
-    q[0] = make_float4(f[0], f[1], f[2], f[3]);
-    q[1] = make_float4(f[4], f[5], f[6], f[7]);
-  }
-  __device__ static uint32_t store8m(void* p, int64_t i, const float f[8]) {
-    store8(p, i, f);
-    uint32_t m = 0;
-#pragma unroll
-    for (int k = 0; k < 8; ++k) m |= (f[k] > 0.0f ? 1u : 0u) << k;
-    return m;
-  }
-  __device__ static void pos8(const void* p, int64_t i, bool m[8]) {
-    float f[8];
-    load8(p, i, f);
-#pragma unroll
-    for (int k = 0; k < 8; ++k) m[k] = f[k] > 0.0f;
-  }
-};
 
 template <typename IO>
 __global__ __launch_bounds__(kBlock) void bn_fwd_stats_kernel(const void* __restrict__ x, int64_t M, int C,
@@ -587,12 +485,12 @@
 }
 
 void launch_bn_apply(int dtype, const void* x, const void* res, void* y, int64_t M, int64_t C,
-                     const float* coef_a, const float* coef_b, bool relu, hipStream_t s) {
-  BnGeometry g = bn_geometry(M, C);
-  switch (dtype) {
-    case 0: fwd_apply_dispatch<F32>(relu, res != nullptr, x, res, y, coef_a, coef_b, M, (int)C, g.apply_blocks, s); break;
-    case 1: fwd_apply_dispatch<BF16>(relu, res != nullptr, x, res, y, coef_a, coef_b, M, (int)C, g.apply_blocks, s); break;
-    default: fwd_apply_dispatch<F16>(relu, res != nullptr, x, res, y, coef_a, coef_b, M, (int)C, g.apply_blocks, s); break;
+                     const float* coef_a, const float* coef_b, bool relu, hipStream_t s, uint8_t* mask) {
+  BnGeometry g = bn_geometry(M, C);
+  switch (dtype) {
+    case 0: fwd_apply_dispatch<F32>(relu, res != nullptr, x, res, y, coef_a, coef_b, M, (int)C, g.apply_blocks, s, mask); break;
+    case 1: fwd_apply_dispatch<BF16>(relu, res != nullptr, x, res, y, coef_a, coef_b, M, (int)C, g.apply_blocks, s, mask); break;
+    default: fwd_apply_dispatch<F16>(relu, res != nullptr, x, res, y, coef_a, coef_b, M, (int)C, g.apply_blocks, s, mask); break;
   }
 }
 
diff --git a/csrc/kernels/conv_kernels.hip b/csrc/kernels/conv_kernels.hip
--- a/csrc/kernels/conv_kernels.hip
+++ b/csrc/kernels/conv_kernels.hip
@@ -42,27 +42,6 @@
 
 }
 
-typedef _Float16 f16x8_t __attribute__((ext_vector_type(8)));
-typedef _Float16 f16x2_t __attribute__((ext_vector_type(2)));
-
-template <bool F16>
-__device__ __forceinline__ f32x16_t cmfma(bf16x8_t a, bf16x8_t b, f32x16_t c) {
-  if constexpr (F16)
-    return __builtin_amdgcn_mfma_f32_32x32x16_f16(__builtin_bit_cast(f16x8_t, a), __builtin_bit_cast(f16x8_t, b), c,
-                                                  0, 0, 0);
-  else
-    return __builtin_amdgcn_mfma_f32_32x32x16_bf16(a, b, c, 0, 0, 0);
-}
-template <bool F16>
-__device__ __forceinline__ uint32_t cpack(f32x2_t v) {
-  if constexpr (F16) return __builtin_bit_cast(uint32_t, __builtin_convertvector(v, f16x2_t));
-  else return __builtin_bit_cast(uint32_t, __builtin_convertvector(v, bf16x2_t));
-}
-template <bool F16>
-__device__ __forceinline__ float cunpack(uint32_t u, int h) {
-  if constexpr (F16) return (float)__builtin_bit_cast(_Float16, (uint16_t)(h ? (u >> 16) : (u & 0xffffu)));
-  else return __uint_as_float(h ? (u & 0xffff0000u) : (u << 16));
-}
 
 struct ConvSk {
   float* part = nullptr;
diff --git a/csrc/kernels/kernels.h b/csrc/kernels/kernels.h
--- a/csrc/kernels/kernels.h
+++ b/csrc/kernels/kernels.h
@@ -66,7 +66,12 @@
                                   float* dbeta2, void* dx, void* dx2, float* kbuf, hipStream_t s);
 void bn_set_skip_finalize(int on);
 void launch_bn_apply(int dtype, const void* x, const void* res, void* y, int64_t M, int64_t C,
-                     const float* coef_a, const float* coef_b, bool relu, hipStream_t s);
+                     const float* coef_a, const float* coef_b, bool relu, hipStream_t s, uint8_t* mask = nullptr);
+
+const char* tail_conv1_refusal(int64_t M, int64_t Cin, int64_t Cout);
+void launch_tail_conv1_fwd(bool f16, const uint16_t* x3, const uint16_t* r, const float* coef, const float* coef2,
+                           const uint16_t* w, uint16_t* y, uint8_t* mask, uint16_t* x1, float* psum, float* psq,
+                           int64_t M, int Cin, int Cout, hipStream_t s);
 void launch_bn_bwd(int dtype, const void* dy, const void* dy2, const void* y, const void* x, int64_t M,
                    int64_t C, const float* gamma, const float* mean, const float* invstd, const float* coef,
                    float* dgamma, float* dbeta, void* dx, void* dz, float* workspace, bool relu, hipStream_t s);
diff --git a/csrc/kernels/mfma.h b/csrc/kernels/mfma.h
--- a/csrc/kernels/mfma.h
+++ b/csrc/kernels/mfma.h
@@ -14,6 +14,28 @@
 
 __device__ __forceinline__ f32x16_t mfma32(bf16x8_t a, bf16x8_t b, f32x16_t c) {
   return __builtin_amdgcn_mfma_f32_32x32x16_bf16(a, b, c, 0, 0, 0);
+}
+
+typedef _Float16 f16x8_t __attribute__((ext_vector_type(8)));
+typedef _Float16 f16x2_t __attribute__((ext_vector_type(2)));
+
+template <bool F16>
+__device__ __forceinline__ f32x16_t cmfma(bf16x8_t a, bf16x8_t b, f32x16_t c) {
+  if constexpr (F16)
+    return __builtin_amdgcn_mfma_f32_32x32x16_f16(__builtin_bit_cast(f16x8_t, a), __builtin_bit_cast(f16x8_t, b), c,
+                                                  0, 0, 0);
+  else
+    return __builtin_amdgcn_mfma_f32_32x32x16_bf16(a, b, c, 0, 0, 0);
+}
+template <bool F16>
+__device__ __forceinline__ uint32_t cpack(f32x2_t v) {
+  if constexpr (F16) return __builtin_bit_cast(uint32_t, __builtin_convertvector(v, f16x2_t));
+  else return __builtin_bit_cast(uint32_t, __builtin_convertvector(v, bf16x2_t));
+}
+template <bool F16>
+__device__ __forceinline__ float cunpack(uint32_t u, int h) {
+  if constexpr (F16) return (float)__builtin_bit_cast(_Float16, (uint16_t)(h ? (u >> 16) : (u & 0xffffu)));
+  else return __uint_as_float(h ? (u & 0xffff0000u) : (u << 16));
 }
 
 template <int RB>
diff --git a/csrc/kernels/tail_conv1_kernels.hip b/csrc/kernels/tail_conv1_kernels.hip
--- /dev/null
+++ b/csrc/kernels/tail_conv1_kernels.hip
@@ -0,0 +1,297 @@
+#include <stdexcept>
+#include <string>
+#include <type_traits>
+
+#include "bn_io.h"
+#include "common.h"
+#include "kernels.h"
+#include "mfma.h"
+
+namespace dpt {
+
+namespace tc1 {
+constexpr int BM = 128;
+constexpr int BK = 64;
+constexpr int kThreads = 256;
+constexpr int kRowBytes = BK * 2;
+constexpr int A_BYTES = BM * kRowBytes;
+constexpr uint32_t kOOB = 0xFFFFFF00u;
+
+__device__ __forceinline__ int swz(int row, int chunk) { return chunk ^ ((row >> 1) & 7); }
+
+template <int BN>
+__host__ __device__ constexpr int lds_epi() { return BM * (BN * 2 + 16) + 2 * (4 / (BN / 64)) * BN * 4; }
+template <int BN>
+__host__ __device__ constexpr int lds_main(int Cin, bool aff) {
+  const int main = A_BYTES + BN * kRowBytes + (aff ? 4 : 2) * Cin * 4, epi = lds_epi<BN>();
+  return main > epi ? main : epi;
+}
+}
+
+struct TailConv1Args {
+  const uint16_t* x3 = nullptr;
+  const uint16_t* r = nullptr;
+  const float* coef = nullptr;
+  const float* coef2 = nullptr;
+  const uint16_t* w = nullptr;
+  uint16_t* y = nullptr;
+  uint8_t* mask = nullptr;
+  uint16_t* x1 = nullptr;
+  float* psum = nullptr;
+  float* psq = nullptr;
+  int64_t M = 0;
+  int Cin = 0, m_tiles = 0, rev = 0;
+};
+
+template <typename IO>
+struct Rnd;
+template <>
+struct Rnd<BF16> {
+  __device__ static float up(uint32_t h) { return bf16_to_f32((uint16_t)h); }
+  __device__ static uint32_t down(float v) { return f32_to_bf16(v); }
+  __device__ static bool pos(uint32_t h) { return BF16::pos16(h); }
+};
+template <>
+struct Rnd<F16> {
+  __device__ static float up(uint32_t h) { return f16_to_f32((uint16_t)h); }
+  __device__ static uint32_t down(float v) { return F16::to16(v); }
+  __device__ static bool pos(uint32_t h) { return (float)__builtin_bit_cast(_Float16, (uint16_t)h) > 0.0f; }
+};
+
+template <typename IO, int BN, bool AFF>
+__global__ __launch_bounds__(tc1::kThreads, (BN == 64 && !AFF) ? 3 : 2) void tail_conv1_fwd_kernel(TailConv1Args p) {
+  using namespace tc1;
+  constexpr bool F16V = std::is_same<IO, F16>::value;
+  constexpr int WN = BN / 64, WM = 4 / WN, MI = BM / (WM * 32), NI = 2;
+  constexpr int B_PER_T = BN * 8 / kThreads;
+  constexpr int C_STRIDE = BN * 2 + 16;
+  typedef unsigned u32x4 __attribute__((ext_vector_type(4)));
+  extern __shared__ __attribute__((aligned(16))) unsigned char lds[];
+  unsigned char* la = lds;
+  unsigned char* lb = lds + A_BYTES;
+  float* lc = reinterpret_cast<float*>(lds + A_BYTES + BN * kRowBytes);
+
+  const int tid = threadIdx.x, lane = tid & 63, wid = tid >> 6;
+  const int wm = wid / WN, wn = wid % WN;
+  const int lr = lane & 31, lh = lane >> 5;
+  const int mt = p.rev ? p.m_tiles - 1 - (int)blockIdx.x : (int)blockIdx.x;
+  const int64_t m0 = (int64_t)mt * BM;
+  const int Cin = p.Cin, nk = Cin / BK;
+  const int mrow = Cin >> 3;
+  unsigned char* lm = lds + lds_main<BN>(Cin, AFF);
+
+  const int c = tid & 7, rb = tid >> 3;
+  const uint32_t nbytes = (uint32_t)(p.M * Cin * 2);
+  const __amdgpu_buffer_rsrc_t rx = __builtin_amdgcn_make_buffer_rsrc((void*)p.x3, 0, (int)nbytes, 0x00020000);
+  const __amdgpu_buffer_rsrc_t rr = __builtin_amdgcn_make_buffer_rsrc((void*)p.r, 0, (int)nbytes, 0x00020000);
+  uint32_t voff[4];
+  bool live[4];
+#pragma unroll
+  for (int i = 0; i < 4; ++i) {
+    const int64_t m = m0 + rb + 32 * i;
+    live[i] = m < p.M;
+    voff[i] = live[i] ? (uint32_t)((m * Cin + c * 8) * 2) : kOOB;
+  }
+  const uint16_t* wrow[B_PER_T];
+#pragma unroll
+  for (int i = 0; i < B_PER_T; ++i) wrow[i] = p.w + (int64_t)(rb + 32 * i) * Cin + c * 8;
+
+  u32x4 xa[4], ra[4];
+  u32x4 wb[B_PER_T];
+  auto load_a = [&](int i, int ks) {
+    const uint32_t o = live[i] ? voff[i] + (uint32_t)ks * kRowBytes : kOOB;
+    xa[i] = __builtin_amdgcn_raw_buffer_load_b128(rx, o, 0, 0);
+    ra[i] = __builtin_amdgcn_raw_buffer_load_b128(rr, o, 0, 0);
+  };
+  auto load_b = [&](int ks) {
+#pragma unroll
+    for (int i = 0; i < B_PER_T; ++i) wb[i] = *reinterpret_cast<const u32x4*>(wrow[i] + ks * BK);
+  };
+#pragma unroll
+  for (int i = 0; i < 4; ++i) load_a(i, 0);
+  load_b(0);
+  for (int i = tid; i < 2 * Cin; i += kThreads) {
+    lc[i] = p.coef[i];
+    if (AFF) lc[2 * Cin + i] = p.coef2[i];
+  }
+
+  f32x16_t acc[MI][NI];
+#pragma unroll
+  for (int i = 0; i < MI; ++i)
+#pragma unroll
+    for (int j = 0; j < NI; ++j)
+#pragma unroll
+      for (int e = 0; e < 16; ++e) acc[i][j][e] = 0.f;
+
+  __syncthreads();
+  for (int ks = 0; ks < nk; ++ks) {
+    const bool more = ks + 1 < nk;
+    float a[8], b[8], a2[8], b2[8];
+    const int ch0 = ks * BK + c * 8;
+#pragma unroll
+    for (int k = 0; k < 8; ++k) {
+      a[k] = lc[ch0 + k];
+      b[k] = lc[Cin + ch0 + k];
+      a2[k] = AFF ? lc[2 * Cin + ch0 + k] : 0.f;
+      b2[k] = AFF ? lc[3 * Cin + ch0 + k] : 0.f;
+    }
+    u32x4 yv[4];
+#pragma unroll
+    for (int i = 0; i < 4; ++i) {
+      const uint32_t xu[4] = {xa[i].x, xa[i].y, xa[i].z, xa[i].w};
+      const uint32_t ru[4] = {ra[i].x, ra[i].y, ra[i].z, ra[i].w};
+      float v[8], q[8];
+#pragma unroll
+      for (int k = 0; k < 8; ++k) {
+        v[k] = Rnd<IO>::up(k & 1 ? xu[k >> 1] >> 16 : xu[k >> 1] & 0xffffu);
+        q[k] = Rnd<IO>::up(k & 1 ? ru[k >> 1] >> 16 : ru[k >> 1] & 0xffffu);
+      }
+      if (more) load_a(i, ks + 1);
+      uint32_t h[8], msk = 0;
+#pragma unroll
+      for (int k = 0; k < 8; ++k) {
+        float o = __builtin_fmaf(v[k], a[k], b[k]);
+        if (AFF) o += __builtin_fmaf(q[k], a2[k], b2[k]);
+        else o += q[k];
+        o = o < 0.0f ? 0.0f : o;
+        h[k] = Rnd<IO>::down(o);
+        msk |= (Rnd<IO>::pos(h[k]) ? 1u : 0u) << k;
+      }
+      yv[i] = u32x4{h[0] | (h[1] << 16), h[2] | (h[3] << 16), h[4] | (h[5] << 16), h[6] | (h[7] << 16)};
+      const int row = rb + 32 * i;
+      lm[row * mrow + (ch0 >> 3)] = (uint8_t)msk;
+      if (live[i]) *reinterpret_cast<u32x4*>(p.y + (m0 + row) * Cin + ch0) = yv[i];
+      else yv[i] = u32x4{0u, 0u, 0u, 0u};
+    }
+    if (ks > 0) __syncthreads();
+#pragma unroll
+    for (int i = 0; i < 4; ++i) {
+      const int row = rb + 32 * i;
+      *reinterpret_cast<u32x4*>(la + row * kRowBytes + swz(row, c) * 16) = yv[i];
+    }
+#pragma unroll
+    for (int i = 0; i < B_PER_T; ++i) {
+      const int row = rb + 32 * i;
+      *reinterpret_cast<u32x4*>(lb + row * kRowBytes + swz(row, c) * 16) = wb[i];
+    }
+    if (more) load_b(ks + 1);
+    __syncthreads();
+#pragma unroll
+    for (int kk = 0; kk < BK / 16; ++kk) {
+      const int ch = kk * 2 + lh;
+      bf16x8_t fa[MI], fb[NI];
+#pragma unroll
+      for (int i = 0; i < MI; ++i) {
+        const int row = wm * (MI * 32) + i * 32 + lr;
+        fa[i] = *reinterpret_cast<const bf16x8_t*>(la + row * kRowBytes + swz(row, ch) * 16);
+      }
+#pragma unroll
+      for (int j = 0; j < NI; ++j) {
+        const int row = wn * 64 + j * 32 + lr;
+        fb[j] = *reinterpret_cast<const bf16x8_t*>(lb + row * kRowBytes + swz(row, ch) * 16);
+      }
+#pragma unroll
+      for (int i = 0; i < MI; ++i)
+#pragma unroll
+        for (int j = 0; j < NI; ++j) acc[i][j] = cmfma<F16V>(fa[i], fb[j], acc[i][j]);
+    }
+  }
+  __syncthreads();
+
+  float cs[NI], cq[NI];
+#pragma unroll
+  for (int j = 0; j < NI; ++j) { cs[j] = 0.f; cq[j] = 0.f; }
+#pragma unroll
+  for (int i = 0; i < MI; ++i)
+#pragma unroll
+    for (int j = 0; j < NI; ++j) {
+      const int col = wn * 64 + j * 32 + lr;
+      const int rbase = wm * (MI * 32) + i * 32 + 4 * lh;
+#pragma unroll
+      for (int e = 0; e < 16; e += 2) {
+        const int r0 = rbase + (e & 3) + 8 * (e >> 2);
+        const f32x2_t v = {acc[i][j][e], acc[i][j][e + 1]};
+        const uint32_t u = cpack<F16V>(v);
+        *reinterpret_cast<uint16_t*>(lds + r0 * C_STRIDE + col * 2) = (uint16_t)u;
+        *reinterpret_cast<uint16_t*>(lds + (r0 + 1) * C_STRIDE + col * 2) = (uint16_t)(u >> 16);
+        const float f0 = cunpack<F16V>(u, 0), f1 = cunpack<F16V>(u, 1);
+        cs[j] += f0 + f1;
+        cq[j] = __builtin_fmaf(f0, f0, __builtin_fmaf(f1, f1, cq[j]));
+      }
+    }
+  float* red = reinterpret_cast<float*>(lds + BM * C_STRIDE);
+#pragma unroll
+  for (int j = 0; j < NI; ++j) {
+    cs[j] += __shfl_xor(cs[j], 32, 64);
+    cq[j] += __shfl_xor(cq[j], 32, 64);
+    if (lh == 0) {
+      const int col = wn * 64 + j * 32 + lr;
+      red[wm * BN + col] = cs[j];
+      red[WM * BN + wm * BN + col] = cq[j];
+    }
+  }
+  __syncthreads();
+  if (tid < BN) {
+    float s = 0.f, q = 0.f;
+#pragma unroll
+    for (int w = 0; w < WM; ++w) { s += red[w * BN + tid]; q += red[WM * BN + w * BN + tid]; }
+    p.psum[(int64_t)tid * p.m_tiles + mt] = s;
+    p.psq[(int64_t)tid * p.m_tiles + mt] = q;
+  }
+  for (int j = tid; j < BM * mrow / 8; j += kThreads) {
+    if (m0 + (j * 8) / mrow < p.M)
+      *reinterpret_cast<uint2*>(p.mask + m0 * mrow + j * 8) = *reinterpret_cast<const uint2*>(lm + j * 8);
+  }
+  constexpr int CPR = BN / 8, RPP = kThreads / CPR, NPASS = BM / RPP;
+  const int oc = tid % CPR, orow = tid / CPR;
+#pragma unroll
+  for (int g = 0; g < NPASS; ++g) {
+    const int row = g * RPP + orow;
+    const int64_t m = m0 + row;
+    if (m < p.M)
+      *reinterpret_cast<uint4*>(p.x1 + m * BN + oc * 8) = *reinterpret_cast<const uint4*>(lds + row * C_STRIDE + oc * 16);
+  }
+}
+
+static size_t tail_conv1_lds(int Cin, int Cout, bool aff) {
+  const size_t front = Cout == 128 ? tc1::lds_main<128>(Cin, aff) : tc1::lds_main<64>(Cin, aff);
+  return front + (size_t)tc1::BM * (Cin / 8);
+}
+
+const char* tail_conv1_refusal(int64_t M, int64_t Cin, int64_t Cout) {
+  if (Cin < 64 || Cin % 64 != 0) return "needs Cin % 64 == 0 and Cin >= 64";
+  if (Cout != 64 && Cout != 128) return "needs Cout of 64 or 128 (one output-channel tile)";
+  if (!bn_supported(Cin)) return "Cin is not a fused-BatchNorm channel count";
+  if (M < 1) return "empty input";
+  if (M * Cin * 2 >= 0xFFFFFF00ll || Cout * Cin * 2 >= 0x7FFFFFFFll) return "operand tensors beyond 2^31 elements";
+  if (tail_conv1_lds((int)Cin, (int)Cout, true) > 65536) return "the coefficients and the mask tile do not fit the LDS";
+  if (conv_fwd_splits_for(M, (int)Cout, Cin, false) != 1 || conv_fwd_splits_for(M, (int)Cout, Cin, true) != 1)
+    return "the split-K policy splits this conv";
+  return nullptr;
+}
+
+constexpr int kTailReverse = 1;
+
+template <typename IO>
+static void tail_conv1_dispatch(const TailConv1Args& a, int Cout, bool aff, hipStream_t s) {
+  const dim3 grid((unsigned)a.m_tiles), block(tc1::kThreads);
+  const size_t lds = tail_conv1_lds(a.Cin, Cout, aff);
+#define DPT_TC1(BN, AFFV) \
+  hipLaunchKernelGGL((tail_conv1_fwd_kernel<IO, BN, AFFV>), grid, block, lds, s, a)
+  if (Cout == 128) { if (aff) DPT_TC1(128, true); else DPT_TC1(128, false); }
+  else { if (aff) DPT_TC1(64, true); else DPT_TC1(64, false); }
+#undef DPT_TC1
+}
+
+void launch_tail_conv1_fwd(bool f16, const uint16_t* x3, const uint16_t* r, const float* coef, const float* coef2,
+                           const uint16_t* w, uint16_t* y, uint8_t* mask, uint16_t* x1, float* psum, float* psq,
+                           int64_t M, int Cin, int Cout, hipStream_t s) {
+  if (const char* why = tail_conv1_refusal(M, Cin, Cout)) throw std::runtime_error(std::string("tail_conv1_fwd: ") + why);
+  TailConv1Args a;
+  a.x3 = x3; a.r = r; a.coef = coef; a.coef2 = coef2; a.w = w; a.y = y; a.mask = mask; a.x1 = x1;
+  a.psum = psum; a.psq = psq; a.M = M; a.Cin = Cin; a.m_tiles = conv_m_tiles(M); a.rev = kTailReverse;
+  if (f16) tail_conv1_dispatch<F16>(a, Cout, coef2 != nullptr, s);
+  else tail_conv1_dispatch<BF16>(a, Cout, coef2 != nullptr, s);
+}
+
+}
diff --git a/distributed_pytorch_training_amd/models/layers.py b/distributed_pytorch_training_amd/models/layers.py
--- a/distributed_pytorch_training_amd/models/layers.py
+++ b/distributed_pytorch_training_amd/models/layers.py
@@ -21,11 +21,12 @@
             return False
         return fused_bn.bn_act_supported(x, self.num_features)
 
-    def act(self, x: torch.Tensor, relu: bool, residual: Optional[torch.Tensor], pair: bool = False):
+    def act(self, x: torch.Tensor, relu: bool, residual: Optional[torch.Tensor], pair: bool = False,
+            consumer: Optional[nn.Module] = None):
         if self.training:
             return fused_bn.bn_act_train(x, residual, self.weight, self.bias, self.running_mean,
                                          self.running_var, self.num_batches_tracked, self.momentum,
-                                         self.eps, relu, pair)
+                                         self.eps, relu, pair, consumer)
         y = fused_bn.bn_act_eval(x, residual, self.weight, self.bias, self.running_mean,
                                  self.running_var, self.eps, relu)
         return (y, y) if pair else y
@@ -69,14 +70,14 @@
     return ds(x)
 
 
-def bn_act_block_out(bn: nn.Module, x: torch.Tensor, residual):
+def bn_act_block_out(bn: nn.Module, x: torch.Tensor, residual, consumer: Optional[nn.Module] = None):
     if isinstance(residual, DeferredBN):
         if (isinstance(bn, FusedBatchNorm2d) and bn.can_fuse(x) and bn.training
                 and residual.x.shape == x.shape and residual.x.dtype == x.dtype):
-            return fused_bn.bn2_add_relu_train(x, bn, residual.x, residual.bn)
+            return fused_bn.bn2_add_relu_train(x, bn, residual.x, residual.bn, consumer)
         residual = residual.materialize()
     if isinstance(bn, FusedBatchNorm2d) and bn.can_fuse(x):
-        return bn.act(x, True, residual, pair=True)
+        return bn.act(x, True, residual, pair=True, consumer=consumer)
     return bn_act(bn, x, True, residual)
 
 
diff --git a/distributed_pytorch_training_amd/models/resnet.py b/distributed_pytorch_training_amd/models/resnet.py
--- a/distributed_pytorch_training_amd/models/resnet.py
+++ b/distributed_pytorch_training_amd/models/resnet.py
@@ -59,7 +59,15 @@
         out = bn_act(self.bn1, self.conv1(xc))
         identity = xi if self.downsample is None else downsample_branch(self.downsample, xi, self.bn3)
         out = bn_act(self.bn2, self.conv2(out))
-        return bn_act_block_out(self.bn3, self.conv3(out), identity)
+        nxt = self.__dict__.get("dpt_tail_next")
+        return bn_act_block_out(self.bn3, self.conv3(out), identity, None if nxt is None else nxt.conv1)
+
+
+def link_tail_consumers(stages) -> None:
+    blocks = [b for stage in stages for b in stage]
+    for blk, nxt in zip(blocks, blocks[1:]):
+        if isinstance(blk, Bottleneck) and isinstance(nxt, Bottleneck):
+            blk.__dict__["dpt_tail_next"] = nxt
 
 
 class ResNet(nn.Module):
@@ -77,6 +85,7 @@
         self.layer4 = self._make_layer(block, 512, layers[3], stride=2)
         self.avgpool = nn.AdaptiveAvgPool2d((1, 1))
         self.fc = nn.Linear(512 * block.expansion, num_classes)
+        link_tail_consumers([self.layer1, self.layer2, self.layer3, self.layer4])
 
         for m in self.modules():
             if isinstance(m, nn.Conv2d):
diff --git a/distributed_pytorch_training_amd/ops/bn.py b/distributed_pytorch_training_amd/ops/bn.py
--- a/distributed_pytorch_training_amd/ops/bn.py
+++ b/distributed_pytorch_training_amd/ops/bn.py
@@ -7,9 +7,10 @@
 import os
 
 from . import native, native_available
-from .conv import COMPACT_RES, MASKED_NO_RES, take_bnb_partials
+from .conv import COMPACT_RES, MASKED_NO_RES, materialize_tail, take_bnb_partials
 
 BNR_FUSE = os.environ.get("DPT_BNR_FUSE", "1") != "0"
+TAIL_CONV1_FUSE = os.environ.get("DPT_TAIL_CONV1_FUSE", "1") != "0"
 
 
 def _cl(t: torch.Tensor) -> torch.Tensor:
@@ -54,11 +55,19 @@
 def _fwd(ctx, x, residual, weight, bias, running_mean, running_var, num_batches, momentum, eps, relu,
          pair=False, partials=None, links=(None, None)):
     ps, pq = partials if partials is not None else (None, None)
-    own_slot, res_slot = links
+    own_slot, res_slot = links[0], links[1]
+    defer = links[2] if len(links) > 2 else None
     mask = _relu_mask(x) if (own_slot is not None and relu and residual is not None) else None
-    y, mean, invstd, coef = native().bn_fwd_train(x, residual, weight, bias, running_mean, running_var,
-                                                  num_batches, float(momentum), float(eps), bool(relu), ps, pq,
-                                                  mask_out=mask)
+    if defer is not None:
+        _, mean, invstd, coef = native().bn_fwd_train(x, residual, weight, bias, running_mean, running_var,
+                                                      num_batches, float(momentum), float(eps), bool(relu), ps, pq,
+                                                      False)
+        y = torch.empty_like(x)
+        defer.update(x3=x, r=residual, coef=coef, coef2=None, y=y, mask=mask)
+    else:
+        y, mean, invstd, coef = native().bn_fwd_train(x, residual, weight, bias, running_mean, running_var,
+                                                      num_batches, float(momentum), float(eps), bool(relu), ps, pq,
+                                                      mask_out=mask)
     ctx.relu = bool(relu)
     ctx.has_res = residual is not None
     mask_from_x = ctx.relu and not ctx.has_res and not pair
@@ -120,7 +129,7 @@
 
     @staticmethod
     def forward(ctx, x, x2, w, b, rm, rv, nb, w2, b2, rm2, rv2, nb2, momentum, eps, momentum2, eps2,
-                partials, partials2, own_slot):
+                partials, partials2, own_slot, defer):
         C = native()
         ps, pq = partials if partials is not None else (None, None)
         ps2, pq2 = partials2 if partials2 is not None else (None, None)
@@ -129,7 +138,11 @@
         _, mean2, invstd2, coef2 = C.bn_fwd_train(x2, None, w2, b2, rm2, rv2, nb2, float(momentum2), float(eps2),
                                                   False, ps2, pq2, False)
         mask = _relu_mask(x) if own_slot is not None else None
-        y = C.bn_apply_aff(x, x2, coef, coef2, mask_out=mask)
+        if defer is not None:
+            y = torch.empty_like(x)
+            defer.update(x3=x, r=x2, coef=coef, coef2=coef2, y=y, mask=mask)
+        else:
+            y = C.bn_apply_aff(x, x2, coef, coef2, mask_out=mask)
         ctx.save_for_backward(x, x2, y, w, w2, mean, invstd, mean2, invstd2)
         ctx.set_materialize_grads(False)
         if own_slot is not None:
@@ -143,7 +156,7 @@
         if dy is None:
             dy, dy2 = dy2, None
         if dy is None:
-            return (None,) * 19
+            return (None,) * 20
         want = [ctx.needs_input_grad[i] for i in (2, 3, 7, 8)]
         want_params = any(want)
         C = native()
@@ -163,19 +176,48 @@
                                         bool(want_params), None)
         g = [dg, db, dg2, db2]
         g = [t if (want_params and want[i]) else None for i, t in enumerate(g)]
-        return (dx, dx2, g[0], g[1], None, None, None, g[2], g[3]) + (None,) * 10
-
-
-def bn2_add_relu_train(x, bn, x2, bn2):
+        return (dx, dx2, g[0], g[1], None, None, None, g[2], g[3]) + (None,) * 11
+
+
+def _tail_defer(x, own_slot, consumer):
+    if not (TAIL_CONV1_FUSE and consumer is not None and own_slot is not None and torch.is_grad_enabled()):
+        return None
+    w = getattr(consumer, "weight", None)
+    if w is None or w.dim() != 4 or tuple(w.shape[1:]) != (x.shape[1], 1, 1):
+        return None
+    if getattr(consumer, "dpt_native_conv", True) is False:
+        return None
+    m = x.shape[0] * x.shape[2] * x.shape[3]
+    return {} if native().conv1x1_tail_refusal(m, x.shape[1], w.shape[0]) is None else None
+
+
+def run_tail_consumer(out, defer, consumer) -> None:
+    yc = out[0]
+    yc._dpt_tail_pending = defer
+    try:
+        consumer(yc)
+    finally:
+        yc.__dict__.pop("_dpt_tail_pending", None)
+        if not defer.get("done"):
+            materialize_tail(defer)
+            defer.pop("conv", None)
+    if "conv" in defer:
+        yc._dpt_conv1_out = defer["conv"]
+
+
+def bn2_add_relu_train(x, bn, x2, bn2, consumer=None):
     x2 = _cl(x2.to(x.dtype))
     partials = x.__dict__.pop("_dpt_bn_partials", None)
     partials2 = x2.__dict__.pop("_dpt_bn_partials", None)
     own_slot = {} if (BNR_FUSE and x.dtype in (torch.bfloat16, torch.float16)) else None
+    defer = _tail_defer(x, own_slot, consumer)
     out = _BN2AddReLUPair.apply(x, x2, bn.weight, bn.bias, bn.running_mean, bn.running_var, bn.num_batches_tracked,
                                 bn2.weight, bn2.bias, bn2.running_mean, bn2.running_var, bn2.num_batches_tracked,
-                                bn.momentum, bn.eps, bn2.momentum, bn2.eps, partials, partials2, own_slot)
+                                bn.momentum, bn.eps, bn2.momentum, bn2.eps, partials, partials2, own_slot, defer)
     if own_slot is not None:
         out[1]._dpt_res_slot = own_slot
+    if defer is not None:
+        run_tail_consumer(out, defer, consumer)
     return out
 
 
@@ -187,7 +229,7 @@
 
 
 def bn_act_train(x: torch.Tensor, residual: Optional[torch.Tensor], weight, bias, running_mean, running_var,
-                 num_batches, momentum: float, eps: float, relu: bool, pair: bool = False):
+                 num_batches, momentum: float, eps: float, relu: bool, pair: bool = False, consumer=None):
     res_slot = None
     if residual is not None:
         if residual.dtype == x.dtype and residual.is_contiguous(memory_format=torch.channels_last):
@@ -197,10 +239,13 @@
     own_slot = {} if (pair and relu and residual is not None and BNR_FUSE
                       and x.dtype in (torch.bfloat16, torch.float16)) else None
     fn = _BNActTrainPair if pair else _BNActTrain
+    defer = _tail_defer(x, own_slot, consumer)
     out = fn.apply(x, residual, weight, bias, running_mean, running_var, num_batches, momentum, eps, relu,
-                   partials, (own_slot, res_slot))
+                   partials, (own_slot, res_slot, defer))
     if own_slot is not None:
         out[1]._dpt_res_slot = own_slot
+    if defer is not None:
+        run_tail_consumer(out, defer, consumer)
     return out
 
 
diff --git a/distributed_pytorch_training_amd/ops/conv.py b/distributed_pytorch_training_amd/ops/conv.py
--- a/distributed_pytorch_training_amd/ops/conv.py
+++ b/distributed_pytorch_training_amd/ops/conv.py
@@ -214,12 +214,43 @@
         return _backward(ctx, dy) + (None,) * 6
 
 
+def materialize_tail(pending) -> None:
+    if pending.get("done"):
+        return
+    x3, r, coef, coef2 = pending["x3"], pending["r"], pending["coef"], pending["coef2"]
+    c = x3.shape[1]
+    if coef2 is None:
+        native().bn_apply(x3, r, coef[:c], coef[c:], True, mask_out=pending["mask"], y_out=pending["y"])
+    else:
+        native().bn_apply_aff(x3, r, coef, coef2, mask_out=pending["mask"], y_out=pending["y"])
+    pending["done"] = True
+
+
+def _tail_fwd(x, w, stride, pad, out_hw, pending):
+    if pending["y"].data_ptr() != x.data_ptr() or tuple(out_hw) != (0, 0):
+        materialize_tail(pending)
+        return None
+    try:
+        out = native().conv1x1_tail_fwd(pending["x3"], pending["r"], pending["coef"], pending["coef2"], w, x,
+                                        pending["mask"], stride, pad)
+    except RuntimeError:
+        materialize_tail(pending)
+        return None
+    pending["done"] = True
+    return out
+
+
 class _ConvStats(torch.autograd.Function):
     @staticmethod
-    def forward(ctx, x, w, stride: int, pad: int, out_hw, bn_src, res_slot, compact_dres):
+    def forward(ctx, x, w, stride: int, pad: int, out_hw, bn_src, res_slot, compact_dres, pending):
         e0 = _mark()
-        y, ps, pq = native().conv_fwd(x, w, stride, pad, True, *out_hw)
-        _note("fwd", x, w, stride, pad, "stats", e0, out_hw)
+        fused = _tail_fwd(x, w, stride, pad, out_hw, pending) if pending is not None else None
+        if fused is not None:
+            y, ps, pq = fused
+            _note("fwd", x, w, stride, pad, "tail-apply+stats", e0, out_hw)
+        else:
+            y, ps, pq = native().conv_fwd(x, w, stride, pad, True, *out_hw)
+            _note("fwd", x, w, stride, pad, "stats", e0, out_hw)
         ctx.save_for_backward(x, w)
         ctx.stride, ctx.pad, ctx.bn_src, ctx.res_slot = stride, pad, bn_src, res_slot
         ctx.compact_dres = compact_dres
@@ -229,12 +260,20 @@
 
     @staticmethod
     def backward(ctx, dy, _dps, _dpq):
-        return _backward(ctx, dy) + (None,) * 6
+        return _backward(ctx, dy) + (None,) * 7
 
 
 def conv2d(x: torch.Tensor, w: torch.Tensor, stride: int, pad: int, bn_stats: bool = False,
            out_hw=(0, 0)) -> torch.Tensor:
     w = _cl(w)
+    done = x.__dict__.pop("_dpt_conv1_out", None)
+    if done is not None and done[0] is w and done[1:4] == (int(stride), int(pad), bool(bn_stats)) \
+            and tuple(out_hw) == (0, 0):
+        return done[4]
+    pending = x.__dict__.pop("_dpt_tail_pending", None)
+    if pending is not None and not bn_stats:
+        materialize_tail(pending)
+        pending = None
     if _FLIP["on"] and int(stride) == 1 and x.requires_grad:
         _FLIP["pending"].setdefault((w.data_ptr(), tuple(w.shape)), w)
     bn_src = x.__dict__.get("_dpt_bn_src")
@@ -247,8 +286,11 @@
                         and tuple(out_hw) == (0, 0) and res_slot is not None and res_slot.get("fold_s2"))
     if not bn_stats:
         return _Conv.apply(x, w, int(stride), int(pad), tuple(out_hw), bn_src, res_slot, compact_dres)
-    y, ps, pq = _ConvStats.apply(x, w, int(stride), int(pad), tuple(out_hw), bn_src, res_slot, compact_dres)
+    y, ps, pq = _ConvStats.apply(x, w, int(stride), int(pad), tuple(out_hw), bn_src, res_slot, compact_dres,
+                                 pending)
     y._dpt_bn_partials = (ps, pq)
+    if pending is not None:
+        pending["conv"] = (w, int(stride), int(pad), True, y)
     return y
 
 
```

Measured after the change: 12850 (median of 6 runs). 1.4% higher.
